# bigpon/QPNet

Measured on AMD Instinct MI355X. Metric: train steps/sec (batch-1 chunk-steps of RF+20000 samples, aggregate over GPUs), higher is better.
Workload: dtype f32; 1 GPU; config[1]: paper-size SI-QPNet (C=64,S=256,4F+4A) training step, forward+CE+backward+Adam on one chunk of 20900 samples (RF 946 + batch_length 19954), batch 1 per GPU; global_batch=1, parallelism=dp1 (utterance-sharded chunks, one flat-gradient all-reduce per step), backend=none, world_size=1, aux_1x1=frame rate (hoisted: K = 128 + one 4-deep step)

## Files before the change

qpnet_amd/csrc/train_bwd.hip:

```cpp
#include "train_common.h"
#include "train_post.h"
#include "qpn_handle.h"
#include <string.h>
#include <stdlib.h>
#include <math.h>

template <int MT>
__global__ __launch_bounds__(512) void k_post_bwd(TrainParams p, TrainBwd bw) {
    constexpr int TM = 16 * MT;
    extern __shared__ float sm[];
    const int S = p.S, Q = p.Q, LC = p.LC;
    const int ldp = tr_lda(Q > S ? Q : S), ldr = tr_lda(S);
    float* P = sm; float* R = sm + TM * ldp;
    const int b = blockIdx.y, t0 = blockIdx.x * TM;
    const int tid = threadIdx.x, lane = tid & 63, wave = tid >> 6;
    const int NTS = S / 16;
    const int npairs = (NTS + 1) / 2;
    const int np0 = wave < npairs ? wave : 0;
    const int pnt[2] = {2 * np0, (2 * np0 + 1 < NTS) ? 2 * np0 + 1 : 2 * np0};
    float my[2][MT][4], ms[2][MT][4];
    auto mask_load = [&](const float* src, float (&m)[2][MT][4]) {
#pragma unroll
        for (int j = 0; j < 2; ++j)
#pragma unroll
// ... 288 lines not shown
        rdg = *(const float4*)(DGS + (__umul24((unsigned)nw, (unsigned)p.LC) + 4u * sc4));
    };
    auto store_rows = [&](int t, float* B) {
        const int n = ly.s_out + t * 16 + srow;
        const bool in = n < N1;
        const float4 z = make_float4(0.f, 0.f, 0.f, 0.f);
        const float4 dx = (in && !LAST) ? make_float4(ra.x + rb2.x, ra.y + rb2.y, ra.z + rb2.z, ra.w + rb2.w) : z;
        const float4 sg = in ? rsg : z, th = in ? rth : z, dg = (in && n >= win0) ? rdg : z;
        float* d0 = B + (size_t)srow * ldx + 4 * sc4;
        *(float2*)d0 = make_float2(dx.x, dx.y); *(float2*)(d0 + 2) = make_float2(dx.z, dx.w);
        float* d1 = d0 + 16 * ldx; *(float2*)d1 = make_float2(sg.x, sg.y); *(float2*)(d1 + 2) = make_float2(sg.z, sg.w);
        float* d2 = d1 + 16 * ldx; *(float2*)d2 = make_float2(th.x, th.y); *(float2*)(d2 + 2) = make_float2(th.z, th.w);
        float* d3 = d2 + 16 * ldx; *(float2*)d3 = make_float2(dg.x, dg.y); *(float2*)(d3 + 2) = make_float2(dg.z, dg.w);
    };
    const int zrow = tid >> 6, zc2 = (tid & 63) * 2;
    float* const dmy = dummy + (size_t)(blockIdx.y * gridDim.x + blockIdx.x) * 2 * 128;
    int tprow[4], tpnext[4];
    auto load_taps = [&](int t, int (&tp)[4]) {
#pragma unroll
        for (int i = 0; i < 4; ++i) { const int n = ly.s_out + t * 16 + 4 * wave + i; tp[i] = taps[n < N1 ? n : N1 - 1]; }
    };
    float2 cwj[4], nwj[4]; float cpa[4], npa[4]; int cpoff = 0, npoff = 0;
    auto load_aux = [&](int t, float2 (&wj)[4], float (&pa)[4], int& poff) {
        const int n0 = ly.s_out + t * 16;
        poff = tr_pa_off(p, l, b, n0);
        const float2* w = p.WJ + n0 + 4 * (lane >> 4);
        const float* q4 = p.PA + poff + 16 * wave + (lane & 15);
#pragma unroll
        for (int i = 0; i < 4; ++i) wj[i] = w[i];
        pa[0] = q4[0]; pa[1] = q4[C]; pa[2] = q4[2 * C]; pa[3] = q4[3 * C];
    };
    load_rows(t_first);
    if constexpr (HOIST) load_aux(t_first, cwj, cpa, cpoff);
    load_taps(t_first, tprow);
    store_rows(t_first, sm);
    const int arow = lane & 15, ak = lane >> 4;
    const int c = 16 * wave + (lane & 15);
    for (int ti = 0; ti < t_count; ++ti) {
        const int t = t_first + ti, n0 = ly.s_out + t * 16;
        float* Dx = sm + (ti & 1) * 4 * 16 * ldx; float* Sg = Dx + 16 * ldx; float* Th = Sg + 16 * ldx; float* Dg = Th + 16 * ldx;
        { const int tn = t + 1 < t_last ? t + 1 : t_last; load_rows(tn); load_taps(tn, tpnext); if constexpr (HOIST) load_aux(tn, nwj, npa, npoff); }
        TR_LDS_BARRIER();
        float xa[4][4];
#pragma unroll
        for (int ks = 0; ks < 4; ++ks) { const float* ap = Dx + (size_t)arow * ldx + 16 * ks + ak; xa[ks][0] = ap[0]; xa[ks][1] = ap[4]; xa[ks][2] = ap[8]; xa[ks][3] = ap[12]; }
        __builtin_amdgcn_sched_barrier(0);
        f32x4 a0 = (f32x4){0, 0, 0, 0}, a1 = (f32x4){0, 0, 0, 0};
        if (!LAST) {
#pragma unroll
            for (int ks = 0; ks < 4; ks += 2) {
                a0 = __builtin_amdgcn_mfma_f32_16x16x4f32(xa[ks][0], wr[ks].x, a0, 0, 0, 0); a1 = __builtin_amdgcn_mfma_f32_16x16x4f32(xa[ks + 1][0], wr[ks + 1].x, a1, 0, 0, 0);
                a0 = __builtin_amdgcn_mfma_f32_16x16x4f32(xa[ks][1], wr[ks].y, a0, 0, 0, 0); a1 = __builtin_amdgcn_mfma_f32_16x16x4f32(xa[ks + 1][1], wr[ks + 1].y, a1, 0, 0, 0);
                a0 = __builtin_amdgcn_mfma_f32_16x16x4f32(xa[ks][2], wr[ks].z, a0, 0, 0, 0); a1 = __builtin_amdgcn_mfma_f32_16x16x4f32(xa[ks + 1][2], wr[ks + 1].z, a1, 0, 0, 0);
                a0 = __builtin_amdgcn_mfma_f32_16x16x4f32(xa[ks][3], wr[ks].w, a0, 0, 0, 0); a1 = __builtin_amdgcn_mfma_f32_16x16x4f32(xa[ks + 1][3], wr[ks + 1].w, a1, 0, 0, 0);
            }
        }
        float dzs[4], dzt[4];
#pragma unroll
        for (int i = 0; i < 4; ++i) {
            const int r = 4 * (lane >> 4) + i;
            const float dg = (a0[i] + a1[i]) + Dg[(size_t)r * ldx + c];
            const float sg = Sg[(size_t)r * ldx + c], th = Th[(size_t)r * ldx + c];
            tr_gate_bwd(dg, sg, th, dzs[i], dzt[i]);
            Dz[(size_t)r * ldz + c] = dzs[i];
            Dz[(size_t)r * ldz + C + c] = dzt[i];
        }
        float dacc[4] = {0.f, 0.f, 0.f, 0.f}, eacc[2] = {0.f, 0.f};
        if constexpr (HOIST) {
            const TrAuxBwd ab = tr_aux_bwd(cwj, cpa, dzs, dzt, lane);
#pragma unroll
            for (int k = 0; k < 4; ++k) dacc[k] = ab.d[k];
            eacc[0] = ab.e[0]; eacc[1] = ab.e[1];
            if ((lane & 15) == 0) { float* gq = Gp + 16 * wave + 4 * (lane >> 4); gq[0] = ab.gp[0]; gq[1] = ab.gp[1]; gq[2] = ab.gp[2]; gq[3] = ab.gp[3]; }
        }
        TR_LDS_BARRIER();
        float za[8][4];
#pragma unroll
        for (int ks = 0; ks < 8; ++ks) { const float* zp = Dz + (size_t)arow * ldz + 16 * ks + ak; za[ks][0] = zp[0]; za[ks][1] = zp[4]; za[ks][2] = zp[8]; za[ks][3] = zp[12]; }
        __builtin_amdgcn_sched_barrier(0);
        f32x4 acc[NJ];
#pragma unroll
        for (int j = 0; j < NJ; ++j) acc[j] = (f32x4){0, 0, 0, 0};
#pragma unroll
        for (int ks = 0; ks < 8; ++ks) {
#pragma unroll
            for (int j = 0; j < NJ; ++j) acc[j] = __builtin_amdgcn_mfma_f32_16x16x4f32(za[ks][0], w1[j][ks].x, acc[j], 0, 0, 0);
#pragma unroll
            for (int j = 0; j < NJ; ++j) acc[j] = __builtin_amdgcn_mfma_f32_16x16x4f32(za[ks][1], w1[j][ks].y, acc[j], 0, 0, 0);
#pragma unroll
            for (int j = 0; j < NJ; ++j) acc[j] = __builtin_amdgcn_mfma_f32_16x16x4f32(za[ks][2], w1[j][ks].z, acc[j], 0, 0, 0);
#pragma unroll
            for (int j = 0; j < NJ; ++j) acc[j] = __builtin_amdgcn_mfma_f32_16x16x4f32(za[ks][3], w1[j][ks].w, acc[j], 0, 0, 0);
        }
        {
#pragma unroll
            for (int k = 0; k < 4; ++k) {
                const int r = zrow + 4 * k;
                float* d = DZg + (__umul24((unsigned)(n0 + r), 2u * C) + zc2);
                d = n0 + r < N1 ? d : dmy + zc2;
                *(float2*)d = *(const float2*)(Dz + (size_t)r * ldz + zc2);
            }
        }
#pragma unroll
        for (int j = 0; j < NJ; ++j) {
            const int nt = wave + 4 * j;
            if (nt >= NTK) continue;
#pragma unroll
            for (int i = 0; i < 4; ++i) Os[(size_t)(4 * (lane >> 4) + i) * ldo + 16 * nt + (lane & 15)] = acc[j][i];
        }
        TR_LDS_BARRIER();
#pragma unroll
        for (int i = 0; i < 4; ++i) {
            const int r = 4 * wave + i, n = n0 + r;
            const bool in = n < N1;
            const float own = Os[(size_t)r * ldo + lane] + Dx[(size_t)r * ldx + lane];
            float* da = DAout + (__umul24((unsigned)n, (unsigned)C) + lane);
            *(in ? da : dmy + lane) = own;
            const float past = Os[(size_t)r * ldo + C + lane];
            float* db = DBout + (__umul24((unsigned)tprow[i], (unsigned)C) + lane);
            db = in ? db : dmy + 128 + lane;
            if (ly.adaptive) atomicAdd(db, past);
            else *db = past;
            if constexpr (!HOIST) if (lane < Ap) {
                float* dh = DH + (__umul24((unsigned)n, (unsigned)Ap) + lane);
                atomicAdd(in ? dh : dmy + 192 + lane, Os[(size_t)r * ldo + 2 * C + lane]);
            }
        }
        if constexpr (HOIST) {
            if (lane < 16) {
                float* dp = bw.DPA + cpoff + 16 * wave + lane;
                atomicAdd(dp, dacc[0]); atomicAdd(dp + C, dacc[1]); atomicAdd(dp + 2 * C, dacc[2]); atomicAdd(dp + 3 * C, dacc[3]);
                float* ep = bw.EB + (size_t)(l * TR_EB_SLOTS + (blockIdx.x & (TR_EB_SLOTS - 1))) * 2 * C + 16 * wave + lane;
                atomicAdd(ep, eacc[0]); atomicAdd(ep + C, eacc[1]);
            }
            if (tid < 16 && n0 + tid < N1) GWl[n0 + tid] = (Gp[tid] + Gp[16 + tid]) + (Gp[32 + tid] + Gp[48 + tid]);
        }
        store_rows(t + 1 < t_last ? t + 1 : t_last, sm + ((ti + 1) & 1) * 4 * 16 * ldx);
#pragma unroll
        for (int i = 0; i < 4; ++i) tprow[i] = tpnext[i];
        if constexpr (HOIST) {
#pragma unroll
            for (int i = 0; i < 4; ++i) { cwj[i] = nwj[i]; cpa[i] = npa[i]; }
            cpoff = npoff;
        }
    }
}

struct Wg2 {
    const float* A; const float* A2; size_t A_lstride; int lda, M;
    int rowsA;
    int bmode; const float* B1; const float* B2; size_t B_lstride; int ldb, N, Nvalid;
    int rowsB;
    const float* hup; const int* tap; int C, Ap;
    const int* xc;
    int nb, nlayers;
    float* slab; int gstage;
    int row0A[TR_MAXL], row0B[TR_MAXL], R[TR_MAXL];
    int goff[TR_MAXL], gbias[TR_MAXL], tap_off[TR_MAXL], dil[TR_MAXL];
    int ldc, ncol_groups;
};

struct Wg2L {
    const float* A; const float* A2; const float* B1; const float* B2; const float* hup; const int* tap;
    int lda, ldb, M, Ng, Nvalid, rowsA, rowsB, row0A, row0B, C, Ap, dil, nb, ncol0, rend;
    unsigned uR;
};

template <int NB>
__device__ __forceinline__ void wg_taps(const Wg2L& q, int rs, int (&tp)[NB], bool b_act, int b_row0, int b_rstep) {
#pragma unroll
    for (int k = 0; k < NB; ++k) {
        const int r = b_row0 + k * b_rstep, rr = rs + r;
        int v = 0;
        if (b_act && r < 32 && rr < q.rend) {
            const unsigned b = q.nb > 1 ? (unsigned)rr / q.uR : 0u; const int i = rr - (int)(b * q.uR);
            const int nloc = q.row0B + i;
            v = q.tap ? q.tap[(size_t)b * q.rowsB + nloc] : nloc - q.dil;
        }
        tp[k] = v;
    }
}

template <int BMODE, int NA, int NB>
__device__ __forceinline__ void wg_fetch(const Wg2L& q, int rs, float4 (&ra)[NA], float4 (&ra2)[NA], float4 (&rb)[NB], float4 (&rb2)[NB], const int (&tpv)[NB],
                                         bool a_act, int a_row0, int a_rstep, int a_col, bool b_act, int b_row0, int b_rstep, int b_col) {
#pragma unroll
    for (int k = 0; k < NA; ++k) {
        const int r = a_row0 + k * a_rstep, rr = rs + r;
        float4 v = make_float4(0.f, 0.f, 0.f, 0.f), v2 = v;
        if (a_act && r < 32 && rr < q.rend && a_col < q.M) {
            const unsigned b = q.nb > 1 ? (unsigned)rr / q.uR : 0u; const int i = rr - (int)(b * q.uR);
            const size_t o = ((size_t)b * q.rowsA + q.row0A + i) * q.lda + a_col;
            v = *(const float4*)(q.A + o);
            if (q.A2) v2 = *(const float4*)(q.A2 + o);
        }
        ra[k] = v; ra2[k] = v2;
    }
#pragma unroll
    for (int k = 0; k < NB; ++k) {
        const int r = b_row0 + k * b_rstep, rr = rs + r;
        const int n = q.ncol0 + b_col;
        float4 v = make_float4(0.f, 0.f, 0.f, 0.f), v2 = make_float4(1.f, 1.f, 1.f, 1.f);
        if (b_act && r < 32 && rr < q.rend && b_col < q.Ng && n < q.Nvalid) {
            const unsigned b = q.nb > 1 ? (unsigned)rr / q.uR : 0u; const int i = rr - (int)(b * q.uR);
            const int nloc = q.row0B + i;
            const size_t row = (size_t)b * q.rowsB + nloc;
            if (BMODE <= 1) v = *(const float4*)(q.B1 + row * q.ldb + n);
            else if (BMODE == 2) { v = *(const float4*)(q.B1 + row * q.ldb + n); v2 = *(const float4*)(q.B2 + row * q.ldb + n); }
            else {
                if (n < q.C) v = *(const float4*)(q.B1 + row * q.C + n);
                else if (n < 2 * q.C) v = *(const float4*)(q.B1 + ((size_t)b * q.rowsB + tpv[k]) * q.C + (n - q.C));
                else v = *(const float4*)(q.hup + row * q.Ap + (n - 2 * q.C));
            }
        }
        rb[k] = v; rb2[k] = v2;
    }
}

template <int BMODE, int MPW, int NTMAX>
__global__ __launch_bounds__(256) void k_wgrad2(Wg2 w, int nch) {
    extern __shared__ float sm[];
    constexpr int RS = 32;
    constexpr int NA = 2 * MPW;
    constexpr int NB = (NTMAX + 1) / 2 + 1;
    const int y = blockIdx.y, ch = blockIdx.x, zg = blockIdx.z;
    const int Mp = (w.M + 15) & ~15, Ng = w.N / w.ncol_groups, Np = (Ng + 15) & ~15;
    const int ldA = tr_ldt(Mp), ldB = tr_ldt(Np);
    float* As = sm; float* Bs = sm + RS * ldA;
    const int tid = threadIdx.x, lane = tid & 63, wave = tid >> 6;
    const int MT = Mp / 16, NT = Np / 16;
    const int Rl = w.R[y];
    const int64_t total = (int64_t)Rl * w.nb;
    const int64_t per = ((total + nch - 1) / nch + RS - 1) / RS * RS;
    const int rbeg = (int)(per * ch), rend = (int)(per * ch + per < total ? per * ch + per : total);
    Wg2L q;
    q.A = w.A + (size_t)y * w.A_lstride; q.A2 = w.A2 ? w.A2 + (size_t)y * w.A_lstride : nullptr;
    q.B1 = w.B1 + (size_t)y * w.B_lstride; q.B2 = w.B2 ? w.B2 + (size_t)y * w.B_lstride : nullptr;
    q.hup = w.hup; q.tap = (w.tap && w.tap_off[y] >= 0) ? w.tap + w.tap_off[y] : nullptr;
    q.lda = w.lda; q.ldb = w.ldb; q.M = w.M; q.Ng = Ng; q.Nvalid = w.Nvalid; q.rowsA = w.rowsA; q.rowsB = w.rowsB;
    q.row0A = w.row0A[y]; q.row0B = w.row0B[y]; q.C = w.C; q.Ap = w.Ap; q.dil = w.dil[y]; q.nb = w.nb; q.ncol0 = zg * Ng; q.rend = rend;
    q.uR = (unsigned)(Rl > 0 ? Rl : 1);
    const int gbias = zg == 0 ? w.gbias[y] : -1, goff = w.goff[y];
    const int A4 = Mp / 4, B4 = Np / 4;
    const int a_col = (tid % A4) * 4, a_row0 = tid / A4, a_rstep = 256 / A4;
    const int b_rstep = 256 / B4 > 0 ? 256 / B4 : 1;
    const int b_col = (tid % B4) * 4, b_row0 = tid / B4;
    const bool a_act = tid < a_rstep * A4, b_act = tid < b_rstep * B4;
    f32x4 acc[MPW][NTMAX];
#pragma unroll
    for (int a = 0; a < MPW; ++a)
#pragma unroll
        for (int b = 0; b < NTMAX; ++b) acc[a][b] = (f32x4){0, 0, 0, 0};
    float csum = 0.f;
    float4 ra[NA], ra2[NA], rb[NB], rb2[NB];
    int tpv[NB];
#pragma unroll
    for (int k = 0; k < NB; ++k) tpv[k] = 0;
    if (BMODE == 3 && rbeg < rend) wg_taps<NB>(q, rbeg, tpv, b_act, b_row0, b_rstep);
    if (rbeg < rend) wg_fetch<BMODE, NA, NB>(q, rbeg, ra, ra2, rb, rb2, tpv, a_act, a_row0, a_rstep, a_col, b_act, b_row0, b_rstep, b_col);
    if (BMODE == 3 && rbeg + RS < rend) wg_taps<NB>(q, rbeg + RS, tpv, b_act, b_row0, b_rstep);
    const int g = lane >> 4, cl = lane & 15;
    for (int rs = rbeg; rs < rend; rs += RS) {
#pragma unroll
        for (int k = 0; k < NA; ++k) {
            const int r = a_row0 + k * a_rstep;
            if (a_act && r < RS) {
                float4 v = ra[k];
                v.x += ra2[k].x; v.y += ra2[k].y; v.z += ra2[k].z; v.w += ra2[k].w;
                *(float4*)(As + (size_t)r * ldA + a_col) = v;
            }
        }
#pragma unroll
        for (int k = 0; k < NB; ++k) {
            const int r = b_row0 + k * b_rstep;
            if (b_act && r < RS) {
                float4 v = rb[k];
                if (BMODE == 1) { v.x = fmaxf(v.x, 0.f); v.y = fmaxf(v.y, 0.f); v.z = fmaxf(v.z, 0.f); v.w = fmaxf(v.w, 0.f); }
                else if (BMODE == 2) { v.x *= rb2[k].x; v.y *= rb2[k].y; v.z *= rb2[k].z; v.w *= rb2[k].w; }
                *(float4*)(Bs + (size_t)r * ldB + b_col) = v;
            }
        }
        __syncthreads();
        if (rs + RS < rend) wg_fetch<BMODE, NA, NB>(q, rs + RS, ra, ra2, rb, rb2, tpv, a_act, a_row0, a_rstep, a_col, b_act, b_row0, b_rstep, b_col);
        if (BMODE == 3 && rs + 2 * RS < rend) wg_taps<NB>(q, rs + 2 * RS, tpv, b_act, b_row0, b_rstep);
        if (gbias >= 0 && tid < q.M) { float s = 0.f; for (int r = 0; r < RS; ++r) s += As[r * ldA + tid]; csum += s; }
#pragma unroll
        for (int ks = 0; ks < RS / 4; ++ks) {
            float bfr[NTMAX];
#pragma unroll
            for (int nt = 0; nt < NTMAX; ++nt) bfr[nt] = nt < NT ? Bs[(4 * ks + g) * ldB + 16 * nt + cl] : 0.f;
#pragma unroll
            for (int mi = 0; mi < MPW; ++mi) {
                const int mt = wave + 4 * mi;
                if (mt < MT) {
                    const float a = As[(4 * ks + g) * ldA + 16 * mt + cl];
#pragma unroll
                    for (int nt = 0; nt < NTMAX; ++nt)
                        if (nt < NT) acc[mi][nt] = __builtin_amdgcn_mfma_f32_16x16x4f32(a, bfr[nt], acc[mi][nt], 0, 0, 0);
                }
            }
        }
        __syncthreads();
    }
    float* out = w.slab + (size_t)ch * w.gstage;
#pragma unroll
    for (int mi = 0; mi < MPW; ++mi) {
        const int mt = wave + 4 * mi;
        if (mt >= MT) continue;
#pragma unroll
        for (int nt = 0; nt < NTMAX; ++nt) {
            if (nt >= NT) continue;
#pragma unroll
            for (int i = 0; i < 4; ++i) {
                const int m = 16 * mt + 4 * (lane >> 4) + i, n = 16 * nt + (lane & 15);
                if (m < q.M && n < Ng) out[goff + (size_t)m * w.ldc + q.ncol0 + n] = acc[mi][nt][i];
            }
        }
    }
    if (gbias >= 0 && tid < q.M) out[gbias + tid] = csum;
}

template <int BMODE, int MPW, int NTMAX>
static int launch_wgrad2(const Wg2& w, int nch, hipStream_t stream) {
    const int Mp = (w.M + 15) & ~15, Np = ((w.N / w.ncol_groups) + 15) & ~15;
    if (Mp / 16 > 4 * MPW || Np / 16 > NTMAX) return -1;
    const size_t lds = (size_t)32 * (tr_ldt(Mp) + tr_ldt(Np)) * sizeof(float);
    if (lds > 64 * 1024) (void)hipFuncSetAttribute((const void*)k_wgrad2<BMODE, MPW, NTMAX>, hipFuncAttributeMaxDynamicSharedMemorySize, (int)lds);
    hipLaunchKernelGGL((k_wgrad2<BMODE, MPW, NTMAX>), dim3(nch, w.nlayers, w.ncol_groups), dim3(256), lds, stream, w, nch);
    return 0;
}
template <int BMODE>
static bool wgrad2_mode(const Wg2& w, int nch, hipStream_t stream) {
    if (launch_wgrad2<BMODE, 1, 4>(w, nch, stream) == 0) return true;
    if (launch_wgrad2<BMODE, 4, 4>(w, nch, stream) == 0) return true;
    if (launch_wgrad2<BMODE, 2, 12>(w, nch, stream) == 0) return true;
    if (launch_wgrad2<BMODE, 4, 8>(w, nch, stream) == 0) return true;
    return false;
}
struct UpArgs { const float* h; const float* DHUP; float* gflat; int64_t up_w, up_b; float gscale; int U, Ap, A, F, N1, nfr, B; };
static UpArgs up_args(const TrainParams& p, const TrainBwd& bw) {
    UpArgs u; u.h = p.h; u.DHUP = bw.DHUP; u.gflat = bw.gflat; u.gscale = bw.gscale; u.U = p.U; u.Ap = p.Ap; u.A = p.A; u.F = p.F; u.N1 = p.N1;
    u.up_w = p.up_w; u.up_b = p.up_b; u.B = p.B;
    const int64_t q0 = (int64_t)p.F * p.U - p.N1;
    u.nfr = p.U > 0 ? (int)(((int64_t)p.F * p.U - 1) / p.U - q0 / p.U + 1) : 0;
    return u;
}
__device__ __forceinline__ void up_bwd_body(const UpArgs& p, int fx, int b, int tid, int nthr) {
    __shared__ float hcol[64];
    __shared__ float red[4];
    const int U = p.U, Ap = p.Ap, A = p.A;
    const int64_t q0 = (int64_t)p.F * U - p.N1;
    const int f = (int)(q0 / U) + fx;
    float dsum = 0.f;
    for (int a0 = 0; a0 < A; a0 += 64) {
        __syncthreads();
        if (tid < 64) hcol[tid] = (a0 + tid < A && f < p.F) ? p.h[((size_t)b * A + a0 + tid) * p.F + f] : 0.f;
        __syncthreads();
        for (int j = tid; j < U; j += nthr) {
            const int64_t n = (int64_t)f * U + j - q0;
            if (n < 0 || n >= p.N1 || f >= p.F) continue;
            const float* row = p.DHUP + ((size_t)b * p.N1 + n) * Ap + a0;
            float acc = 0.f;
            const int na = A - a0 < 64 ? A - a0 : 64;
            const int nq = na >> 2;
            float4 v[16];
#pragma unroll
            for (int q = 0; q < 16; ++q) v[q] = *(const float4*)(row + 4 * (q < nq ? q : 0));
#pragma unroll
            for (int q = 0; q < 16; ++q)
                if (q < nq) { acc += v[q].x * hcol[4 * q] + v[q].y * hcol[4 * q + 1] + v[q].z * hcol[4 * q + 2] + v[q].w * hcol[4 * q + 3]; dsum += (v[q].x + v[q].y) + (v[q].z + v[q].w); }
            for (int a = 4 * nq; a < na; ++a) { const float v1 = row[a]; acc += v1 * hcol[a]; dsum += v1; }
            atomicAdd(&p.gflat[p.up_w + j], acc * p.gscale);
        }
    }
    for (int s = 32; s >= 1; s >>= 1) dsum += __shfl_xor(dsum, s);
    if ((tid & 63) == 0) red[tid >> 6] = dsum;
    __syncthreads();
    if (tid == 0) { float a = 0.f; for (int k = 0; k < nthr / 64; ++k) a += red[k]; atomicAdd(&p.gflat[p.up_b], a * p.gscale); }
}

template <int BMODE, int MPW, int NT, bool TWO_A>
__device__ __forceinline__ void wgrad3_body(const Wg2& w, const int nch, const int ch, const int y, const int zg) {
    extern __shared__ float sm[];
    constexpr int RS = 32, Mp = 64 * MPW, Np = 16 * NT;
    constexpr int ldA = ((Mp + 15) / 32) * 32 + 16, ldB = ((Np + 15) / 32) * 32 + 16;
    constexpr int A4 = Mp / 4, ARS = 256 / A4, NA = RS / ARS;
    constexpr int B4 = Np / 4, BRS = 256 / B4, NB = (RS + BRS - 1) / BRS;
    static_assert(256 % A4 == 0 && RS % ARS == 0, "A staging must tile the stage's rows exactly");
    constexpr int BUF = RS * (ldA + ldB);
    float* As = sm; float* Bs = sm + RS * ldA;
    const int tid = threadIdx.x, lane = tid & 63, wave = tid >> 6;
    const int Rl = w.R[y];
    const int64_t total = (int64_t)Rl * w.nb;
    const int64_t per = ((total + nch - 1) / nch + RS - 1) / RS * RS;
    const int rbeg = (int)(per * ch), rend = (int)(per * ch + per < total ? per * ch + per : total);
    const float* A = w.A + (size_t)y * w.A_lstride;
    const float* A2 = TWO_A ? w.A2 + (size_t)y * w.A_lstride : nullptr;
    const float* B1 = BMODE == 4 ? nullptr : w.B1 + (size_t)y * w.B_lstride;
    const float* B2 = w.B2 ? w.B2 + (size_t)y * w.B_lstride : nullptr;
    const int* tap = BMODE == 3 ? w.tap + w.tap_off[y] : nullptr;
    const int row0A = w.row0A[y], row0B = w.row0B[y], ncol0 = zg * Np;
    const unsigned uR = (unsigned)(Rl > 0 ? Rl : 1);
    const bool multi = w.nb > 1;
    const int gbias = zg == 0 ? w.gbias[y] : -1, goff = w.goff[y];
    const int a_col = (tid % A4) * 4, a_row0 = tid / A4;
    const int b_col = (tid % B4) * 4, b_row0 = tid / B4;
    const int n = ncol0 + b_col;
    const bool b_act = tid < BRS * B4;
    const bool b_pad = n >= w.Nvalid;
    const float* bbase; int bstride; bool use_tap = false;
    if (BMODE == 3) {
        if (n < w.C) { bbase = B1 + n; bstride = w.C; }
        else if (n < 2 * w.C) { bbase = B1 + (n - w.C); bstride = w.C; use_tap = true; }
        else { bbase = w.hup + (b_pad ? 0 : n - 2 * w.C); bstride = w.Ap; }
    } else if (BMODE == 4) { bbase = nullptr; bstride = 0; }
    else { bbase = B1 + n; bstride = w.ldb; }
    const ptrdiff_t b2off = (BMODE == 2) ? (B2 - B1) : 0;

    f32x4 acc[MPW][NT];
#pragma unroll
    for (int a = 0; a < MPW; ++a)
#pragma unroll
        for (int b = 0; b < NT; ++b) acc[a][b] = (f32x4){0, 0, 0, 0};
    float4 cs4 = make_float4(0.f, 0.f, 0.f, 0.f);
    float4 ra[NA], ra2[NA], rb[NB], rb2[NB];
    int tpv[NB];
    int rbi[NB];
    unsigned okA = 0, okB = 0;

    const unsigned a_voff = (unsigned)a_row0 * (unsigned)w.lda + (unsigned)a_col, a_kstep = (unsigned)ARS * (unsigned)w.lda;
    const unsigned b_voff = (unsigned)b_row0 * (unsigned)w.ldb + (unsigned)n, b_kstep = (unsigned)BRS * (unsigned)w.ldb;

    auto rowsplit = [&](int rr, int& b, int& i) { if (multi) { b = (int)((unsigned)rr / uR); i = rr - b * (int)uR; } else { b = 0; i = rr; } };
    auto stage_fast = [&](int rs, int& b0, int& i0) {
        rowsplit(rs, b0, i0);
        return rs + RS <= rend && i0 + RS <= (int)uR;
    };
    auto taps = [&](int rs) {
        int b0, i0;
        if (stage_fast(rs, b0, i0)) {
            const int* tst = tap + ((size_t)b0 * w.rowsB + row0B + i0);
#pragma unroll
            for (int k = 0; k < NB; ++k) { const int r = b_row0 + k * BRS; tpv[k] = tst[r < RS ? r : b_row0]; }
            return;
        }
#pragma unroll
        for (int k = 0; k < NB; ++k) {
            const int r = b_row0 + k * BRS;
            int rr = rs + r; rr = rr < rend ? rr : rend - 1;
            int b, i; rowsplit(rr, b, i);
            const int nloc = row0B + i;
            tpv[k] = tap[(size_t)b * w.rowsB + nloc];
        }
    };
    auto fetch = [&](int rs) {
        const float* pa[NA]; const float* pb[NB]; const int* pi[NB];
        int b0, i0;
        if (stage_fast(rs, b0, i0)) {
            const float* Ast = A + ((size_t)b0 * w.rowsA + row0A + i0) * w.lda;
#pragma unroll
            for (int k = 0; k < NA; ++k) pa[k] = Ast + (k * a_kstep + a_voff);
            okA = ~0u;
            const size_t brow = (size_t)b0 * w.rowsB + row0B + i0;
            const float* bsrc = BMODE == 3 ? bbase + (size_t)b0 * w.rowsB * bstride : B1 + brow * w.ldb;
#pragma unroll
            for (int k = 0; k < NB; ++k) {
                const int r = b_row0 + k * BRS;
                if (BMODE == 4) pi[k] = w.xc + brow + (r < RS ? r : b_row0);
                else if (BMODE == 3) {
                    const unsigned row = use_tap ? (unsigned)tpv[k] : (unsigned)(row0B + i0 + (r < RS ? r : b_row0));
                    pb[k] = bsrc + __umul24(row, (unsigned)bstride);
                } else pb[k] = bsrc + ((r < RS ? k * b_kstep : 0u) + b_voff);
            }
            okB = b_pad ? 0u : ~0u;
        } else {
            okA = 0; okB = 0;
#pragma unroll
            for (int k = 0; k < NA; ++k) {
                const int r = a_row0 + k * ARS;
                int rr = rs + r; const bool ok = rr < rend; rr = ok ? rr : rend - 1;
                int b, i; rowsplit(rr, b, i);
                pa[k] = A + (((size_t)b * w.rowsA + row0A + i) * w.lda + a_col);
                okA |= ok ? 1u << k : 0u;
            }
#pragma unroll
            for (int k = 0; k < NB; ++k) {
                const int r = b_row0 + k * BRS;
                int rr = rs + r; const bool ok = r < RS && rr < rend && !b_pad; rr = rr < rend ? rr : rend - 1;
                int b, i; rowsplit(rr, b, i);
                const size_t row = (size_t)b * w.rowsB + ((BMODE == 3 && use_tap) ? tpv[k] : row0B + i);
                if (BMODE == 4) pi[k] = w.xc + row; else pb[k] = bbase + row * bstride;
                okB |= ok ? 1u << k : 0u;
            }
        }
#pragma unroll
        for (int k = 0; k < NA; ++k) {
            ra[k] = *(const float4*)pa[k];
            if (TWO_A) ra2[k] = *(const float4*)(pa[k] + (A2 - A));
        }
        if (b_act) {
#pragma unroll
            for (int k = 0; k < NB; ++k) {
                if (BMODE == 4) rbi[k] = *pi[k];
                else {
                    rb[k] = *(const float4*)pb[k];
                    if (BMODE == 2) rb2[k] = *(const float4*)(pb[k] + b2off);
                }
            }
        }
    };
    if (rbeg < rend) {
        if (BMODE == 3) taps(rbeg);
        fetch(rbeg);
        if (BMODE == 3 && rbeg + RS < rend) taps(rbeg + RS);
    }
    const int g = lane >> 4, cl = lane & 15;
    auto to_lds = [&](int buf) {
        float* Ab = As + buf * BUF; float* Bb = Bs + buf * BUF;
#pragma unroll
        for (int k = 0; k < NA; ++k) {
            float4 v = ra[k];
            if (TWO_A) { v.x += ra2[k].x; v.y += ra2[k].y; v.z += ra2[k].z; v.w += ra2[k].w; }
            { const bool ok = (okA >> k) & 1u; v.x = ok ? v.x : 0.f; v.y = ok ? v.y : 0.f; v.z = ok ? v.z : 0.f; v.w = ok ? v.w : 0.f; }
            cs4.x += v.x; cs4.y += v.y; cs4.z += v.z; cs4.w += v.w;
            *(float4*)(Ab + (size_t)(a_row0 + k * ARS) * ldA + a_col) = v;
        }
        if (b_act) {
#pragma unroll
            for (int k = 0; k < NB; ++k) {
                const int r = b_row0 + k * BRS;
                if (r < RS) {
                    float4 v;
                    if (BMODE == 4) { const int dlt = rbi[k] - n; v = make_float4(dlt == 0 ? 1.f : 0.f, dlt == 1 ? 1.f : 0.f, dlt == 2 ? 1.f : 0.f, dlt == 3 ? 1.f : 0.f); }
                    else v = rb[k];
                    if (BMODE == 1) { v.x = fmaxf(v.x, 0.f); v.y = fmaxf(v.y, 0.f); v.z = fmaxf(v.z, 0.f); v.w = fmaxf(v.w, 0.f); }
                    else if (BMODE == 2) { v.x *= rb2[k].x; v.y *= rb2[k].y; v.z *= rb2[k].z; v.w *= rb2[k].w; }
                    { const bool ok = (okB >> k) & 1u; v.x = ok ? v.x : 0.f; v.y = ok ? v.y : 0.f; v.z = ok ? v.z : 0.f; v.w = ok ? v.w : 0.f; }
                    *(float4*)(Bb + (size_t)r * ldB + b_col) = v;
                }
            }
        }
    };
    auto ksteps = [&](int buf, int k0, int k1) {
        const float* Ab = As + buf * BUF; const float* Bb = Bs + buf * BUF;
#pragma unroll
        for (int ks = k0; ks < k1; ++ks) {
            float bfr[NT];
#pragma unroll
            for (int nt = 0; nt < NT; ++nt) bfr[nt] = Bb[(4 * ks + g) * ldB + 16 * nt + cl];
#pragma unroll
            for (int mi = 0; mi < MPW; ++mi) {
                const float a = Ab[(4 * ks + g) * ldA + 16 * (wave + 4 * mi) + cl];
#pragma unroll
                for (int nt = 0; nt < NT; ++nt) acc[mi][nt] = __builtin_amdgcn_mfma_f32_16x16x4f32(a, bfr[nt], acc[mi][nt], 0, 0, 0);
            }
        }
    };
    for (int rs = rbeg; rs < rend; rs += RS) {
        to_lds(0);
        __syncthreads();
        if (rs + RS < rend) {
            fetch(rs + RS);
            if (BMODE == 3 && rs + 2 * RS < rend) taps(rs + 2 * RS);
        }
        ksteps(0, 0, RS / 4);
        __syncthreads();
    }
    float* out = w.slab + (size_t)ch * w.gstage;
#pragma unroll
    for (int mi = 0; mi < MPW; ++mi) {
        const int mt = wave + 4 * mi;
#pragma unroll
        for (int nt = 0; nt < NT; ++nt) {
#pragma unroll
            for (int i = 0; i < 4; ++i) {
                const int m = 16 * mt + 4 * (lane >> 4) + i, nn = 16 * nt + (lane & 15);
                out[goff + (size_t)m * w.ldc + ncol0 + nn] = acc[mi][nt][i];
            }
        }
    }
    if (gbias >= 0) {
        *(float4*)(sm + (size_t)a_row0 * Mp + a_col) = cs4;
        __syncthreads();
        if (tid < Mp) { float s = 0.f; for (int r = 0; r < ARS; ++r) s += sm[r * Mp + tid]; out[gbias + tid] = s; }
    }
}
template <int BMODE, int MPW, int NT, bool TWO_A, int MINW = 1>
__global__ __launch_bounds__(256, MINW) void k_wgrad3(Wg2 w, int nch) {
    wgrad3_body<BMODE, MPW, NT, TWO_A>(w, nch, blockIdx.x, blockIdx.y, blockIdx.z);
}

#ifndef QPN_WGRAD_MINW
#define QPN_WGRAD_MINW 2
#endif
template <int BMODE, int MPW, int NT, bool TWO_A>
static void launch_wgrad3_k(const Wg2& w, int nch, size_t lds, hipStream_t stream) {
    constexpr int MINW = (MPW == 4 && NT == 4 && !TWO_A) ? QPN_WGRAD_MINW : 1;
    if (lds > 64 * 1024) (void)hipFuncSetAttribute((const void*)k_wgrad3<BMODE, MPW, NT, TWO_A, MINW>, hipFuncAttributeMaxDynamicSharedMemorySize, (int)lds);
    hipLaunchKernelGGL((k_wgrad3<BMODE, MPW, NT, TWO_A, MINW>), dim3(nch, w.nlayers, w.ncol_groups), dim3(256), lds, stream, w, nch);
}
template <int BMODE, int MPW, int NT>
static bool wgrad3_fits(const Wg2& w) {
    const int Ng = w.N / w.ncol_groups;
    if (w.bmode != BMODE) return false;
    if (w.rowsB >= (1 << 24) || (int64_t)w.rowsB * (w.C > w.ldb ? w.C : w.ldb) >= (1ll << 32)) return false;
    if (w.M != 64 * MPW || Ng != 16 * NT || w.N % w.ncol_groups || (w.Nvalid != w.N && (w.ncol_groups != 1 || w.Nvalid % 4))) return false;
    if (BMODE == 3 && (w.ldb != w.C || w.ncol_groups != 1 || (w.C % 4) || (w.Ap % 4) || !w.tap)) return false;
    if (BMODE == 3) for (int l = 0; l < w.nlayers; ++l) if (w.tap_off[l] < 0) return false;
    return true;
}
template <int MPW, int NT> static constexpr size_t wgrad3_lds() { return (size_t)32 * (tr_ldt(64 * MPW) + tr_ldt(16 * NT)) * sizeof(float); }
template <int BMODE, int MPW, int NT>
static bool launch_wgrad3(const Wg2& w, int nch, hipStream_t stream) {
    if (!wgrad3_fits<BMODE, MPW, NT>(w)) return false;
    const size_t lds = wgrad3_lds<MPW, NT>();
    if (w.A2) launch_wgrad3_k<BMODE, MPW, NT, true>(w, nch, lds, stream);
    else launch_wgrad3_k<BMODE, MPW, NT, false>(w, nch, lds, stream);
    return true;
}
static bool wgrad3_any(const Wg2& w, int nch, bool generic, hipStream_t stream) {
    if (w.bmode == 4) return launch_wgrad3<4, 1, 8>(w, nch, stream) || launch_wgrad3<4, 1, 4>(w, nch, stream);
    if (generic) return false;
    switch (w.bmode) {
    case 3: return launch_wgrad3<3, 2, 11>(w, nch, stream) || launch_wgrad3<3, 2, 8>(w, nch, stream) || launch_wgrad3<3, 1, 7>(w, nch, stream);
    case 0: return launch_wgrad3<0, 1, 4>(w, nch, stream) || launch_wgrad3<0, 4, 4>(w, nch, stream);
    case 1: return launch_wgrad3<1, 4, 4>(w, nch, stream);
    default: return false;
    }
}

static int wgrad_col_groups(int M, int N) {
    const int nt_max = M <= 64 ? 4 : M <= 128 ? 12 : 8;
    for (int g = 1; g <= N / 16; ++g)
        if (N % g == 0 && (N / g) % 4 == 0 && (N / g + 15) / 16 <= nt_max) return g;
    return 1;
}

static bool wgrad2_any(const Wg2& w, int nch, bool generic, hipStream_t stream) {
    if (w.M > 256 && w.bmode != 4) {
        bool ok = true;
        for (int m0 = 0; m0 < w.M && ok; m0 += 256) {
            Wg2 sub = w;
            sub.A = w.A + m0; if (w.A2) sub.A2 = w.A2 + m0;
            sub.M = w.M - m0 < 256 ? w.M - m0 : 256;
            for (int l = 0; l < w.nlayers; ++l) { sub.goff[l] = w.goff[l] + m0 * w.ldc; if (w.gbias[l] >= 0) sub.gbias[l] = w.gbias[l] + m0; }
            sub.ncol_groups = wgrad_col_groups(sub.M, sub.N);
            ok = wgrad2_any(sub, nch, generic, stream);
        }
        return ok;
    }
    if (wgrad3_any(w, nch, generic, stream)) return true;
    switch (w.bmode) {
    case 4: return false;
    case 1: return wgrad2_mode<1>(w, nch, stream);
    case 2: return wgrad2_mode<2>(w, nch, stream);
    case 3: return wgrad2_mode<3>(w, nch, stream);
    default: return wgrad2_mode<0>(w, nch, stream);
    }
}

__global__ void k_reduce_grad_s(const float* __restrict__ slab, const int* __restrict__ gdst, const int* __restrict__ gdst_list, const int* __restrict__ gzero, int n_gzero,
                                int nch, int gstage, int64_t n, float* __restrict__ g, float scale, int append_scale, int s0, int s1, int skip0, int skip1, int tail,
                                const int* __restrict__ status, int flag_again) {
    int64_t i = (int64_t)blockIdx.x * blockDim.x + threadIdx.x + s0;
    if (flag_again && append_scale && i == s0) g[n + 1] = (status && *status) ? 1.f : 0.f;
    if (i < s1) {
        if (i >= skip0 && i < skip1) return;
        const int k0 = gdst[i], k1 = gdst[i + 1];
        if (k0 == k1) return;
        float a = 0.f;
        const float* sp = slab + i;
        int c = 0;
        for (; c + 8 <= nch; c += 8) {
            float v[8];
#pragma unroll
            for (int k = 0; k < 8; ++k) v[k] = sp[(size_t)(c + k) * gstage];
            a += ((v[0] + v[1]) + (v[2] + v[3])) + ((v[4] + v[5]) + (v[6] + v[7]));
        }
        for (; c < nch; ++c) a += sp[(size_t)c * gstage];
        a *= scale;
        for (int k = k0; k < k1; ++k) g[gdst_list[k]] = a;
        return;
    }
    if (!tail) return;
    const int64_t j = i - s1;
    if (j < n_gzero) g[gzero[j]] = 0.f;
    else if (append_scale && j < n_gzero + 4 && !(flag_again && j == n_gzero + 1)) g[n + (j - n_gzero)] = j == n_gzero ? scale : (j == n_gzero + 1 && status && *status) ? 1.f : 0.f;
}

__global__ __launch_bounds__(256) void k_causal_bwd(TrainParams p, TrainBwd bw, int rows_per_wg, int CB) {
    extern __shared__ float tab[];
    const int C = p.C, Q = p.Q;
    const int tid = threadIdx.x;
    const int64_t total = (int64_t)p.B * p.N1;
    const int64_t r0 = (int64_t)blockIdx.x * rows_per_wg, r1 = r0 + rows_per_wg < total ? r0 + rows_per_wg : total;
    for (int cb = 0; cb < C; cb += CB) {
        const int cbv = C - cb < CB ? C - cb : CB;
        for (int i = tid; i < 2 * Q * CB; i += 256) tab[i] = 0.f;
        __syncthreads();
        const int cpr = cbv;
        for (int64_t idx = r0 * cpr + tid; idx < r1 * cpr; idx += 256) {
            const int64_t rr = idx / cpr; const int c = (int)(idx - rr * cpr);
            const int b = (int)(rr / p.N1), n = (int)(rr - (int64_t)b * p.N1);
            const size_t o = ((size_t)b * p.N1 + n) * C + cb + c;
            const float v = bw.DXA[0][o] + bw.DXB[0][o];
            const int64_t xo = (int64_t)p.T - p.N0 + n;
            int64_t s0 = p.x[(size_t)b * p.T + xo] % Q, s1 = p.x[(size_t)b * p.T + xo + 1] % Q;
            if (s0 < 0) s0 += Q;
            if (s1 < 0) s1 += Q;
            atomicAdd(&tab[(0 * Q + s0) * CB + c], v);
            atomicAdd(&tab[(1 * Q + s1) * CB + c], v);
        }
        __syncthreads();
        for (int i = tid; i < 2 * Q * cbv; i += 256) {
            const int c = i / (2 * Q), qt = i - c * 2 * Q, q = qt >> 1, tp = qt & 1;
            const float v = tab[(tp * Q + q) * CB + c];
            if (v != 0.f) atomicAdd(&bw.gflat[p.causal_w + ((size_t)(cb + c) * Q + q) * 2 + tp], v * bw.gscale);
        }
        for (int c = tid; c < cbv; c += 256) {
            float s = 0.f;
            for (int q = 0; q < Q; ++q) s += tab[(0 * Q + q) * CB + c];
            atomicAdd(&bw.gflat[p.causal_b + cb + c], s * bw.gscale);
        }
        __syncthreads();
    }
}

__global__ __launch_bounds__(128) void k_up_bwd(UpArgs u) { up_bwd_body(u, blockIdx.x, blockIdx.y, threadIdx.x, 128); }

__global__ __launch_bounds__(128) void k_aux_tail(AuxArgs p) {
    __shared__ float hrow[1024];
    __shared__ float red[2];
    const AuxGeom& ag = p.g;
    const int C = p.C, A = p.A, L = p.L, tid = threadIdx.x;
    const int bx = blockIdx.x;
    float v = 0.f;
    const bool role_a = bx < L * A;
    if (role_a) {
        const int l = bx / A, a = bx - l * A, n = tid;
        const size_t wi = (n < C ? ag.auxS[l] + (size_t)n * A : ag.auxT[l] + (size_t)(n - C) * A) + a;
        const float va = p.flat[wi];
        float e = 0.f;
        {
            float ev[TR_EB_SLOTS];
#pragma unroll
            for (int k = 0; k < TR_EB_SLOTS; ++k) ev[k] = p.EB[(size_t)(l * TR_EB_SLOTS + k) * 2 * C + n];
#pragma unroll
            for (int k = 0; k < TR_EB_SLOTS; ++k) e += ev[k];
        }
        float acc = 0.f;
        for (int b = 0; b < p.B; ++b) {
            const float* hb = p.h + ((size_t)b * A + a) * p.F + p.ffirst;
            const float* D = p.DPA + (size_t)(l * p.B + b) * (p.nfr + 1) * 2 * C + n;
            for (int f0 = 0; f0 < p.nfr; f0 += 1024) {
                const int nf = p.nfr - f0 < 1024 ? p.nfr - f0 : 1024;
                __syncthreads();
                for (int i = tid; i < nf; i += 128) hrow[i] = hb[f0 + i];
                __syncthreads();
                int f = 0;
                for (; f + 64 <= nf; f += 64) {
                    float d[64];
#pragma unroll
                    for (int k = 0; k < 64; ++k) d[k] = D[(size_t)(f0 + f + k) * 2 * C];
#pragma unroll
                    for (int k = 0; k < 64; ++k) acc += d[k] * hrow[f + k];
                }
                for (; f + 16 <= nf; f += 16) {
                    float d[16];
#pragma unroll
                    for (int k = 0; k < 16; ++k) d[k] = D[(size_t)(f0 + f + k) * 2 * C];
#pragma unroll
                    for (int k = 0; k < 16; ++k) acc += d[k] * hrow[f + k];
                }
                for (; f < nf; ++f) acc += D[(size_t)(f0 + f) * 2 * C] * hrow[f];
            }
        }
        p.gflat[wi] = (acc + p.flat[p.up_b] * e) * p.gscale;
        v = va * e;
    } else {
        const int j = bx - L * A;
        const int q0 = p.F * p.U - p.N1;
        const int items = L * p.B * p.nfr;
        for (int it = tid; it < items; it += 128) {
            const int fx = it % p.nfr, lb = it / p.nfr, l = lb / p.B;
            const int n = (p.ffirst + fx) * p.U + j - q0;
            if (n >= ag.s_out[l] && n < p.N1) v += p.GW[(size_t)lb * p.N1 + n];
        }
    }
    for (int sft = 32; sft >= 1; sft >>= 1) v += __shfl_xor(v, sft);
    if ((tid & 63) == 0) red[tid >> 6] = v;
    __syncthreads();
    if (tid == 0) {
        if (role_a) atomicAdd(p.gflat + p.up_b, (red[0] + red[1]) * p.gscale);
        else p.gflat[p.up_w + (bx - L * A)] = (red[0] + red[1]) * p.gscale;
    }
}

struct AdamReports { int* h_status; double* h_loss; const double* d_loss; };
__device__ __forceinline__ void adam_update(float* __restrict__ w, float* __restrict__ m, float* __restrict__ v, int64_t i, float gi,
                                            float lr, float b1, float b2, float eps, float wd, float bc1, float bc2_sqrt) {
    if (wd != 0.f) gi += wd * w[i];
    const float mi = m[i] + (gi - m[i]) * (1.0f - b1);
    const float vi = v[i] * b2 + (1.0f - b2) * gi * gi;
    m[i] = mi; v[i] = vi;
    const float denom = sqrtf(vi) / bc2_sqrt + eps;
    w[i] = w[i] - (lr / bc1) * (mi / denom);
}
__global__ void k_adam(float* __restrict__ w, const float* __restrict__ g, float* __restrict__ m, float* __restrict__ v, int64_t n,
                       float lr, float b1, float b2, float eps, float wd, float bc1, float bc2_sqrt, const float* __restrict__ den, int* __restrict__ status, AdamReports rep) {
    int64_t i = (int64_t)blockIdx.x * blockDim.x + threadIdx.x;
    const bool peer = den && den[1] > 0.f;
    const bool skip = peer || (status && *status);
    if (blockIdx.x == 0) {
        if (rep.h_loss && threadIdx.x < 64) rep.h_loss[threadIdx.x] = rep.d_loss[threadIdx.x];
        if (threadIdx.x == 0 && status) {
            int st = *status;
            if (peer && !st) { st = 8; atomicOr(status, 8); }
            if (rep.h_status) *rep.h_status = st;
            if (!skip) atomicAdd((unsigned long long*)(status + 2), 1ull);
        }
    }
    if (i >= n || skip) return;
    float gi = g[i];
    if (den) gi = gi / den[0];
    adam_update(w, m, v, i, gi, lr, b1, b2, eps, wd, bc1, bc2_sqrt);
}

__device__ __forceinline__ double block_sum_f64(double x, double* red) {
    for (int sft = 32; sft >= 1; sft >>= 1) x += __shfl_xor(x, sft);
    if ((threadIdx.x & 63) == 0) red[threadIdx.x >> 6] = x;
    __syncthreads();
    return (red[0] + red[1]) + (red[2] + red[3]);
}
__global__ __launch_bounds__(256) void k_grad_sumsq(const float* __restrict__ g, int64_t n, double* __restrict__ part) {
    __shared__ double red[4];
    const int64_t nq = n >> 2, nthr = (int64_t)gridDim.x * 256, t = (int64_t)blockIdx.x * 256 + threadIdx.x;
    double acc = 0.0;
    if ((reinterpret_cast<uintptr_t>(g) & 15) == 0) {
        const float4* g4 = reinterpret_cast<const float4*>(g);
#pragma unroll 4
        for (int64_t q = t; q < nq; q += nthr) {
            const float4 x = g4[q];
            acc += (double)x.x * (double)x.x; acc += (double)x.y * (double)x.y; acc += (double)x.z * (double)x.z; acc += (double)x.w * (double)x.w;
        }
    } else {
#pragma unroll 4
        for (int64_t q = t; q < nq; q += nthr) {
            const float x0 = g[4 * q], x1 = g[4 * q + 1], x2 = g[4 * q + 2], x3 = g[4 * q + 3];
            acc += (double)x0 * (double)x0; acc += (double)x1 * (double)x1; acc += (double)x2 * (double)x2; acc += (double)x3 * (double)x3;
        }
    }
    if (t == nq % nthr) for (int64_t i = nq * 4; i < n; ++i) acc += (double)g[i] * (double)g[i];
    const double s = block_sum_f64(acc, red);
    if (threadIdx.x == 0) part[blockIdx.x] = s;
}

__global__ __launch_bounds__(256) void k_adam_clip(float* __restrict__ w, const float* __restrict__ g, float* __restrict__ m, float* __restrict__ v, int64_t n,
                                                   float lr, float b1, float b2, float eps, float wd, float bc1, float bc2_sqrt, const float* __restrict__ den, int* __restrict__ status, AdamReports rep,
                                                   const double* __restrict__ part, int npart, float max_norm, double* __restrict__ d_norm, double* h_norm) {
    __shared__ double red[4];
    int64_t i = (int64_t)blockIdx.x * blockDim.x + threadIdx.x;
    double total = sqrt(block_sum_f64((int)threadIdx.x < npart ? part[threadIdx.x] : 0.0, red));
    if (den) total = total / (double)den[0];
    const bool bad = !isfinite(total);
    const bool peer = den && den[1] > 0.f;
    const bool skip = bad || peer || (status && *status);
    if (blockIdx.x == 0) {
        if (rep.h_loss && threadIdx.x < 64) rep.h_loss[threadIdx.x] = rep.d_loss[threadIdx.x];
        if (threadIdx.x == 0) {
            *d_norm = total;
            if (h_norm) *h_norm = total;
            if (status) {
                int st = *status;
                if (peer && !st) { st = 8; atomicOr(status, 8); }
                if (bad) { st |= 1 << 16; atomicOr(status, 1 << 16); }
                if (rep.h_status) *rep.h_status = st;
                if (!skip) atomicAdd((unsigned long long*)(status + 2), 1ull);
            }
        }
    }
    if (i >= n || skip) return;
    const double c = (double)max_norm / (total + 1e-6);
    const float coef = c < 1.0 ? (float)c : 1.0f;
    float gi = g[i];
    if (den) gi = gi / den[0];
    gi = __fmul_rn(gi, coef);
    adam_update(w, m, v, i, gi, lr, b1, b2, eps, wd, bc1, bc2_sqrt);
}

__device__ __forceinline__ void zero_dx_slice(const TrainParams& p, const TrainBwd& bw, int j, int b, size_t part, size_t nparts, int t, int nthr) {
    const int C = p.C;
    const TrLayer ly = p.layers[j];
    const size_t nDX = (size_t)p.B * p.N1 * C;
    float* A = bw.DXA[0] + (size_t)j * nDX + (size_t)b * p.N1 * C;
    float* Bq = bw.DXB[0] + (size_t)j * nDX + (size_t)b * p.N1 * C;
    const int a0 = j == 0 ? 0 : ly.s_in, a1 = ly.s_out;
    const int b0 = ly.adaptive ? 0 : p.N1 - ly.dilation, b1 = p.N1;
    const size_t na = (size_t)(a1 - a0) * C / 4, nb = (size_t)(b1 > b0 ? b1 - b0 : 0) * C / 4;
    const float4 z = make_float4(0.f, 0.f, 0.f, 0.f);
    const size_t nh = p.hoist ? (size_t)(p.nfr + 1) * 2 * C / 4 : (j == 0 ? (size_t)p.N1 * p.Ap / 4 : 0);
    const size_t ne = (p.hoist && b == 0) ? (size_t)TR_EB_SLOTS * 2 * C / 4 : 0;
    float* H = p.hoist ? bw.DPA + (size_t)(j * p.B + b) * (p.nfr + 1) * 2 * C : bw.DHUP + (size_t)b * p.N1 * p.Ap;
    for (size_t i = part * nthr + t; i < na + nb + nh + ne; i += nparts * nthr) {
        if (i < na) ((float4*)(A + (size_t)a0 * C))[i] = z;
        else if (i < na + nb) ((float4*)(Bq + (size_t)(b0 > 0 ? b0 : 0) * C))[i - na] = z;
        else if (i < na + nb + nh) ((float4*)H)[i - na - nb] = z;
        else ((float4*)(bw.EB + (size_t)j * TR_EB_SLOTS * 2 * C))[i - na - nb - nh] = z;
    }
}
__global__ void k_zero_dx(TrainParams p, TrainBwd bw) {
    zero_dx_slice(p, bw, blockIdx.y, blockIdx.z, blockIdx.x, gridDim.x, threadIdx.x, blockDim.x);
}

void qpn_launch_zero_dx(const TrainParams& p, const TrainBwd& bw, hipStream_t stream) {
    hipLaunchKernelGGL(k_zero_dx, dim3(64, p.L, p.B), dim3(256), 0, stream, p, bw);
}

static void launch_reduce_early(const TrainBwd& bw, hipStream_t st, int tail, int nch_side) {
    const TrainSlabs& sl = *bw.sl;
    const int64_t n = (int64_t)(sl.g_early1 - sl.g_early0) + (tail ? bw.n_gzero + 4 : 0);
    hipLaunchKernelGGL(k_reduce_grad_s, dim3((unsigned)((n + 255) / 256)), dim3(256), 0, st, bw.slab, bw.gdst, bw.gdst_list, bw.gzero, bw.n_gzero,
                       nch_side, bw.gstage, bw.n_params, bw.gflat, bw.gscale, bw.append_scale, sl.g_early0, sl.g_early1, 0, 0, tail, bw.status, 0);
}
static void launch_up_bwd(const TrainParams& p, const TrainBwd& bw, hipStream_t st) {
    const UpArgs u = up_args(p, bw);
    hipLaunchKernelGGL(k_up_bwd, dim3(u.nfr, p.B), dim3(128), 0, st, u);
}

static void launch_aux_tail(const TrainParams& p, const TrainBwd& bw, const AuxGeom& ag, hipStream_t st) {
    hipLaunchKernelGGL(k_aux_tail, dim3(p.L * p.A + p.U), dim3(128), 0, st, tr_aux_args(p, &bw, ag));
}

int qpn_launch_grad_tail(const TrainParams& p, const TrainBwd& bw, const AuxGeom* ag, hipStream_t stream, bool early_done, bool up_done) {
    const int C = p.C, Q = p.Q, B = p.B, N1 = p.N1;
    const TrainSlabs& sl = *bw.sl;
    hipLaunchKernelGGL(k_reduce_grad_s, dim3((unsigned)(((int64_t)bw.gstage + (up_done ? 0 : bw.n_gzero + 4) + 255) / 256)), dim3(256), 0, stream, bw.slab, bw.gdst, bw.gdst_list, bw.gzero, bw.n_gzero,
                       bw.nch, bw.gstage, bw.n_params, bw.gflat, bw.gscale, bw.append_scale, 0, bw.gstage, early_done ? sl.g_early0 : 0, early_done ? sl.g_early1 : 0, up_done ? 0 : 1, bw.status, bw.append_scale == 1 ? 1 : 0);
    {
        const int64_t total = (int64_t)B * N1;
        const int nwg = 128, rpw = (int)((total + nwg - 1) / nwg);
        if (sl.g_cw < 0) {
            int CB = C < 64 ? C : 64;
            while (CB > 1 && (size_t)2 * Q * CB * sizeof(float) > 128 * 1024) CB /= 2;
            const size_t lds_c = (size_t)2 * Q * CB * sizeof(float);
            if (lds_c > 160 * 1024) { qpn_set_error("causal-table gradient: n_quantize too large for the LDS histogram"); return QPN_EINVAL; }
            if (lds_c > 48 * 1024) QPN_HIP(hipFuncSetAttribute((const void*)k_causal_bwd, hipFuncAttributeMaxDynamicSharedMemorySize, (int)lds_c));
            hipLaunchKernelGGL(k_causal_bwd, dim3(nwg), dim3(256), lds_c, stream, p, bw, rpw, CB);
        }
        if (p.U > 0 && !up_done && !p.hoist) launch_up_bwd(p, bw, stream);
        if (p.hoist && ag && !up_done) launch_aux_tail(p, bw, *ag, stream);
    }
    qpn_prof_mark(PG_GRAD_TAIL, stream);
    QPN_HIP(hipGetLastError());
    return QPN_OK;
}

bool qpn_stack_bwd_fits(const TrainParams& p);
int qpn_launch_stack_bwd(const TrainParams& p, const TrainBwd& bw, const StackQ& q, const TrainKnobs& k, hipStream_t stream);

void qpn_launch_post_fb(const TrainParams& p, const TrainBwd& bw, hipStream_t stream) {
    constexpr int MTW = 5;
    const size_t ldsw = (size_t)16 * MTW * (tr_lda(256) + 2 * tr_lda(64)) * sizeof(float);
    (void)hipFuncSetAttribute((const void*)k_post_fb_w<MTW>, hipFuncAttributeMaxDynamicSharedMemorySize, (int)ldsw);
    hipLaunchKernelGGL((k_post_fb_w<MTW>), dim3((p.BL + 16 * MTW - 1) / (16 * MTW), p.B), dim3(512), ldsw, stream, p, bw, 1);
}

int qpn_launch_bwd(const TrainParams& p, const TrainBwd& bw, const TrainKnobs& k, const AuxGeom& ag, const StackQ* sq, hipStream_t stream, bool post_done) {
    const int C = p.C, S = p.S, Q = p.Q, L = p.L, B = p.B, N1 = p.N1, BL = p.BL;
    const TrainSlabs& sl = *bw.sl;
    const bool off32 = N1 < (1 << 24) && (int64_t)N1 * (p.LC > 2 * C ? p.LC : 2 * C) < (1ll << 32);
    const bool persist = C == 64 && (p.Ktp == 176 || p.hoist) && p.Ap <= 64 && off32 && k.persist_bwd;
    const bool stack_q = persist && k.stack_q_bwd && sq && sq->flags && p.qctl && qpn_stack_bwd_fits(p);
    const bool wr_summed = stack_q;
    const size_t nDX = (size_t)B * N1 * C;
    const size_t lds_post = (size_t)16 * (tr_lda(Q > S ? Q : S) + tr_lda(S)) * sizeof(float);
    const size_t lds_layer = (size_t)16 * (4 * tr_lda(C) + tr_lda(2 * C)) * sizeof(float);
    if (lds_post > 160 * 1024 || lds_layer > 160 * 1024) { qpn_set_error("backward tiles do not fit LDS"); return QPN_EINVAL; }
    hipStream_t side = bw.side; hipEvent_t ev_fork = bw.ev_fork, ev_join = bw.ev_join;
    const bool overlap = side && !qpn_prof_serial() && !k.serial;
    const bool post_wide = S == 256 && Q == 256 && C == 64 && (p.LC == 256 || p.LC == 512) && k.post_wide;
    const bool zero_in_post = post_wide && k.zero_in_post;
    if (post_done) { }
    else if (!zero_in_post) qpn_launch_zero_dx(p, bw, stream);
    if (post_done) { }
    else if (post_wide) {
        constexpr int MTW = 5;
        const size_t ldsw = (size_t)16 * MTW * tr_lda(256) * sizeof(float);
        QPN_HIP(hipFuncSetAttribute((const void*)k_post_bwd_w<MTW>, hipFuncAttributeMaxDynamicSharedMemorySize, (int)ldsw));
        hipLaunchKernelGGL((k_post_bwd_w<MTW>), dim3((BL + 16 * MTW - 1) / (16 * MTW), B), dim3(512), ldsw, stream, p, bw, zero_in_post ? 1 : 0);
    } else {
        if (lds_post > 48 * 1024) (void)hipFuncSetAttribute((const void*)k_post_bwd<1>, hipFuncAttributeMaxDynamicSharedMemorySize, (int)lds_post);
        hipLaunchKernelGGL((k_post_bwd<1>), dim3((BL + 15) / 16, B), dim3(512), lds_post, stream, p, bw);
    }
    qpn_prof_mark(PG_POST_BWD, stream);
    const int nch = bw.nch;
    int nch_side_ = nch;
    const bool gen = k.wgrad_generic;
    Wg2 wbase; memset(&wbase, 0, sizeof(wbase));
    wbase.slab = bw.slab; wbase.gstage = bw.gstage; wbase.nb = B; wbase.C = C; wbase.Ap = p.Ap; wbase.hup = p.HUP; wbase.tap = p.TAP; wbase.ncol_groups = 1;
    bool ok = true;
    auto launch_skip_post = [&](hipStream_t st) {
        Wg2 w = wbase;
        {
            w.nlayers = L;
            w.A = bw.DS0; w.A2 = nullptr; w.A_lstride = 0; w.lda = S; w.M = S; w.rowsA = BL;
            w.bmode = 0; w.B1 = p.TH; w.B2 = nullptr; w.B_lstride = nDX; w.ldb = C; w.N = C; w.Nvalid = C; w.rowsB = N1; w.ldc = C;
            w.ncol_groups = wgrad_col_groups(w.M, w.N);
            for (int l = 0; l < L; ++l) { w.row0A[l] = 0; w.row0B[l] = N1 - BL; w.R[l] = BL; w.goff[l] = sl.g_ws[l]; w.gbias[l] = l == 0 ? sl.g_bs : -1; w.tap_off[l] = -1; }
            ok = ok && wgrad2_any(w, nch_side_, gen, st);
            qpn_prof_mark(PG_WGRAD_SKIP, st);
        }
        {
            w.nlayers = 1; w.A_lstride = w.B_lstride = 0; w.B2 = nullptr; w.bmode = 1; w.rowsA = w.rowsB = BL;
            w.row0A[0] = w.row0B[0] = 0; w.R[0] = BL; w.tap_off[0] = -1;
            w.ncol_groups = S % 64 == 0 ? S / 64 : 1;
            w.A = bw.dlogits; w.lda = Q; w.M = Q; w.B1 = p.Y0; w.ldb = S; w.N = S; w.Nvalid = S; w.ldc = S; w.goff[0] = sl.g_p2; w.gbias[0] = sl.g_bp2;
            if (Q == S && k.post_pair) {
                w.nlayers = 2;
                w.A_lstride = (size_t)(bw.DY0 - bw.dlogits); w.B_lstride = (size_t)(p.S0 - p.Y0);
                w.row0A[1] = w.row0B[1] = 0; w.R[1] = BL; w.tap_off[1] = -1; w.goff[1] = sl.g_p1; w.gbias[1] = sl.g_bp1;
                ok = ok && wgrad2_any(w, nch_side_, gen, st);
            } else {
                ok = ok && wgrad2_any(w, nch_side_, gen, st);
                w.A = bw.DY0; w.lda = S; w.M = S; w.B1 = p.S0; w.goff[0] = sl.g_p1; w.gbias[0] = sl.g_bp1;
                ok = ok && wgrad2_any(w, nch_side_, gen, st);
            }
            qpn_prof_mark(PG_WGRAD_POST, st);
        }
    };
    auto build_w1 = [&]() {
        Wg2 w = wbase;
        w.A = bw.DZ; w.A2 = nullptr; w.A_lstride = (size_t)B * N1 * 2 * C; w.lda = 2 * C; w.M = 2 * C; w.rowsA = N1;
        w.bmode = 3; w.B1 = p.X; w.B2 = nullptr; w.B_lstride = nDX; w.ldb = C; w.N = p.Ktp; w.Nvalid = p.hoist ? 2 * C : 2 * C + p.Ap; w.rowsB = N1;
        w.nlayers = L; w.ldc = p.Ktp; w.ncol_groups = wgrad_col_groups(w.M, w.N);
        for (int l = 0; l < L; ++l) {
            const TrLayer& ly = p.layers[l];
            w.row0A[l] = w.row0B[l] = ly.s_out; w.R[l] = N1 - ly.s_out; w.goff[l] = sl.g_w1[l]; w.gbias[l] = sl.g_b1[l];
            w.tap_off[l] = ly.tap_off; w.dil[l] = ly.dilation;
        }
        return w;
    };
    auto build_wr = [&]() {
        Wg2 w = wbase;
        w.A = bw.DXA[0] + nDX; w.A2 = wr_summed ? nullptr : bw.DXB[0] + nDX; w.A_lstride = nDX; w.lda = C; w.M = C; w.rowsA = N1;
        w.bmode = 0; w.B1 = p.TH; w.B2 = nullptr; w.B_lstride = nDX; w.ldb = C; w.N = C; w.Nvalid = C; w.rowsB = N1; w.ldc = C;
        w.nlayers = L; w.ncol_groups = wgrad_col_groups(w.M, w.N);
        for (int l = 0; l < L; ++l) {
            w.row0A[l] = w.row0B[l] = p.layers[l].s_out;
            w.R[l] = l == L - 1 ? 0 : N1 - p.layers[l].s_out; w.goff[l] = sl.g_wr[l]; w.gbias[l] = sl.g_br[l]; w.tap_off[l] = -1; w.dil[l] = 0;
        }
        return w;
    };
    const bool early_reduce = overlap && bw.gdst && sl.g_early1 > sl.g_early0 && k.reduce_early;
    const bool up_side = early_reduce && p.U > 0 && k.up_side;
    if (early_reduce) {
        nch_side_ = k.wgrad_chunks_side > 0 && k.wgrad_chunks_side <= nch ? k.wgrad_chunks_side : (nch <= 48 ? nch : 48);
    }
    if (overlap) {
        QPN_HIP(hipEventRecord(ev_fork, stream));
        QPN_HIP(hipStreamWaitEvent(side, ev_fork, 0));
        qpn_prof_mark(-1, side);
        launch_skip_post(side);
        if (early_reduce) { launch_reduce_early(bw, side, up_side ? 1 : 0, nch_side_); qpn_prof_mark(PG_GRAD_TAIL, side); }
        if (early_reduce && up_side && bw.ev_early && bw.early_recorded) { QPN_HIP(hipEventRecord(bw.ev_early, side)); *bw.early_recorded = 1; }
    }
    const int swz = k.xcd_swizzle ? 1 : 0;
    if (p.hoist && !persist) { qpn_set_error("internal: the frame-rate aux term needs the register-resident layer kernels"); return QPN_EINVAL; }
    if (stack_q) {
        const int rcq = qpn_launch_stack_bwd(p, bw, *sq, k, stream);
        if (rcq) return rcq;
    }
    for (int l = L - 1; l >= 0 && !stack_q; --l) {
        const TrLayer& ly = p.layers[l];
        const int rows = N1 - ly.s_out;
        const int tiles = (rows + 15) / 16;
        if (persist) {
            int G = qpn_num_cus() * 2; if (G > tiles) G = tiles;
            if (G > 1024) G = 1024;
            const size_t ldsp = (size_t)(8 * 16 * tr_lda(C) + 16 * tr_lda(2 * C) + 16 * tr_lda(p.Ktp) + 64) * sizeof(float);
            const bool last = l == L - 1;
            const void* kf = p.hoist ? (last ? (const void*)k_layer_bwd_p<8, true> : (const void*)k_layer_bwd_p<8, false>)
                                     : (last ? (const void*)k_layer_bwd_p<11, true> : (const void*)k_layer_bwd_p<11, false>);
            (void)hipFuncSetAttribute(kf, hipFuncAttributeMaxDynamicSharedMemorySize, (int)ldsp);
            if (p.hoist) {
                if (last) hipLaunchKernelGGL((k_layer_bwd_p<8, true>), dim3(G, B), dim3(256), ldsp, stream, p, bw, l, swz ? 2 : 0, tiles, p.scratch_rows);
                else hipLaunchKernelGGL((k_layer_bwd_p<8, false>), dim3(G, B), dim3(256), ldsp, stream, p, bw, l, swz ? 2 : 0, tiles, p.scratch_rows);
            } else {
                if (last) hipLaunchKernelGGL((k_layer_bwd_p<11, true>), dim3(G, B), dim3(256), ldsp, stream, p, bw, l, swz ? 2 : 0, tiles, p.scratch_rows);
                else hipLaunchKernelGGL((k_layer_bwd_p<11, false>), dim3(G, B), dim3(256), ldsp, stream, p, bw, l, swz ? 2 : 0, tiles, p.scratch_rows);
            }
        } else {
            if (lds_layer > 48 * 1024) (void)hipFuncSetAttribute((const void*)k_layer_bwd<1>, hipFuncAttributeMaxDynamicSharedMemorySize, (int)lds_layer);
            hipLaunchKernelGGL((k_layer_bwd<1>), dim3(tiles, B), dim3(256), lds_layer, stream, p, bw, l, l == L - 1 ? 1 : 0, swz);
        }
    }
    auto build_causal = [&]() {
        Wg2 w = wbase;
        w.nlayers = 2; w.ncol_groups = Q / (Q % 64 == 0 ? 64 : 128);      w.bmode = 4; w.xc = p.XC; w.B1 = w.B2 = nullptr; w.B_lstride = 0;
        w.A = bw.DXA[0]; w.A2 = bw.DXB[0]; w.A_lstride = 0; w.lda = C; w.M = C; w.rowsA = N1;
        w.N = Q; w.Nvalid = Q; w.rowsB = N1 + 1; w.ldb = 0; w.ldc = Q;
        for (int tp = 0; tp < 2; ++tp) { w.row0A[tp] = 0; w.row0B[tp] = tp; w.R[tp] = N1; w.goff[tp] = sl.g_cw + tp * C * Q; w.gbias[tp] = tp == 0 ? sl.g_cb : -1; w.tap_off[tp] = -1; w.dil[tp] = 0; }
        return w;
    };
    const bool wr_side = overlap && k.wr_side;
    if (wr_side || up_side) {
        QPN_HIP(hipEventRecord(bw.ev_mid, stream));
        QPN_HIP(hipStreamWaitEvent(side, bw.ev_mid, 0));
        qpn_prof_mark(-1, side);
        if (up_side) { if (p.hoist) launch_aux_tail(p, bw, ag, side); else launch_up_bwd(p, bw, side); qpn_prof_mark(PG_GRAD_TAIL, side); }
        if (wr_side) { ok = ok && wgrad2_any(build_wr(), nch, gen, side); qpn_prof_mark(PG_WGRAD_WR, side); }
    }
    if (overlap) QPN_HIP(hipEventRecord(ev_join, side));
    qpn_prof_mark(PG_LAYER_BWD, stream);
    ok = ok && wgrad2_any(build_w1(), nch, gen, stream);
    qpn_prof_mark(PG_WGRAD, stream);
    if (!wr_side) { ok = ok && wgrad2_any(build_wr(), nch, gen, stream); qpn_prof_mark(PG_WGRAD_WR, stream); }
    if (!overlap) launch_skip_post(stream);
    if (sl.g_cw >= 0) ok = ok && wgrad2_any(build_causal(), nch, gen, stream);
    qpn_prof_mark(PG_WGRAD_CAUSAL, stream);
    if (overlap) { QPN_HIP(hipStreamWaitEvent(stream, ev_join, 0)); qpn_prof_mark(-1, stream); }
    if (!ok) { qpn_set_error("weight-gradient tiles: unsupported geometry (n_resch <= 128 on this path; wider stacks take the GEMM path)"); return QPN_EINVAL; }
    return qpn_launch_grad_tail(p, bw, &ag, stream, early_reduce, up_side);
}

int qpn_launch_adam(float* w, const float* g, float* m, float* v, int64_t n, int step, float lr, float b1, float b2, float eps, float wd, const float* den, int* status,
                    int* h_status, double* h_loss, const double* d_loss, hipStream_t stream) {
    const double bc1 = 1.0 - pow((double)b1, step), bc2 = 1.0 - pow((double)b2, step);
    AdamReports rep; rep.h_status = status ? h_status : nullptr; rep.h_loss = d_loss ? h_loss : nullptr; rep.d_loss = d_loss;
    hipLaunchKernelGGL(k_adam, dim3((unsigned)((n + 255) / 256)), dim3(256), 0, stream, w, g, m, v, n, lr, b1, b2, eps, wd, (float)bc1, (float)sqrt(bc2), den, status, rep);
    qpn_prof_mark(PG_ADAM, stream);
    QPN_HIP(hipGetLastError());
    return QPN_OK;
}

int qpn_launch_adam_clip(float* w, const float* g, float* m, float* v, int64_t n, int step, float lr, float b1, float b2, float eps, float wd, const float* den, int* status,
                         int* h_status, double* h_loss, const double* d_loss, float max_norm, double* part, double* d_norm, double* h_norm, hipStream_t stream) {
    const double bc1 = 1.0 - pow((double)b1, step), bc2 = 1.0 - pow((double)b2, step);
    AdamReports rep; rep.h_status = status ? h_status : nullptr; rep.h_loss = d_loss ? h_loss : nullptr; rep.d_loss = d_loss;
    const int64_t want = ((n >> 2) + 1 + 255) / 256;
    const int nb = want < TR_GN_BLOCKS ? (int)want : TR_GN_BLOCKS;
    hipLaunchKernelGGL(k_grad_sumsq, dim3(nb), dim3(256), 0, stream, g, n, part);
    hipLaunchKernelGGL(k_adam_clip, dim3((unsigned)((n + 255) / 256)), dim3(256), 0, stream, w, g, m, v, n, lr, b1, b2, eps, wd, (float)bc1, (float)sqrt(bc2), den, status, rep,
                       (const double*)part, nb, max_norm, d_norm, h_norm);
    qpn_prof_mark(PG_ADAM, stream);
    QPN_HIP(hipGetLastError());
    return QPN_OK;
}
```

qpnet_amd/csrc/train_common.h:

```cpp
#pragma once
#include "qpn_common.h"

typedef float f32x4 __attribute__((ext_vector_type(4)));

#define TR_MAXL QPN_MAX_LAYERS

__host__ __device__ static inline int tr_lda(int K) { return ((K + 29) / 32) * 32 + 2; }
__host__ __device__ static inline int tr_ldt(int N) { return ((N + 15) / 32) * 32 + 16; }

struct TrLayer {
    int adaptive, dilation;
    int s_in, s_out;
    int tap_off;
    int w1_f4, wr_f4;
    int w1t_f4, wrt_f4;
    int bias1, biasr;
};

struct TrainParams {
    int C, S, Q, A, Ap, L, U;
    int B, T, F, Td, BL, N1, N0, maxd;
    int Kt, Ktp;
    int LC;
    const float* flat;
    const float4* wp;
    const float* ct;
    float* bp;
    const int64_t* x; const float* h; const float* d;
    float* X;
    float* SG; float* TH;
    float* HUP;
    int hoist;
    int nfr, ffirst;
    float* PA;
    float2* WJ;
    int* TAP;
    int* XC;
    float* S0; float* Y0;
    float* logits;
    const int64_t* ce_tgt; int64_t ce_stride; float* ce_dlogits; double* ce_loss;
    int* status;
    float* scratch_rows;
    unsigned* qctl;
    int4* qtab;
    int4* qtab_b;
    int qtotal;
    int qP[TR_MAXL + 1];
    int qT[TR_MAXL];
    int ws_f4, p1_f4, p2_f4;
    int wst_f4, p1t_f4, p2t_f4;
    int bias_s, bias_p1, bias_p2;
    int64_t causal_w, causal_b, up_w, up_b;
    TrLayer layers[TR_MAXL];
};

struct TrainSlabs {
    int g_w1[TR_MAXL], g_b1[TR_MAXL], g_wr[TR_MAXL], g_br[TR_MAXL], g_ws[TR_MAXL], g_bs;
    int g_p1, g_bp1, g_p2, g_bp2;
    int g_early0, g_early1;
    int g_cw, g_cb;
};

struct TrainBwd {
    const float* dlogits; float* gflat;
    float* DXA[2]; float* DXB[2];
    float* DZ;
    float* DS0; float* DY0;
    float* DGS;
    float* DHUP;
    float* DPA;
    float* GW;
    float* EB;
    float* slab;
    const int* gdst; const int* gdst_list;
    const int* gzero; int n_gzero;
    int nch, gstage;
    int64_t n_params;
    const struct TrainSlabs* sl;
    float gscale;
    int append_scale;
    const int* status;
    hipStream_t side; hipEvent_t ev_fork, ev_join, ev_mid;
    hipEvent_t ev_early; int* early_recorded;
};


struct AuxGeom { int auxS[TR_MAXL], auxT[TR_MAXL], bias1[TR_MAXL], s_out[TR_MAXL]; };
struct AuxArgs {
    const float* flat; const float* h; float* PA; float* bp; const float* DPA; const float* EB; const float* GW; float* gflat;
    float gscale; int C, A, L, B, F, U, N1, nfr, ffirst; int64_t up_w, up_b;
    AuxGeom g;
};
static inline AuxArgs tr_aux_args(const TrainParams& p, const TrainBwd* bw, const AuxGeom& ag) {
    AuxArgs a; a.flat = p.flat; a.h = p.h; a.PA = p.PA; a.bp = p.bp; a.DPA = bw ? bw->DPA : nullptr; a.EB = bw ? bw->EB : nullptr; a.GW = bw ? bw->GW : nullptr;
    a.gflat = bw ? bw->gflat : nullptr; a.gscale = bw ? bw->gscale : 1.f;
    a.C = p.C; a.A = p.A; a.L = p.L; a.B = p.B; a.F = p.F; a.U = p.U; a.N1 = p.N1; a.nfr = p.nfr; a.ffirst = p.ffirst; a.up_w = p.up_w; a.up_b = p.up_b; a.g = ag;
    return a;
}
struct TrainKnobs {
    bool serial;
    bool stack_q_fwd, stack_q_bwd;
    int stack_wgs, stack_wgs_bwd;
    bool persist_fwd, persist_bwd;
    bool wgrad_generic;
    int wgrad_chunks, wgrad_chunks_side;
    bool post_fuse;
    bool up_side, reduce_early, wr_side;
    bool post_pair, zero_in_post, post_wide;
    bool xcd_swizzle;
    bool ce_separate;
    bool event_fence;
    bool aux_hoist;
    bool test_stack_gives_up;
};
void qpn_train_knobs_parse(TrainKnobs& k);

#define TR_QHEAD_STRIDE 1056
#define TR_QHDR_WORDS 17920
struct StackQ {
    unsigned* flags;
    unsigned* head;
    unsigned* stats;
    unsigned* abort;
    const int4* tab;
    unsigned epoch;
    unsigned epoch_pub;
    unsigned spin_limit;
    int total, nq;
};

__host__ __device__ __forceinline__ int tr_pa_off(const TrainParams& p, int l, int b, int n0) {
    const int q = p.F * p.U - p.N1 + n0;
    return ((l * p.B + b) * (p.nfr + 1) + (q / p.U - p.ffirst)) * 2 * p.C;
}

__device__ __forceinline__ void tr_queue_entry_fwd(const TrainParams& p, int pos, int4& a, int4& b) {
    const bool valid = pos < p.qtotal;
    const int ps = valid ? pos : 0;
    int l = 0;
    for (int k = 1; k < p.L; ++k) l += ps >= p.qP[k] ? 1 : 0;
    const int r = ps - p.qP[l], T = p.qT[l];
    const int bi = r / T, t = r - bi * T;
    const TrLayer ly = p.layers[l];
    const int n0 = ly.s_out + 16 * t;
    int first = 0, n = 0;
    if (valid && l > 0) {
        const int reach = ly.s_out - ly.s_in, s_prev = p.layers[l - 1].s_out;
        int lo = n0 - reach; if (lo < s_prev) lo = s_prev;
        int hi = n0 + 15; if (hi > p.N1 - 1) hi = p.N1 - 1;
        const int t_lo = (lo - s_prev) >> 4, t_hi = (hi - s_prev) >> 4;
        first = p.qP[l - 1] + bi * p.qT[l - 1] + t_lo; n = t_hi - t_lo + 1;
    }
    a = make_int4(n0, l | (bi << 8) | (l == p.L - 1 ? 1 << 24 : 0) | (valid ? 1 << 25 : 0), first, n);
    b = make_int4((l * p.B + bi) * p.N1, ly.tap_off + bi * p.N1, p.hoist ? tr_pa_off(p, l, bi, n0) : bi * p.N1, 0);
}

__device__ __forceinline__ void tr_queue_entry_bwd(const TrainParams& p, int pos, int4& a, int4& b) {
    const bool valid = pos < p.qtotal;
    const int ps = valid ? pos : 0;
    int k = 0, base = 0;
    for (int j = 0; j + 1 < p.L; ++j) { const int n = p.B * p.qT[p.L - 1 - j]; if (ps >= base + n) { base += n; k = j + 1; } else break; }
    const int l = p.L - 1 - k;
    const int r = ps - base, T = p.qT[l];
    const int bi = r / T, t = r - bi * T;
    const TrLayer ly = p.layers[l];
    const int n0 = ly.s_out + 16 * t;
    int first = 0, n = 0;
    if (valid && l < p.L - 1) {
        const TrLayer up = p.layers[l + 1];
        const int reach = up.s_out - up.s_in;
        int lo = n0 - up.s_out; if (lo < 0) lo = 0;
        int hi = n0 + 15 + reach; if (hi > p.N1 - 1) hi = p.N1 - 1;
        hi -= up.s_out;
        const int t_lo = lo >> 4, t_hi = hi >> 4;
        const int pbase = base - p.B * p.qT[l + 1];
        first = pbase + bi * p.qT[l + 1] + t_lo; n = t_hi - t_lo + 1;
    }
    a = make_int4(n0, l | (bi << 8) | (l == p.L - 1 ? 1 << 24 : 0) | (valid ? 1 << 25 : 0) | (ly.adaptive ? 1 << 26 : 0), first, n);
    b = make_int4((l * p.B + bi) * p.N1, ly.tap_off + bi * p.N1, p.hoist ? tr_pa_off(p, l, bi, n0) : bi * p.N1, bi * p.BL * p.LC + l * p.C);
}

struct TrainGemm {
    const float* wp;
    float* G;
    int K1;
    int N1g, Cg, Sg, Qg, LCg, Ktg;
    long w1[TR_MAXL], w1t[TR_MAXL], wr[TR_MAXL], wrt[TR_MAXL];
    long ws, wst, p1, p1t, p2, p2t;
};

#define TR_LDS_BARRIER() asm volatile("s_waitcnt lgkmcnt(0)\n\ts_barrier" ::: "memory")

int qpn_num_cus();

#define TR_GN_BLOCKS 256

enum { PG_PREP = 0, PG_LAYER_FWD, PG_POST_FWD, PG_CE, PG_POST_BWD, PG_WGRAD, PG_LAYER_BWD, PG_GRAD_TAIL, PG_ADAM, PG_ALLREDUCE,
       PG_WGRAD_WR, PG_WGRAD_SKIP, PG_WGRAD_POST, PG_WGRAD_CAUSAL, PG_COUNT };
void qpn_prof_mark(int group, hipStream_t stream);
bool qpn_prof_serial();
bool qpn_prof_active();

__device__ __forceinline__ int tr_xcd_tile(int orig, int nwg, int swz) {
    if (!swz || nwg <= 8) return orig;
    const int q = nwg / 8, r = nwg % 8, xcd = orig % 8;
    return (xcd < r ? xcd * (q + 1) : r * (q + 1) + (xcd - r) * q) + orig / 8;
}

__device__ __forceinline__ void tr_tile_range(int orig, int G, int tiles, int swz, int& t_first, int& t_count) {
    const int base = tiles / G, rem = tiles - base * G;
    if (!swz || G <= 8) { t_first = orig * base + (orig < rem ? orig : rem); t_count = base + (orig < rem ? 1 : 0); return; }
    const int q = G / 8, r = G % 8, xcd = orig % 8, j = orig / 8;
    const int g = (xcd < r ? xcd * (q + 1) : r * (q + 1) + (xcd - r) * q) + j;
    int before = 0;
    for (int x = 0; x < xcd; ++x) before += rem > x ? (rem - x + 7) / 8 : 0;
    const int mine = rem > xcd ? (rem - xcd + 7) / 8 : 0;
    before += j < mine ? j : mine;
    t_first = g * base + before; t_count = base + (orig < rem ? 1 : 0);
}

__device__ __forceinline__ int tr_aux_slot(float2 wj, int row) { return __float_as_int(wj.y) < row ? 1 : 0; }
__device__ __forceinline__ float tr_aux_a(float2 wj, int lane) { return tr_aux_slot(wj, lane & 15) == (lane >> 4) ? wj.x : 0.f; }
__device__ __forceinline__ float tr_dpp_row_sum(float a) {
    a += __int_as_float(__builtin_amdgcn_update_dpp(0, __float_as_int(a), 0x128, 0xf, 0xf, true));
    a += __int_as_float(__builtin_amdgcn_update_dpp(0, __float_as_int(a), 0x124, 0xf, 0xf, true));
    a += __int_as_float(__builtin_amdgcn_update_dpp(0, __float_as_int(a), 0x4E, 0xf, 0xf, true));
    a += __int_as_float(__builtin_amdgcn_update_dpp(0, __float_as_int(a), 0xB1, 0xf, 0xf, true));
    return a;
}
__device__ __forceinline__ float tr_wave_max(float a) {
    a = fmaxf(a, __int_as_float(__builtin_amdgcn_update_dpp(0, __float_as_int(a), 0x128, 0xf, 0xf, true)));
    a = fmaxf(a, __int_as_float(__builtin_amdgcn_update_dpp(0, __float_as_int(a), 0x124, 0xf, 0xf, true)));
    a = fmaxf(a, __int_as_float(__builtin_amdgcn_update_dpp(0, __float_as_int(a), 0x4E, 0xf, 0xf, true)));
    a = fmaxf(a, __int_as_float(__builtin_amdgcn_update_dpp(0, __float_as_int(a), 0xB1, 0xf, 0xf, true)));
    const int i = __float_as_int(a);
    return fmaxf(fmaxf(__int_as_float(__builtin_amdgcn_readlane(i, 0)), __int_as_float(__builtin_amdgcn_readlane(i, 16))),
// ... 161 lines not shown
```

qpnet_amd/csrc/train_gemm.hip:

```cpp
#include "train_common.h"
#include "qpn_handle.h"
#include <string.h>

typedef float f32x16 __attribute__((ext_vector_type(16)));

#define GM 128
#define GN 128
#ifndef GK
#define GK 16
#endif
#ifndef GKT
#define GKT 16
#endif
#define G_LDA (GK + 1)
#ifndef GEMM_WAVES
#define GEMM_WAVES
#endif
#define G_LDB 128

enum { AL_PLAIN = 0, AL_SUM2 = 1, AL_RELU = 2 };
enum { EP_BIAS = 0, EP_GATE, EP_RES, EP_MASK, EP_DZ, EP_DA, EP_STORE };

struct GArgs {
    int M, N, K, nb;
// ... 301 lines not shown
    auto put = [&](int buf) {
#pragma unroll
        for (int p = 0; p < PT; ++p) {
            const bool ok = (okm >> p) & 1u;
            float4 v = ra[p], w = rb[p];
            if (TWO_A) { v.x += ra2[p].x; v.y += ra2[p].y; v.z += ra2[p].z; v.w += ra2[p].w; }
            if (BMODE == BM_RELU) { w.x = fmaxf(w.x, 0.f); w.y = fmaxf(w.y, 0.f); w.z = fmaxf(w.z, 0.f); w.w = fmaxf(w.w, 0.f); }
            const bool oa = ok && a_ok, ob = ok && b_ok;
            v.x = oa ? v.x : 0.f; v.y = oa ? v.y : 0.f; v.z = oa ? v.z : 0.f; v.w = oa ? v.w : 0.f;
            w.x = ob ? w.x : 0.f; w.y = ob ? w.y : 0.f; w.z = ob ? w.z : 0.f; w.w = ob ? w.w : 0.f;
            *(float4*)(As + buf * (GKT * GM) + (sk + 8 * p) * GM + c4) = v;
            *(float4*)(Bs + buf * (GKT * GN) + (sk + 8 * p) * GN + c4) = w;
        }
    };
    f32x16 acc[4];
#pragma unroll
    for (int j = 0; j < 4; ++j)
#pragma unroll
        for (int r = 0; r < 16; ++r) acc[j][r] = 0.f;
    const int gbias = blockIdx.x == 0 ? g.gbias[y] : -1;
    float csum = 0.f;
    if (kbeg < kend) { taps(kbeg); load(kbeg); if (kbeg + GKT < kend) taps(kbeg + GKT); put(0); }
    __syncthreads();
    int buf = 0;
    for (long k0 = kbeg; k0 < kend; k0 += GKT, buf ^= 1) {
        const bool more = k0 + GKT < kend;
        if (more) { load(k0 + GKT); if (k0 + 2 * GKT < kend) taps(k0 + 2 * GKT); }
        const float* Aq = As + buf * (GKT * GM) + (lane >> 5) * GM + 32 * wave + (lane & 31);
        const float* Bq = Bs + buf * (GKT * GN) + (lane >> 5) * GN + (lane & 31);
        float an = Aq[0], bn0 = Bq[0], bn1 = Bq[32], bn2 = Bq[64], bn3 = Bq[96];
#pragma unroll
        for (int ks = 0; ks < GKT / 2; ++ks) {
            const float a = an, b0 = bn0, b1 = bn1, b2 = bn2, b3 = bn3;
            if (ks + 1 < GKT / 2) {
                an = Aq[2 * (ks + 1) * GM];
                bn0 = Bq[2 * (ks + 1) * GN]; bn1 = Bq[2 * (ks + 1) * GN + 32]; bn2 = Bq[2 * (ks + 1) * GN + 64]; bn3 = Bq[2 * (ks + 1) * GN + 96];
            }
            __builtin_amdgcn_sched_barrier(0);
            acc[0] = __builtin_amdgcn_mfma_f32_32x32x2f32(a, b0, acc[0], 0, 0, 0);
            acc[1] = __builtin_amdgcn_mfma_f32_32x32x2f32(a, b1, acc[1], 0, 0, 0);
            acc[2] = __builtin_amdgcn_mfma_f32_32x32x2f32(a, b2, acc[2], 0, 0, 0);
            acc[3] = __builtin_amdgcn_mfma_f32_32x32x2f32(a, b3, acc[3], 0, 0, 0);
            __builtin_amdgcn_sched_barrier(0);
        }
        if (gbias >= 0 && tid < GM) {
            const float* Ac = As + buf * (GKT * GM) + tid;
            float s = 0.f;
#pragma unroll
            for (int k = 0; k < GKT; ++k) s += Ac[k * GM];
            csum += s;
        }
        if (more) put(buf ^ 1);
        __syncthreads();
    }
    float* out = g.slab + (size_t)sp * g.gstage;
    const int cl = lane & 31, rq = 4 * (lane >> 5);
    const int goff = g.goff[y];
#pragma unroll
    for (int j = 0; j < 4; ++j) {
        const int n = n0 + 32 * j + cl;
        if (n >= g.N) continue;
#pragma unroll
        for (int r = 0; r < 16; ++r) {
            const int m = m0 + 32 * wave + (r & 3) + 8 * (r >> 2) + rq;
            if (m < g.M) out[goff + (size_t)m * g.ldc + n] = acc[j][r];
        }
    }
    if (gbias >= 0 && tid < GM && m0 + tid < g.M) out[gbias + m0 + tid] = csum;
}

static const size_t LDS_NN = (size_t)(2 * GM * G_LDA + 2 * GK * G_LDB) * sizeof(float);
static const size_t LDS_TN = (size_t)(2 * GKT * GM + 2 * GKT * GN) * sizeof(float);

template <int AL, int EPI>
static void launch_nn(const GArgs& g, int ntiles_n, hipStream_t stream) {
    (void)hipFuncSetAttribute((const void*)k_gemm_nn<AL, EPI>, hipFuncAttributeMaxDynamicSharedMemorySize, (int)LDS_NN);
    if (g.M <= 0) return;
    hipLaunchKernelGGL((k_gemm_nn<AL, EPI>), dim3(ntiles_n, (g.M + GM - 1) / GM, g.nb), dim3(256), LDS_NN, stream, g);
}
template <int BMODE>
static void launch_tn(const TArgs& g, int nlayers, hipStream_t stream) {
    (void)hipFuncSetAttribute((const void*)k_gemm_tn<BMODE, false>, hipFuncAttributeMaxDynamicSharedMemorySize, (int)LDS_TN);
    (void)hipFuncSetAttribute((const void*)k_gemm_tn<BMODE, true>, hipFuncAttributeMaxDynamicSharedMemorySize, (int)LDS_TN);
    const dim3 grid((g.N + GN - 1) / GN, (g.M + GM - 1) / GM, nlayers * g.nsplit);
    if (g.a2) hipLaunchKernelGGL((k_gemm_tn<BMODE, true>), grid, dim3(256), LDS_TN, stream, g);
    else hipLaunchKernelGGL((k_gemm_tn<BMODE, false>), grid, dim3(256), LDS_TN, stream, g);
}

static GArgs gbase(const TrainParams& p) {
    GArgs g; memset(&g, 0, sizeof(g));
    g.nb = p.B; g.C = p.C; g.Ap = p.Ap;
    for (int s = 0; s < 3; ++s) { g.a_kend[s] = 1 << 30; g.a[s] = p.X; }
    return g;
}

void qpn_launch_prep(const TrainParams& p, const AuxGeom& ag, hipStream_t stream);

int qpn_launch_fwd_gemm(const TrainParams& p, const TrainGemm& w, hipStream_t stream) {
    const int C = p.C, S = p.S, Q = p.Q, L = p.L, B = p.B, N1 = p.N1, BL = p.BL;
    const size_t nDX = (size_t)B * N1 * C;
    { AuxGeom ag0; memset(&ag0, 0, sizeof(ag0)); qpn_launch_prep(p, ag0, stream); }
    qpn_prof_mark(PG_PREP, stream);
    for (int l = 0; l < L; ++l) {
        const TrLayer& ly = p.layers[l];
        const int rows = N1 - ly.s_out;
        {
            GArgs g = gbase(p);
            g.M = rows; g.N = 2 * C; g.K = w.K1; g.row_base = ly.s_out;
            const float* Xin = p.X + (size_t)l * nDX;
            g.a[0] = Xin; g.a_ld[0] = C; g.a_kend[0] = C; g.a_kvalid[0] = C; g.a_tap[0] = 0; g.a_row0[0] = ly.s_out; g.a_bs[0] = (long)N1 * C;
            g.a[1] = Xin; g.a_ld[1] = C; g.a_kend[1] = 2 * C; g.a_kvalid[1] = C; g.a_tap[1] = 1; g.a_row0[1] = 0; g.a_bs[1] = (long)N1 * C;
            g.a[2] = p.HUP; g.a_ld[2] = p.Ap; g.a_kend[2] = w.K1; g.a_kvalid[2] = p.Ap; g.a_tap[2] = 0; g.a_row0[2] = ly.s_out; g.a_bs[2] = (long)N1 * p.Ap;
            g.tap = ly.adaptive ? p.TAP + ly.tap_off : nullptr; g.tap_bs = N1; g.dil = ly.dilation;
            g.b = w.wp + w.w1[l]; g.ldb = w.N1g;
            g.bias = p.bp + ly.bias1;
            g.o[0] = p.SG + (size_t)l * nDX; g.o[1] = p.TH + (size_t)l * nDX; g.o[2] = w.G + (size_t)l * nDX; g.o_bs = (long)N1 * C; g.o_ld = C; g.o_row0 = ly.s_out;
            launch_nn<AL_PLAIN, EP_GATE>(g, w.N1g / GN, stream);
        }
        if (l + 1 < L) {
            GArgs g = gbase(p);
            g.M = rows; g.N = C; g.K = C; g.row_base = ly.s_out;
            g.a[0] = w.G + (size_t)l * nDX; g.a_ld[0] = C; g.a_kvalid[0] = C; g.a_row0[0] = ly.s_out; g.a_bs[0] = (long)N1 * C;
            g.b = w.wp + w.wr[l]; g.ldb = w.Cg;
            g.bias = p.bp + ly.biasr;
            g.o[0] = p.X + (size_t)(l + 1) * nDX; g.o_bs = (long)N1 * C; g.o_ld = C; g.o_row0 = ly.s_out;
            g.e[0] = p.X + (size_t)l * nDX; g.e_bs = (long)N1 * C; g.e_ld = C; g.e_row0 = ly.s_out;
            launch_nn<AL_PLAIN, EP_RES>(g, w.Cg / GN, stream);
        }
    }
    qpn_prof_mark(PG_LAYER_FWD, stream);
    {
        GArgs g = gbase(p);
        g.M = BL; g.N = S; g.K = L * C; g.row_base = N1 - BL;
        g.a[0] = w.G; g.a_ld[0] = C; g.a_kvalid[0] = L * C; g.a_row0[0] = N1 - BL; g.a_bs[0] = (long)N1 * C;
        g.a_rep_len = C; g.a_rep_stride = (long)nDX;
        g.b = w.wp + w.ws; g.ldb = w.Sg; g.bias = p.bp + p.bias_s;
        g.o[0] = p.S0; g.o_bs = (long)BL * S; g.o_ld = S; g.o_row0 = 0;
        launch_nn<AL_PLAIN, EP_BIAS>(g, w.Sg / GN, stream);
        g = gbase(p);
        g.M = BL; g.N = S; g.K = S; g.a[0] = p.S0; g.a_ld[0] = S; g.a_kvalid[0] = S; g.a_bs[0] = (long)BL * S;
        g.b = w.wp + w.p1; g.ldb = w.Sg; g.bias = p.bp + p.bias_p1;
        g.o[0] = p.Y0; g.o_bs = (long)BL * S; g.o_ld = S;
        launch_nn<AL_RELU, EP_BIAS>(g, w.Sg / GN, stream);
        g.N = Q; g.a[0] = p.Y0; g.b = w.wp + w.p2; g.ldb = w.Qg; g.bias = p.bp + p.bias_p2;
        g.o[0] = p.logits; g.o_bs = (long)BL * Q; g.o_ld = Q;
        launch_nn<AL_RELU, EP_BIAS>(g, w.Qg / GN, stream);
    }
    qpn_prof_mark(PG_POST_FWD, stream);
    QPN_HIP(hipGetLastError());
    return QPN_OK;
}

void qpn_launch_zero_dx(const TrainParams& p, const TrainBwd& bw, hipStream_t stream);
int qpn_launch_grad_tail(const TrainParams& p, const TrainBwd& bw, const AuxGeom* ag, hipStream_t stream, bool early_done, bool up_done);

static void launch_post_wgrad_gemm(const TrainParams& p, const TrainBwd& bw, hipStream_t stream) {
    TArgs a; memset(&a, 0, sizeof(a));
    a.nb = p.B; a.nsplit = bw.nch; a.slab = bw.slab; a.gstage = bw.gstage; a.C = p.C; a.Ap = p.Ap;
    a.M = p.Q; a.N = p.S; a.a = bw.dlogits; a.lda = p.Q; a.rowsA = p.BL; a.b1 = p.Y0; a.ldb = p.S; a.rowsB = p.BL; a.ldc = p.S;
    a.R[0] = p.BL; a.goff[0] = bw.sl->g_p2; a.gbias[0] = bw.sl->g_bp2; a.tap_off[0] = -1;
    launch_tn<BM_RELU>(a, 1, stream);
    a.M = p.S; a.a = bw.DY0; a.lda = p.S; a.b1 = p.S0; a.goff[0] = bw.sl->g_p1; a.gbias[0] = bw.sl->g_bp1;
    launch_tn<BM_RELU>(a, 1, stream);
}

int qpn_launch_bwd_gemm(const TrainParams& p, const TrainBwd& bw, const TrainGemm& w, hipStream_t stream) {
    const int C = p.C, S = p.S, Q = p.Q, L = p.L, B = p.B, N1 = p.N1, BL = p.BL;
    const size_t nDX = (size_t)B * N1 * C;
    qpn_launch_zero_dx(p, bw, stream);
    {
        GArgs g = gbase(p);
        g.M = BL; g.N = S; g.K = Q; g.a[0] = bw.dlogits; g.a_ld[0] = Q; g.a_kvalid[0] = Q; g.a_bs[0] = (long)BL * Q;
        g.b = w.wp + w.p2t; g.ldb = w.Sg;
        g.o[0] = bw.DY0; g.o_bs = (long)BL * S; g.o_ld = S; g.e[0] = p.Y0; g.e_bs = (long)BL * S; g.e_ld = S;
        launch_nn<AL_PLAIN, EP_MASK>(g, w.Sg / GN, stream);
        g.K = S; g.a[0] = bw.DY0; g.a_ld[0] = S; g.a_kvalid[0] = S; g.a_bs[0] = (long)BL * S;
        g.b = w.wp + w.p1t; g.o[0] = bw.DS0; g.e[0] = p.S0;
        launch_nn<AL_PLAIN, EP_MASK>(g, w.Sg / GN, stream);
        g = gbase(p);
        g.M = BL; g.N = L * C; g.K = S; g.a[0] = bw.DS0; g.a_ld[0] = S; g.a_kvalid[0] = S; g.a_bs[0] = (long)BL * S;
        g.b = w.wp + w.wst; g.ldb = w.LCg;
        g.o[0] = bw.DGS; g.o_bs = (long)BL * L * C; g.o_ld = L * C;
        launch_nn<AL_PLAIN, EP_STORE>(g, w.LCg / GN, stream);
    }
    qpn_prof_mark(PG_POST_BWD, stream);
    for (int l = L - 1; l >= 0; --l) {
        const TrLayer& ly = p.layers[l];
        const int rows = N1 - ly.s_out;
        const bool last = l == L - 1;
        float* DZl = bw.DZ + (size_t)l * B * N1 * 2 * C;
        {
            GArgs g = gbase(p);
            g.M = rows; g.N = C; g.K = last ? 0 : C; g.row_base = ly.s_out;
            g.a[0] = bw.DXA[0] + (size_t)(l + 1) * nDX; g.a2 = bw.DXB[0] + (size_t)(l + 1) * nDX;
            g.a_ld[0] = C; g.a_kvalid[0] = C; g.a_row0[0] = ly.s_out; g.a_bs[0] = (long)N1 * C;
            g.b = w.wp + w.wrt[l]; g.ldb = w.Cg;
            g.o[0] = DZl; g.o_bs = (long)N1 * 2 * C; g.o_ld = 2 * C; g.o_row0 = ly.s_out;
            g.e[0] = p.SG + (size_t)l * nDX; g.e[1] = p.TH + (size_t)l * nDX; g.e_bs = (long)N1 * C; g.e_ld = C; g.e_row0 = ly.s_out;
            g.e3 = bw.DGS; g.e3_bs = (long)BL * L * C; g.e3_ld = L * C; g.e3_col0 = l * C; g.e3_rowmin = N1 - BL;
            launch_nn<AL_SUM2, EP_DZ>(g, w.Cg / GN, stream);
        }
        {
            GArgs g = gbase(p);
            g.M = rows; g.N = 2 * C + p.Ap; g.K = 2 * C; g.row_base = ly.s_out;
            g.a[0] = DZl; g.a_ld[0] = 2 * C; g.a_kvalid[0] = 2 * C; g.a_row0[0] = ly.s_out; g.a_bs[0] = (long)N1 * 2 * C;
            g.b = w.wp + w.w1t[l]; g.ldb = w.Ktg;
            g.tap = ly.adaptive ? p.TAP + ly.tap_off : nullptr; g.tap_bs = N1; g.dil = ly.dilation; g.adaptive = ly.adaptive; g.last = last;
            g.o[0] = bw.DXA[0] + (size_t)l * nDX; g.o_bs = (long)N1 * C; g.o_ld = C;
            g.e[0] = bw.DXA[0] + (size_t)(l + 1) * nDX; g.e[1] = bw.DXB[0] + (size_t)(l + 1) * nDX; g.e_bs = (long)N1 * C; g.e_ld = C; g.e_row0 = ly.s_out;
            g.db = bw.DXB[0] + (size_t)l * nDX; g.db_bs = (long)N1 * C;
            g.dh = bw.DHUP; g.dh_bs = (long)N1 * p.Ap;
            launch_nn<AL_PLAIN, EP_DA>(g, w.Ktg / GN, stream);
        }
    }
    qpn_prof_mark(PG_LAYER_BWD, stream);
    TArgs t; memset(&t, 0, sizeof(t));
    t.nb = B; t.nsplit = bw.nch; t.slab = bw.slab; t.gstage = bw.gstage; t.hup = p.HUP; t.tap = p.TAP; t.C = C; t.Ap = p.Ap;
    {
        TArgs a = t;
        a.M = 2 * C; a.N = 2 * C + p.Ap; a.a = bw.DZ; a.a_ls = (long)B * N1 * 2 * C; a.lda = 2 * C; a.rowsA = N1;
        a.b1 = p.X; a.b_ls = (long)nDX; a.ldb = C; a.rowsB = N1; a.ldc = p.Ktp;
        for (int l = 0; l < L; ++l) {
            const TrLayer& ly = p.layers[l];
            a.row0A[l] = a.row0B[l] = ly.s_out; a.R[l] = N1 - ly.s_out; a.goff[l] = bw.sl->g_w1[l]; a.gbias[l] = bw.sl->g_b1[l];
            a.tap_off[l] = ly.adaptive ? ly.tap_off : -1; a.dil[l] = ly.dilation;
        }
        launch_tn<BM_GATHER>(a, L, stream);
    }
    {
        TArgs a = t;
        a.M = C; a.N = C; a.a = bw.DXA[0] + nDX; a.a2 = bw.DXB[0] + nDX; a.a_ls = (long)nDX; a.lda = C; a.rowsA = N1;
        a.b1 = w.G; a.b_ls = (long)nDX; a.ldb = C; a.rowsB = N1; a.ldc = C;
        for (int l = 0; l < L; ++l) {
            a.row0A[l] = a.row0B[l] = p.layers[l].s_out; a.R[l] = l == L - 1 ? 0 : N1 - p.layers[l].s_out;
            a.goff[l] = bw.sl->g_wr[l]; a.gbias[l] = bw.sl->g_br[l]; a.tap_off[l] = -1;
        }
        launch_tn<BM_PLAIN>(a, L, stream);
    }
    {
        TArgs a = t;
        a.M = S; a.N = C; a.a = bw.DS0; a.a_ls = 0; a.lda = S; a.rowsA = BL;
        a.b1 = w.G; a.b_ls = (long)nDX; a.ldb = C; a.rowsB = N1; a.ldc = C;
        for (int l = 0; l < L; ++l) { a.row0A[l] = 0; a.row0B[l] = N1 - BL; a.R[l] = BL; a.goff[l] = bw.sl->g_ws[l]; a.gbias[l] = l == 0 ? bw.sl->g_bs : -1; a.tap_off[l] = -1; }
        launch_tn<BM_PLAIN>(a, L, stream);
    }
    launch_post_wgrad_gemm(p, bw, stream);
    qpn_prof_mark(PG_WGRAD, stream);
    return qpn_launch_grad_tail(p, bw, nullptr, stream, false, false);
}
```

qpnet_amd/csrc/train_host.hip:

```cpp
#include "train_common.h"
#include "qpn_handle.h"
#include <algorithm>
#include <string.h>

int qpn_launch_fwd(const TrainParams& p, const TrainKnobs& k, const AuxGeom& ag, const StackQ* sq, hipStream_t stream, const TrainBwd* fuse_post_bwd);
void qpn_stack_fill(TrainParams& p);
int qpn_launch_ce(const float* logits, const int64_t* tgt, int64_t tgt_stride, int B, int BL, int Q, float* dlogits, double* loss, int* status, bool loss_cleared, hipStream_t stream);
int qpn_launch_bwd(const TrainParams& p, const TrainBwd& bw, const TrainKnobs& k, const AuxGeom& ag, const StackQ* sq, hipStream_t stream, bool post_done);
int qpn_launch_fwd_gemm(const TrainParams& p, const TrainGemm& w, hipStream_t stream);
int qpn_launch_bwd_gemm(const TrainParams& p, const TrainBwd& bw, const TrainGemm& w, hipStream_t stream);
int qpn_launch_adam(float* w, const float* g, float* m, float* v, int64_t n, int step, float lr, float b1, float b2, float eps, float wd, const float* den, int* status,
                    int* h_status, double* h_loss, const double* d_loss, hipStream_t stream);
int qpn_launch_adam_clip(float* w, const float* g, float* m, float* v, int64_t n, int step, float lr, float b1, float b2, float eps, float wd, const float* den, int* status,
                         int* h_status, double* h_loss, const double* d_loss, float max_norm, double* part, double* d_norm, double* h_norm, hipStream_t stream);

#define LOSS_SLOT 72

struct TrainState {
    std::vector<int> h_wmap;
    std::vector<int> h_bstart, h_blist;
    std::vector<int> h_gsrc;
    int* d_wmap; float* d_wp; int* d_bstart; int* d_blist; float* d_bp; int n_bias;
    int* d_gdst; int* d_gdst_list; int* d_gzero; int n_gzero;
    bool hoist;
    TrainParams tp;
    TrainBwd bw;
    TrainSlabs slabs;
    TrainKnobs knobs;
    AuxGeom ag;
    float* d_ws; size_t ws_cap;
    int* d_tap; size_t tap_cap;
    int* d_status; double* d_loss;
    hipStream_t last_stream;
    int* h_status_pinned; hipEvent_t ev_status[2]; bool status_pending[2]; int status_newest;
    double* h_loss_pinned; hipEvent_t ev_loss[2]; bool loss_pending[2]; int loss_newest;
    double* d_gnorm; bool gnorm_last;
    bool gnorm_slot[2];
    double gnorm_collected; bool gnorm_collected_valid;
    bool fwd_valid;
    bool loss_clear;
    bool use_gemm;
    int* d_ctmap; float* d_ct;
    std::vector<int> h_gmap; int* d_gmap; float* d_gwp;
    TrainGemm gm;
    int64_t generation;
    hipStream_t side; hipEvent_t ev_fork, ev_join, ev_mid;
    hipEvent_t ev_early; int early_recorded; int64_t early_first;
    int64_t bwd_generation;
    const float* post_bwd_dlogits;
    bool post_bwd_done;
    bool stack_disabled;
    unsigned* d_sq; size_t sq_pos_cap, sq_per_dir;
    StackQ sqf, sqb;
};

static int env_int(const char* name, int dflt) { const char* e = getenv(name); return (e && *e) ? atoi(e) : dflt; }
void qpn_train_knobs_parse(TrainKnobs& k) {
    k.serial = env_int("QPN_TRAIN_SERIAL", 0) != 0;
    k.stack_q_fwd = env_int("QPN_STACK_QUEUE", 1) != 0;
    k.stack_q_bwd = k.stack_q_fwd && env_int("QPN_STACK_QUEUE_BWD", 1) != 0;
    k.stack_wgs = env_int("QPN_STACK_WGS", 0); if (k.stack_wgs < 0 || k.stack_wgs > 4096) k.stack_wgs = 0;
    k.stack_wgs_bwd = env_int("QPN_STACK_WGS_BWD", 0); if (k.stack_wgs_bwd < 0 || k.stack_wgs_bwd > 4096) k.stack_wgs_bwd = 0;
    k.persist_fwd = env_int("QPN_LAYER_PERSIST", 1) != 0;
    k.persist_bwd = env_int("QPN_LAYER_BWD_PERSIST", 1) != 0;
    k.wgrad_generic = getenv("QPN_WGRAD_GENERIC") != nullptr;
    k.wgrad_chunks = env_int("QPN_WGRAD_CHUNKS", 0); if (k.wgrad_chunks < 1 || k.wgrad_chunks > 512) k.wgrad_chunks = 0;
    k.wgrad_chunks_side = env_int("QPN_WGRAD_CHUNKS_SIDE", 0); if (k.wgrad_chunks_side < 1 || k.wgrad_chunks_side > 512) k.wgrad_chunks_side = 0;
    k.up_side = env_int("QPN_UP_SIDE", 1) != 0;
    k.reduce_early = env_int("QPN_REDUCE_EARLY", 1) != 0;
    k.wr_side = env_int("QPN_WR_SIDE", 1) != 0;
    k.post_fuse = env_int("QPN_POST_FUSE", 1) != 0;
    k.post_pair = env_int("QPN_POST_WGRAD_PAIR", 1) != 0;
    k.zero_in_post = env_int("QPN_ZERO_IN_POST", 1) != 0;
    k.post_wide = env_int("QPN_POST_WIDE", 1) != 0;
    k.xcd_swizzle = getenv("QPN_NO_XCD_SWIZZLE") == nullptr;
    k.ce_separate = getenv("QPN_CE_SEPARATE") != nullptr;
    k.event_fence = env_int("QPN_EVENT_FENCE", 0) == 1;
    k.aux_hoist = env_int("QPN_AUX_HOIST", 1) != 0;
    k.test_stack_gives_up = false;
#ifdef QPN_TESTING
    k.test_stack_gives_up = env_int("QPN_TEST_STACK_GIVES_UP", 0) == 1;
#endif
}

int qpn_num_cus() {
    static int cached[64] = {0};
    int dev = 0;
    if (hipGetDevice(&dev) != hipSuccess || dev < 0 || dev >= 64) return 256;
    if (!cached[dev]) { int n = 0; if (hipDeviceGetAttribute(&n, hipDeviceAttributeMultiprocessorCount, dev) != hipSuccess || n < 1) n = 256; cached[dev] = n; }
    return cached[dev];
}

struct Prof { bool on = false; bool overlapped = false; std::vector<hipEvent_t> ev; std::vector<int> grp; std::vector<hipStream_t> st; size_t used = 0; };
static thread_local Prof g_prof;
bool qpn_prof_active() { return g_prof.on; }
bool qpn_prof_serial() { return g_prof.on && !g_prof.overlapped; }
void qpn_prof_mark(int group, hipStream_t stream) {
    Prof& P = g_prof;
    if (!P.on) return;
    if (P.used == P.ev.size()) { hipEvent_t e; if (hipEventCreate(&e) != hipSuccess) return; P.ev.push_back(e); P.grp.push_back(0); P.st.push_back(nullptr); }
    P.grp[P.used] = group; P.st[P.used] = stream;
    (void)hipEventRecord(P.ev[P.used++], stream);
}
extern "C" int qpn_train_profile_begin(qpn_handle* h, void* stream) {
    (void)h; g_prof.on = true; g_prof.overlapped = false; g_prof.used = 0;
    qpn_prof_mark(-1, (hipStream_t)stream);
    return QPN_OK;
}
extern "C" int qpn_train_profile_begin_overlapped(qpn_handle* h, void* stream) {
    (void)h; g_prof.on = true; g_prof.overlapped = true; g_prof.used = 0;
    qpn_prof_mark(-1, (hipStream_t)stream);
    return QPN_OK;
}
extern "C" int qpn_train_profile_mark(qpn_handle* h, int group, void* stream) {
    (void)h; qpn_prof_mark(group, (hipStream_t)stream); return QPN_OK;
}
extern "C" int qpn_train_profile_end(qpn_handle* h, float* h_ms, int n, void* stream) {
    Prof& P = g_prof;
    QPN_HIP(hipStreamSynchronize((hipStream_t)stream));
    if (h && h->train && h->train->side) QPN_HIP(hipStreamSynchronize(h->train->side));
    for (int i = 0; i < n; ++i) h_ms[i] = 0.f;
    for (size_t i = 1; i < P.used; ++i) {
        if (P.grp[i] < 0 || P.grp[i] >= n) continue;
        size_t j = i;
        while (j > 0 && P.st[j - 1] != P.st[i]) --j;
        if (j == 0) continue;
        float ms = 0.f;
        QPN_HIP(hipEventElapsedTime(&ms, P.ev[j - 1], P.ev[i]));
        h_ms[P.grp[i]] += ms;
    }
    P.on = false;
    return QPN_OK;
}

__global__ void k_gather_f(const float* __restrict__ flat, const int* __restrict__ map, float* __restrict__ out, int64_t n) {
    int64_t i = (int64_t)blockIdx.x * blockDim.x + threadIdx.x;
    if (i < n) { int m = map[i]; out[i] = m >= 0 ? flat[m] : 0.0f; }
}
__global__ void k_refresh(const float* __restrict__ flat, const int* __restrict__ wmap, float* __restrict__ wout, int64_t nw,
                          const int* __restrict__ ctmap, float* __restrict__ ct, int64_t nct,
                          const int* __restrict__ bstart, const int* __restrict__ blist, float* __restrict__ bp, int nb,
                          int* __restrict__ status, double* __restrict__ loss) {
    int64_t i = (int64_t)blockIdx.x * blockDim.x + threadIdx.x;
    if (i < nw) { const int m = wmap[i]; wout[i] = m >= 0 ? flat[m] : 0.0f; return; }
    i -= nw;
    if (i < nct) { ct[i] = flat[ctmap[i]]; return; }
    i -= nct;
    if (i < nb) { float a = 0.f; for (int j = bstart[i]; j < bstart[i + 1]; ++j) a += flat[blist[j]]; bp[i] = a; return; }
    i -= nb;
    (void)status;
    if (i >= 16 && i < 16 + 64) loss[i - 16] = 0.0;
}
template <class F>
static long kmajor_pack(std::vector<int>& map, int K, int Kp, int N, int Np, F src) {
    const long off = (long)map.size();
    map.resize(map.size() + (size_t)Kp * Np, -1);
    int* m = map.data() + off;
    for (int k = 0; k < K; ++k)
        for (int n = 0; n < N; ++n) m[(size_t)k * Np + n] = (int)src(k, n);
    return off;
}
static inline int pad_to(int v, int q) { return (v + q - 1) / q * q; }

template <class F>
static int frag_pack(std::vector<int>& map, int K, int N, F src) {
    const int NT = N / 16, off4 = (int)(map.size() / 4);
    map.resize(map.size() + (size_t)K * N);
    int* m = map.data() + (size_t)off4 * 4;
    for (int ks4 = 0; ks4 < K / 16; ++ks4)
        for (int nt = 0; nt < NT; ++nt)
            for (int lane = 0; lane < 64; ++lane)
                for (int e = 0; e < 4; ++e) {
                    int k = 16 * ks4 + 4 * e + (lane >> 4), n = 16 * nt + (lane & 15);
                    m[(((size_t)ks4 * NT + nt) * 64 + lane) * 4 + e] = (int)src(k, n);
                }
    return off4;
}

static int train_init(qpn_handle* h) {
    if (h->train) return QPN_OK;
    const Geom& g = h->g;
    const int C = g.C, S = g.S, Q = g.Q, A = g.A, L = g.L;
    if (L > TR_MAXL) { qpn_set_error("training kernels support up to %d residual layers", TR_MAXL); return QPN_EINVAL; }
    if (C % 16 || S % 16 || Q % 16) { qpn_set_error("training kernels need n_resch, n_skipch, n_quantize multiples of 16"); return QPN_EINVAL; }
    TrainState* t = new TrainState();
    memset(&t->tp, 0, sizeof(t->tp)); memset(&t->bw, 0, sizeof(t->bw));
    t->d_wmap = nullptr; t->d_wp = nullptr; t->d_bstart = t->d_blist = nullptr; t->d_bp = nullptr;
    t->d_gdst = t->d_gdst_list = t->d_gzero = nullptr; t->n_gzero = 0;
    t->d_ws = nullptr; t->ws_cap = 0; t->d_tap = nullptr; t->tap_cap = 0; t->d_status = nullptr; t->d_loss = nullptr; t->fwd_valid = false; t->loss_clear = false;
    t->generation = 0; t->side = nullptr; t->ev_fork = t->ev_join = t->ev_mid = nullptr; t->ev_early = nullptr; t->early_recorded = 0; t->early_first = -1;
    t->d_sq = nullptr; t->sq_pos_cap = 0; t->sq_per_dir = 0; t->bwd_generation = -1; t->stack_disabled = false; memset(&t->sqf, 0, sizeof(t->sqf)); memset(&t->sqb, 0, sizeof(t->sqb));
    qpn_train_knobs_parse(t->knobs);
    memset(&t->slabs, 0, sizeof(t->slabs));
    t->use_gemm = (C > 128 || getenv("QPN_TRAIN_GEMM")) && !getenv("QPN_TRAIN_TILES");
    t->d_gmap = nullptr; t->d_gwp = nullptr; t->d_ctmap = nullptr; t->d_ct = nullptr; memset(&t->gm, 0, sizeof(t->gm));
    if (t->use_gemm && (C % 32 || S % 32 || Q % 32)) { qpn_set_error("the GEMM training path needs n_resch, n_skipch, n_quantize multiples of 32"); delete t; return QPN_EINVAL; }
    TrainParams& p = t->tp;
    const int Ap = (A + 3) / 4 * 4;
    t->hoist = !t->use_gemm && C == 64 && g.U >= 16 && A <= 64 && t->knobs.aux_hoist && t->knobs.persist_fwd && t->knobs.persist_bwd;
    p.hoist = t->hoist ? 1 : 0;
    p.C = C; p.S = S; p.Q = Q; p.A = A; p.Ap = Ap; p.L = L; p.U = g.U;
    p.Kt = t->hoist ? 2 * C : 2 * C + Ap; p.Ktp = (p.Kt + 15) / 16 * 16; p.LC = L * C;
    p.causal_w = g.causal_w; p.causal_b = g.causal_b; p.up_w = g.up_w; p.up_b = g.up_b;
    std::vector<int>& map = t->h_wmap;
    std::vector<std::vector<int>> biases;
    auto add_bias = [&](int n, auto f) { int off = (int)biases.size(); for (int i = 0; i < n; ++i) biases.push_back(f(i)); return off; };
    const int Ktp = p.Ktp;
    int n_adapt = 0;
    for (int l = 0; l < L; ++l) {
        const LayerGeom y = g.layers[l];
        TrLayer& ly = p.layers[l];
        ly.adaptive = y.adaptive; ly.dilation = y.dilation;
        ly.tap_off = y.adaptive ? n_adapt++ : -1;
        auto w1src = [&](int k, int n) -> int64_t {
            const int half = n / C, r = n % C;
            if (k < C) return y.adaptive ? (half ? y.wT : y.wS) + (int64_t)r * C + k : (half ? y.wT : y.wS) + ((int64_t)r * C + k) * 2 + 1;
            if (k < 2 * C) { const int kk = k - C; return y.adaptive ? (half ? y.wTP : y.wSP) + (int64_t)r * C + kk : (half ? y.wT : y.wS) + ((int64_t)r * C + kk) * 2; }
            if (k < 2 * C + A) return (half ? y.auxT : y.auxS) + (int64_t)r * A + (k - 2 * C);
            return -1;
        };
        ly.w1_f4 = frag_pack(map, Ktp, 2 * C, w1src);
        ly.w1t_f4 = frag_pack(map, 2 * C, Ktp, [&](int k, int n) { return w1src(n, k); });
        ly.wr_f4 = frag_pack(map, C, C, [&](int k, int n) { return y.res + (int64_t)n * C + k; });
        ly.wrt_f4 = frag_pack(map, C, C, [&](int k, int n) { return y.res + (int64_t)k * C + n; });
        ly.bias1 = add_bias(2 * C, [&](int n) {
            const int half = n / C, r = n % C;
            std::vector<int> v{(int)((half ? y.bT : y.bS) + r), (int)((half ? y.auxTb : y.auxSb) + r)};
            if (y.adaptive) v.push_back((int)((half ? y.bTP : y.bSP) + r));
            return v; });
        ly.biasr = add_bias(C, [&](int n) { return std::vector<int>{(int)(y.resb + n)}; });
    }
    p.ws_f4 = frag_pack(map, L * C, S, [&](int k, int n) { return g.layers[k / C].skip + (int64_t)n * C + (k % C); });
    p.wst_f4 = frag_pack(map, S, L * C, [&](int k, int n) { return g.layers[n / C].skip + (int64_t)k * C + (n % C); });
    p.p1_f4 = frag_pack(map, S, S, [&](int k, int n) { return g.post1_w + (int64_t)n * S + k; });
    p.p1t_f4 = frag_pack(map, S, S, [&](int k, int n) { return g.post1_w + (int64_t)k * S + n; });
    p.p2_f4 = frag_pack(map, S, Q, [&](int k, int n) { return g.post2_w + (int64_t)n * S + k; });
    p.p2t_f4 = frag_pack(map, Q, S, [&](int k, int n) { return g.post2_w + (int64_t)k * S + n; });
    p.bias_s = add_bias(S, [&](int n) { std::vector<int> v; for (int l = 0; l < L; ++l) v.push_back((int)(g.layers[l].skipb + n)); return v; });
    p.bias_p1 = add_bias(S, [&](int n) { return std::vector<int>{(int)(g.post1_b + n)}; });
    p.bias_p2 = add_bias(Q, [&](int n) { return std::vector<int>{(int)(g.post2_b + n)}; });
    if (t->use_gemm) {
        TrainGemm& gm = t->gm;
        std::vector<int>& gmap = t->h_gmap;
        const int Apad = pad_to(Ap, 32);
        gm.K1 = 2 * C + Apad; gm.N1g = pad_to(C, 64) * 2; gm.Cg = pad_to(C, 128); gm.Sg = pad_to(S, 128); gm.Qg = pad_to(Q, 128);
        gm.LCg = pad_to(L * C, 128); gm.Ktg = pad_to(2 * C + Ap, 128);
        for (int l = 0; l < L; ++l) {
            const LayerGeom y = g.layers[l];
            auto w1src = [&](int k, int n) -> int64_t {
                const int half = n / C, r = n % C;
                if (k < C) return y.adaptive ? (half ? y.wT : y.wS) + (int64_t)r * C + k : (half ? y.wT : y.wS) + ((int64_t)r * C + k) * 2 + 1;
                if (k < 2 * C) { const int kk = k - C; return y.adaptive ? (half ? y.wTP : y.wSP) + (int64_t)r * C + kk : (half ? y.wT : y.wS) + ((int64_t)r * C + kk) * 2; }
                if (k < 2 * C + A) return (half ? y.auxT : y.auxS) + (int64_t)r * A + (k - 2 * C);
                return -1;
            };
            gm.w1[l] = kmajor_pack(gmap, 2 * C + A, gm.K1, gm.N1g, gm.N1g, [&](int k, int q) -> int64_t {
                const int tile = q / 128, w = q % 128, half = w / 64, c = 64 * tile + w % 64;
                return c < C ? w1src(k, half * C + c) : -1; });
            gm.w1t[l] = kmajor_pack(gmap, 2 * C, 2 * C, 2 * C + A, gm.Ktg, [&](int k, int n) { return w1src(n, k); });
            gm.wr[l] = kmajor_pack(gmap, C, C, C, gm.Cg, [&](int k, int n) { return y.res + (int64_t)n * C + k; });
            gm.wrt[l] = kmajor_pack(gmap, C, C, C, gm.Cg, [&](int k, int n) { return y.res + (int64_t)k * C + n; });
        }
        gm.ws = kmajor_pack(gmap, L * C, L * C, S, gm.Sg, [&](int k, int n) { return g.layers[k / C].skip + (int64_t)n * C + (k % C); });
        gm.wst = kmajor_pack(gmap, S, S, L * C, gm.LCg, [&](int k, int n) { return g.layers[n / C].skip + (int64_t)k * C + (n % C); });
        gm.p1 = kmajor_pack(gmap, S, S, S, gm.Sg, [&](int k, int n) { return g.post1_w + (int64_t)n * S + k; });
        gm.p1t = kmajor_pack(gmap, S, S, S, gm.Sg, [&](int k, int n) { return g.post1_w + (int64_t)k * S + n; });
        gm.p2 = kmajor_pack(gmap, S, S, Q, gm.Qg, [&](int k, int n) { return g.post2_w + (int64_t)n * S + k; });
        gm.p2t = kmajor_pack(gmap, Q, Q, S, gm.Sg, [&](int k, int n) { return g.post2_w + (int64_t)k * S + n; });
    }
    memset(&t->ag, 0, sizeof(t->ag));
    for (int l = 0; l < L; ++l) { t->ag.auxS[l] = (int)g.layers[l].auxS; t->ag.auxT[l] = (int)g.layers[l].auxT; t->ag.bias1[l] = p.layers[l].bias1; }
    t->n_bias = (int)biases.size();
    t->h_bstart.assign(1, 0);
    for (auto& v : biases) { for (int x : v) t->h_blist.push_back(x); t->h_bstart.push_back((int)t->h_blist.size()); }

    TrainBwd& bw = t->bw;
    TrainSlabs& sl = t->slabs;
    bw.sl = &t->slabs;
    int go = 0;
    auto gtake = [&](int n) { int r = go; go += (n + 63) & ~63; return r; };
    std::vector<int>& gs = t->h_gsrc;
    gs.assign(g.n_params, -1);
    for (int l = 0; l < L; ++l) {
        sl.g_w1[l] = gtake(2 * C * Ktp);
        sl.g_b1[l] = gtake(2 * C);
        sl.g_wr[l] = gtake(C * C);
        sl.g_br[l] = gtake(C);
    }
    sl.g_early0 = go;
    for (int l = 0; l < L; ++l) sl.g_ws[l] = gtake(S * C);
    for (int l = 0; l < L; ++l) {
        const LayerGeom y = g.layers[l];
        for (int n = 0; n < 2 * C; ++n) {
            const int half = n / C, r = n % C;
            if (t->hoist) for (int a = 0; a < A; ++a) gs[(half ? y.auxT : y.auxS) + (int64_t)r * A + a] = -2;
            for (int k = 0; k < (t->hoist ? 2 * C : 2 * C + A); ++k) {
                int64_t dst;
                if (k < C) dst = y.adaptive ? (half ? y.wT : y.wS) + (int64_t)r * C + k : (half ? y.wT : y.wS) + ((int64_t)r * C + k) * 2 + 1;
                else if (k < 2 * C) { const int kk = k - C; dst = y.adaptive ? (half ? y.wTP : y.wSP) + (int64_t)r * C + kk : (half ? y.wT : y.wS) + ((int64_t)r * C + kk) * 2; }
                else dst = (half ? y.auxT : y.auxS) + (int64_t)r * A + (k - 2 * C);
                gs[dst] = sl.g_w1[l] + n * Ktp + k;
            }
            gs[(half ? y.bT : y.bS) + r] = sl.g_b1[l] + n;
            gs[(half ? y.auxTb : y.auxSb) + r] = sl.g_b1[l] + n;
            if (y.adaptive) gs[(half ? y.bTP : y.bSP) + r] = sl.g_b1[l] + n;
        }
        for (int o = 0; o < C; ++o) { for (int c = 0; c < C; ++c) gs[y.res + (int64_t)o * C + c] = sl.g_wr[l] + o * C + c; gs[y.resb + o] = sl.g_br[l] + o; }
        for (int s = 0; s < S; ++s) for (int c = 0; c < C; ++c) gs[y.skip + (int64_t)s * C + c] = sl.g_ws[l] + s * C + c;
    }
    sl.g_bs = gtake(S);
    for (int l = 0; l < L; ++l) for (int s = 0; s < S; ++s) gs[g.layers[l].skipb + s] = sl.g_bs + s;
    sl.g_p1 = gtake(S * S); sl.g_bp1 = gtake(S); sl.g_p2 = gtake(Q * S); sl.g_bp2 = gtake(Q);
    sl.g_early1 = go;
    t->early_first = (g.post1_b == g.post1_w + (int64_t)S * S && g.post2_w == g.post1_b + S && g.post2_b == g.post2_w + (int64_t)Q * S && g.post2_b + Q == g.n_params) ? g.post1_w : -1;
    for (int o = 0; o < S; ++o) { for (int s = 0; s < S; ++s) gs[g.post1_w + (int64_t)o * S + s] = sl.g_p1 + o * S + s; gs[g.post1_b + o] = sl.g_bp1 + o; }
    for (int q = 0; q < Q; ++q) { for (int s = 0; s < S; ++s) gs[g.post2_w + (int64_t)q * S + s] = sl.g_p2 + q * S + s; gs[g.post2_b + q] = sl.g_bp2 + q; }
    sl.g_cw = sl.g_cb = -1;
    if (C == 64 && Q % 128 == 0 && !t->use_gemm) {
        sl.g_cw = gtake(2 * C * Q); sl.g_cb = gtake(C);
        for (int c = 0; c < C; ++c) {
            for (int q = 0; q < Q; ++q) for (int tp = 0; tp < 2; ++tp) gs[g.causal_w + ((int64_t)c * Q + q) * 2 + tp] = sl.g_cw + tp * C * Q + c * Q + q;
            gs[g.causal_b + c] = sl.g_cb + c;
        }
    }
    bw.gstage = go; bw.nch = t->use_gemm ? 4 : 64; bw.n_params = g.n_params;
    if (t->knobs.wgrad_chunks > 0) bw.nch = t->knobs.wgrad_chunks;
    if (t->hoist) for (int j = 0; j < g.U; ++j) gs[g.up_w + j] = -2;

    const size_t nmap = t->use_gemm ? 4 : map.size();
    QPN_HIP(hipMalloc(&t->d_wmap, nmap * sizeof(int)));
    QPN_HIP(hipMalloc(&t->d_wp, nmap * sizeof(float)));
    QPN_HIP(hipMalloc(&t->d_bstart, t->h_bstart.size() * sizeof(int)));
    QPN_HIP(hipMalloc(&t->d_blist, t->h_blist.size() * sizeof(int)));
    QPN_HIP(hipMalloc(&t->d_bp, (size_t)t->n_bias * sizeof(float)));
    QPN_HIP(hipMalloc(&t->d_status, 64));
    QPN_HIP(hipMemset(t->d_status, 0, 64));
    t->last_stream = nullptr;
    t->h_status_pinned = nullptr; t->ev_status[0] = t->ev_status[1] = nullptr; t->status_pending[0] = t->status_pending[1] = false; t->status_newest = 0;
    QPN_HIP(hipHostMalloc((void**)&t->h_status_pinned, 64, hipHostMallocDefault));
    t->h_loss_pinned = nullptr; t->ev_loss[0] = t->ev_loss[1] = nullptr; t->loss_pending[0] = t->loss_pending[1] = false; t->loss_newest = 0;
    QPN_HIP(hipHostMalloc((void**)&t->h_loss_pinned, 2 * LOSS_SLOT * sizeof(double), hipHostMallocDefault));
    t->d_gnorm = nullptr; t->gnorm_last = false; t->gnorm_slot[0] = t->gnorm_slot[1] = false; t->gnorm_collected = 0.0; t->gnorm_collected_valid = false;
    QPN_HIP(hipMalloc(&t->d_gnorm, TR_GN_BLOCKS * sizeof(double)));
    QPN_HIP(hipMemset(t->d_gnorm, 0, TR_GN_BLOCKS * sizeof(double)));
    QPN_HIP(hipEventCreateWithFlags(&t->ev_loss[0], hipEventDisableTiming));
    QPN_HIP(hipEventCreateWithFlags(&t->ev_loss[1], hipEventDisableTiming));
    QPN_HIP(hipEventCreateWithFlags(&t->ev_status[0], hipEventDisableTiming));
    QPN_HIP(hipEventCreateWithFlags(&t->ev_status[1], hipEventDisableTiming));
    QPN_HIP(hipMalloc(&t->d_loss, LOSS_SLOT * sizeof(double)));
    QPN_HIP(hipMemset(t->d_loss, 0, LOSS_SLOT * sizeof(double)));
    if (!t->use_gemm) QPN_HIP(hipMemcpy(t->d_wmap, map.data(), nmap * sizeof(int), hipMemcpyHostToDevice));
    QPN_HIP(hipMemcpy(t->d_bstart, t->h_bstart.data(), t->h_bstart.size() * sizeof(int), hipMemcpyHostToDevice));
    QPN_HIP(hipMemcpy(t->d_blist, t->h_blist.data(), t->h_blist.size() * sizeof(int), hipMemcpyHostToDevice));
    {
        std::vector<int> start((size_t)go + 1, 0), list, gz;
        for (int64_t i = 0; i < g.n_params; ++i) { if (gs[i] >= 0) ++start[(size_t)gs[i] + 1]; else if (gs[i] == -1) gz.push_back((int)i); }
        for (int k = 0; k < go; ++k) start[(size_t)k + 1] += start[k];
        list.resize((size_t)start[go] + 1);
        std::vector<int> fill(start.begin(), start.end() - 1);
        for (int64_t i = 0; i < g.n_params; ++i) if (gs[i] >= 0) list[(size_t)fill[gs[i]]++] = (int)i;
        QPN_HIP(hipMalloc(&t->d_gdst, start.size() * sizeof(int)));
        QPN_HIP(hipMemcpy(t->d_gdst, start.data(), start.size() * sizeof(int), hipMemcpyHostToDevice));
        QPN_HIP(hipMalloc(&t->d_gdst_list, list.size() * sizeof(int)));
        QPN_HIP(hipMemcpy(t->d_gdst_list, list.data(), list.size() * sizeof(int), hipMemcpyHostToDevice));
        t->n_gzero = (int)gz.size();
        QPN_HIP(hipMalloc(&t->d_gzero, (gz.size() + 1) * sizeof(int)));
        if (!gz.empty()) QPN_HIP(hipMemcpy(t->d_gzero, gz.data(), gz.size() * sizeof(int), hipMemcpyHostToDevice));
    }
    if (t->use_gemm) {
        QPN_HIP(hipMalloc(&t->d_gmap, t->h_gmap.size() * sizeof(int)));
        QPN_HIP(hipMalloc(&t->d_gwp, t->h_gmap.size() * sizeof(float)));
        QPN_HIP(hipMemcpy(t->d_gmap, t->h_gmap.data(), t->h_gmap.size() * sizeof(int), hipMemcpyHostToDevice));
        t->gm.wp = t->d_gwp;
        std::vector<int>().swap(t->h_wmap);
    }
    {
        std::vector<int> ctm((size_t)2 * Q * C);
        for (int tp = 0; tp < 2; ++tp) for (int q = 0; q < Q; ++q) for (int c = 0; c < C; ++c)
            ctm[((size_t)tp * Q + q) * C + c] = (int)(g.causal_w + ((int64_t)c * Q + q) * 2 + tp);
        QPN_HIP(hipMalloc(&t->d_ctmap, ctm.size() * sizeof(int)));
        QPN_HIP(hipMalloc(&t->d_ct, ctm.size() * sizeof(float)));
        QPN_HIP(hipMemcpy(t->d_ctmap, ctm.data(), ctm.size() * sizeof(int), hipMemcpyHostToDevice));
    }
    QPN_HIP(hipStreamCreateWithFlags(&t->side, hipStreamNonBlocking));
    const unsigned evf = hipEventDisableTiming | (t->knobs.event_fence ? 0u : (unsigned)hipEventDisableSystemFence);
    QPN_HIP(hipEventCreateWithFlags(&t->ev_fork, evf));
    QPN_HIP(hipEventCreateWithFlags(&t->ev_join, evf));
    QPN_HIP(hipEventCreateWithFlags(&t->ev_mid, evf));
    QPN_HIP(hipEventCreateWithFlags(&t->ev_early, evf));
    h->train = t;
    return QPN_OK;
}

void qpn_train_destroy(TrainState* t) {
    if (!t) return;
    void* bufs[] = {t->d_wmap, t->d_wp, t->d_bstart, t->d_blist, t->d_bp, t->d_gdst, t->d_gdst_list, t->d_gzero, t->d_ws, t->d_tap, t->d_status, t->d_loss, t->d_gmap, t->d_gwp, t->d_ctmap, t->d_ct, t->d_sq, t->d_gnorm};
    for (void* b : bufs) if (b) (void)hipFree(b);
    if (t->h_status_pinned) (void)hipHostFree(t->h_status_pinned);
    if (t->h_loss_pinned) (void)hipHostFree(t->h_loss_pinned);
    for (int i = 0; i < 2; ++i) if (t->ev_loss[i]) (void)hipEventDestroy(t->ev_loss[i]);
    for (int i = 0; i < 2; ++i) if (t->ev_status[i]) (void)hipEventDestroy(t->ev_status[i]);
    if (t->side) (void)hipStreamDestroy(t->side);
    if (t->ev_fork) (void)hipEventDestroy(t->ev_fork);
    if (t->ev_join) (void)hipEventDestroy(t->ev_join);
    if (t->ev_mid) (void)hipEventDestroy(t->ev_mid);
    if (t->ev_early) (void)hipEventDestroy(t->ev_early);
    delete t;
}

static int need_dev(qpn_handle* h) {
    if (!h) { qpn_set_error("null handle"); return QPN_EINVAL; }
    if (h->device < 0) { qpn_set_error("no HIP device: libqpnet_hip has no CPU fallback"); return QPN_ENODEV; }
    return QPN_OK;
}

static int train_forward_impl(qpn_handle* h, const float* d_flat, int B, int64_t T, int64_t F, int64_t Td, int BL, int maxd,
                              const int64_t* d_x, const float* d_h, const float* d_dfac, float* d_logits,
                              const int64_t* d_targets, int64_t tgt_stride, float* d_dlogits, int want_logits, void* stream_, bool fuse_bwd = false) {
    int rc = need_dev(h); if (rc) return rc;
    rc = train_init(h); if (rc) return rc;
    TrainState* t = h->train;
    hipStream_t stream = (hipStream_t)stream_;
    const Geom& g = h->g;
    if (!d_flat || !d_x || !d_h || !d_dfac || !d_logits || B < 1 || BL < 1 || maxd < 1) { qpn_set_error("bad train_forward arguments"); return QPN_EINVAL; }
    if (d_targets && tgt_stride < BL) { qpn_set_error("bad train_forward_loss arguments: target rows shorter than batch_length"); return QPN_EINVAL; }
    const int64_t N0 = (int64_t)g.recA * maxd + g.recF + 1 + BL;
    if (N0 > T || N0 - 1 > Td || N0 - 1 > (g.U > 0 ? F * g.U : F)) {
        qpn_set_error("chunk too short: need receptive field (%lld) + batch_length (%d) = %lld samples, have x:%lld d:%lld h_up:%lld",
                      (long long)(N0 - BL), BL, (long long)N0, (long long)T, (long long)Td, (long long)(g.U > 0 ? F * g.U : F));
        return QPN_EINVAL;
    }
    if (T >= ((int64_t)1 << 31) || Td >= ((int64_t)1 << 31) || F * (g.U > 0 ? g.U : 1) >= ((int64_t)1 << 31) || (int64_t)B * N0 >= ((int64_t)1 << 31)) {
        qpn_set_error("chunk too long: the training kernels index rows with 32 bits"); return QPN_EINVAL;
    }
    TrainParams& p = t->tp;
    p.B = B; p.T = (int)T; p.F = (int)F; p.Td = (int)Td; p.BL = BL; p.N0 = (int)N0; p.N1 = (int)N0 - 1; p.maxd = maxd;
    const int C = g.C, S = g.S, L = g.L, N1 = p.N1;
    int s = 0, nA = 0;
    for (int l = 0; l < L; ++l) {
        TrLayer& ly = p.layers[l];
        ly.s_in = s; s += ly.adaptive ? ly.dilation * maxd : ly.dilation; ly.s_out = s;
        ly.tap_off = (nA++) * B * N1;
        t->ag.s_out[l] = ly.s_out;
    }
    if (t->hoist) {
        if (N1 >= (1 << 24)) { qpn_set_error("chunk too long for the register-resident layer kernels (%d rows; QPN_AUX_HOIST=0 QPN_LAYER_PERSIST=0 QPN_LAYER_BWD_PERSIST=0 selects the tile-per-workgroup kernels)", N1); return QPN_EINVAL; }
        p.ffirst = (int)(((int64_t)F * g.U - N1) / g.U); p.nfr = (int)F - p.ffirst;
    } else { p.ffirst = 0; p.nfr = 0; }
    const size_t nPA = t->hoist ? (size_t)L * B * (p.nfr + 1) * 2 * C : 0, nWJ = t->hoist ? (size_t)2 * (N1 + 16) : 0, nGW = t->hoist ? (size_t)L * B * N1 : 0;
    const size_t nX = (size_t)(L + 1) * B * N1 * C, nG = (size_t)L * B * N1 * C, nH = t->hoist ? 64 : (size_t)B * N1 * p.Ap, nS = (size_t)B * BL * S;
    TrainBwd& bw = t->bw;
    const size_t nDX = (size_t)B * N1 * C, nDZ = (size_t)B * N1 * 2 * C, nDGS = (size_t)B * BL * L * C, nSlab = (size_t)bw.nch * bw.gstage;
    const size_t nXC = (size_t)B * (N1 + 1);
    const size_t nScr = (size_t)B * 1024 * 2 * 128;
    size_t need = nScr + nX + 2 * nG + nH + 2 * (nS + 96 * (size_t)S + 64) + 2 * (size_t)(L + 1) * nDX + (size_t)L * nDZ + 2 * nS + nDGS + nH + nSlab + nXC + (t->use_gemm ? nG : 0) + 2 * nPA + nWJ + nGW + (size_t)L * TR_EB_SLOTS * 2 * C + 8192;
    if (need > t->ws_cap) {
        if (t->d_ws) (void)hipFree(t->d_ws);
        t->d_ws = nullptr; t->ws_cap = 0;
        hipError_t e = hipMalloc(&t->d_ws, need * sizeof(float));
        if (e != hipSuccess) { qpn_set_error("hipMalloc(%zu MiB) for the training workspace failed", need * 4 >> 20); return QPN_ENOMEM; }
        t->ws_cap = need;
    }
    const size_t ntap = (size_t)std::max(nA, 1) * B * N1;
    if (ntap > t->tap_cap) {
        if (t->d_tap) (void)hipFree(t->d_tap);
        t->d_tap = nullptr; t->tap_cap = 0;
        QPN_HIP(hipMalloc(&t->d_tap, ntap * sizeof(int)));
        t->tap_cap = ntap;
    }
    float* w = t->d_ws;
    auto carve = [&](size_t n) { float* r = w; w += (n + 63) & ~(size_t)63; return r; };
    p.X = carve(nX); p.SG = carve(nG); p.TH = carve(nG); p.HUP = carve(nH); p.S0 = carve(nS + 96 * (size_t)S); p.Y0 = carve(nS + 96 * (size_t)S);
    bw.DXA[0] = carve((size_t)(L + 1) * nDX); bw.DXB[0] = carve((size_t)(L + 1) * nDX); bw.DXA[1] = bw.DXB[1] = nullptr;
    bw.DZ = carve((size_t)L * nDZ); bw.DS0 = carve(nS); bw.DY0 = carve(nS); bw.DGS = carve(nDGS); bw.DHUP = carve(nH); bw.slab = carve(nSlab);
    p.XC = (int*)carve(nXC);
    p.scratch_rows = carve(nScr);
    if (t->use_gemm) t->gm.G = carve(nG);
    p.PA = nullptr; p.WJ = nullptr; bw.DPA = nullptr; bw.GW = nullptr;
    bw.EB = nullptr;
    if (t->hoist) { p.PA = carve(nPA); bw.DPA = carve(nPA + (size_t)L * TR_EB_SLOTS * 2 * C); bw.EB = bw.DPA + nPA; p.WJ = (float2*)carve(nWJ); bw.GW = carve(nGW); }
    p.TAP = t->d_tap; p.status = t->d_status;
    t->last_stream = stream;
    {
        qpn_stack_fill(p);
        if ((size_t)p.qtotal > t->sq_pos_cap) {
            if (t->d_sq) (void)hipFree(t->d_sq);
            t->d_sq = nullptr; t->sq_pos_cap = 0;
            const size_t cap = (size_t)p.qtotal + (size_t)p.qtotal / 2 + 64;
            const size_t per_dir = (cap / 32 + 2) * 1056;
            const size_t nsq = TR_QHDR_WORDS + 2 * per_dir + 2 * (cap + 1) * 8;
            QPN_HIP(hipMalloc(&t->d_sq, nsq * sizeof(unsigned)));
            QPN_HIP(hipMemsetAsync(t->d_sq, 0, nsq * sizeof(unsigned), stream));
            t->sq_pos_cap = cap; t->sq_per_dir = per_dir;
        }
        hipStreamCaptureStatus cap_st = hipStreamCaptureStatusNone;
        (void)hipStreamIsCapturing(stream, &cap_st);
        const bool no_queue = t->stack_disabled || cap_st != hipStreamCaptureStatusNone;
        p.qctl = no_queue ? nullptr : t->d_sq;
        p.qtab = no_queue ? nullptr : (int4*)(t->d_sq + TR_QHDR_WORDS + 2 * t->sq_per_dir);
        p.qtab_b = no_queue ? nullptr : p.qtab + 2 * (t->sq_pos_cap + 1);
        const unsigned epoch = (unsigned)((t->generation + 1) % 0xFFFFFFFFll) + 1u;
        StackQ& f = t->sqf; StackQ& bq = t->sqb;
        f.flags = t->d_sq + TR_QHDR_WORDS; f.head = t->d_sq + 1024; f.abort = t->d_sq + 1; f.stats = t->d_sq + 4; f.epoch = epoch; f.total = p.qtotal; f.tab = p.qtab;
        bq.flags = f.flags + t->sq_per_dir; bq.head = f.head + 8 * TR_QHEAD_STRIDE; bq.abort = f.abort; bq.stats = t->d_sq + 8; bq.epoch = epoch; bq.total = p.qtotal; bq.tab = p.qtab_b;
    }
    p.flat = d_flat; p.wp = (const float4*)t->d_wp; p.bp = t->d_bp; p.x = d_x; p.h = d_h; p.d = d_dfac; p.logits = d_logits;
    {
        const int* wmap = t->use_gemm ? t->d_gmap : t->d_wmap;
        float* wout = t->use_gemm ? t->d_gwp : t->d_wp;
        const int64_t nw = (int64_t)(t->use_gemm ? t->h_gmap.size() : t->h_wmap.size()), nct = (int64_t)2 * g.Q * g.C;
        const int64_t tot = nw + nct + t->n_bias + 16 + 64;
        hipLaunchKernelGGL(k_refresh, dim3((unsigned)((tot + 255) / 256)), dim3(256), 0, stream, d_flat, wmap, wout, nw, t->d_ctmap, t->d_ct, nct,
                           t->d_bstart, t->d_blist, t->d_bp, t->n_bias, t->d_status, t->d_loss);
        p.ct = t->d_ct;
    }
    qpn_prof_mark(PG_PREP, stream);
    t->fwd_valid = false; t->loss_clear = true;
    ++t->generation;
    const bool fuse_ce = d_targets && !t->use_gemm && g.Q <= g.S && g.Q % 256 == 0 && !t->knobs.ce_separate;
    p.ce_tgt = fuse_ce ? d_targets : nullptr; p.ce_stride = tgt_stride; p.ce_dlogits = d_dlogits; p.ce_loss = t->d_loss;
    if (fuse_ce && !want_logits) p.logits = nullptr;
    const bool fuse_post = fuse_bwd && fuse_ce && d_dlogits && t->knobs.post_fuse && t->knobs.post_wide && t->knobs.zero_in_post && g.S == 256 && g.Q == 256 && g.C == 64 && (p.LC == 256 || p.LC == 512);
    t->post_bwd_done = false;
    rc = t->use_gemm ? qpn_launch_fwd_gemm(p, t->gm, stream) : qpn_launch_fwd(p, t->knobs, t->ag, &t->sqf, stream, fuse_post ? &t->bw : nullptr);
    if (!rc) { t->post_bwd_done = fuse_post; t->post_bwd_dlogits = d_dlogits; }
    p.ce_tgt = nullptr; p.logits = d_logits;
    if (rc) return rc;
    t->fwd_valid = true;
    if (fuse_ce) { t->loss_clear = false; qpn_prof_mark(PG_CE, stream); }
    else if (d_targets) {
        rc = qpn_launch_ce(d_logits, d_targets, tgt_stride, B, BL, g.Q, d_dlogits, t->d_loss, t->d_status, t->loss_clear, stream); if (rc) return rc;
        t->loss_clear = false;
    }
    return QPN_OK;
}

extern "C" int qpn_train_forward(qpn_handle* h, const float* d_flat, int B, int64_t T, int64_t F, int64_t Td, int BL, int maxd,
                                 const int64_t* d_x, const float* d_h, const float* d_dfac, float* d_logits, void* stream_) {
    return train_forward_impl(h, d_flat, B, T, F, Td, BL, maxd, d_x, d_h, d_dfac, d_logits, nullptr, 0, nullptr, 1, stream_);
}

extern "C" int qpn_train_forward_loss(qpn_handle* h, const float* d_flat, int B, int64_t T, int64_t F, int64_t Td, int BL, int maxd,
                                      const int64_t* d_x, const float* d_h, const float* d_dfac, const int64_t* d_targets, int64_t tgt_stride,
                                      float* d_logits, int want_logits, float* d_dlogits, void* stream_) {
    if (!d_targets) { qpn_set_error("bad train_forward_loss arguments: no targets"); return QPN_EINVAL; }
    return train_forward_impl(h, d_flat, B, T, F, Td, BL, maxd, d_x, d_h, d_dfac, d_logits, d_targets, tgt_stride, d_dlogits, want_logits & 1, stream_, (want_logits & QPN_FWD_BACKWARD_FOLLOWS) != 0);
}

extern "C" int qpn_train_loss(qpn_handle* h, double* h_loss, void* stream_) {
    int rc = need_dev(h); if (rc) return rc;
    if (!h->train || !h_loss) { qpn_set_error("qpn_train_loss needs a preceding qpn_train_forward_loss / qpn_ce_loss"); return QPN_ESTATE; }
    hipStream_t stream = (hipStream_t)stream_;
    double parts[64];
    QPN_HIP(hipMemcpyAsync(parts, h->train->d_loss, sizeof(parts), hipMemcpyDeviceToHost, stream));
    QPN_HIP(hipStreamSynchronize(stream));
    double sum = 0.0;
    for (int i = 0; i < 64; ++i) sum += parts[i];
    *h_loss = sum;
    return QPN_OK;
}

extern "C" int qpn_train_loss_enqueue(qpn_handle* h, void* stream_) {
    int rc = need_dev(h); if (rc) return rc;
    if (!h->train) { qpn_set_error("qpn_train_loss_enqueue needs a preceding qpn_train_forward_loss / qpn_ce_loss"); return QPN_ESTATE; }
    TrainState* t = h->train;
    const int slot = t->loss_newest ^ 1;
    if (t->loss_pending[slot]) QPN_HIP(hipEventSynchronize(t->ev_loss[slot]));
    QPN_HIP(hipMemcpyAsync(t->h_loss_pinned + LOSS_SLOT * slot, t->d_loss, (t->gnorm_last ? 65 : 64) * sizeof(double), hipMemcpyDeviceToHost, (hipStream_t)stream_));
    t->gnorm_slot[slot] = t->gnorm_last;
    QPN_HIP(hipEventRecord(t->ev_loss[slot], (hipStream_t)stream_));
    t->loss_pending[slot] = true; t->loss_newest = slot;
    return QPN_OK;
}
extern "C" int qpn_train_loss_collect(qpn_handle* h, int newest, double* h_loss, int* h_valid) {
    int rc = need_dev(h); if (rc) return rc;
    if (!h_loss || !h_valid) { qpn_set_error("bad loss_collect arguments"); return QPN_EINVAL; }
    *h_valid = 0; *h_loss = 0.0;
    if (!h->train) return QPN_OK;
    TrainState* t = h->train;
    const int slot = newest ? t->loss_newest : t->loss_newest ^ 1;
    t->gnorm_collected_valid = false;
    if (!t->loss_pending[slot]) return QPN_OK;
    QPN_HIP(hipEventSynchronize(t->ev_loss[slot]));
    t->loss_pending[slot] = false;
    double sum = 0.0;
    for (int i = 0; i < 64; ++i) sum += t->h_loss_pinned[LOSS_SLOT * slot + i];
    *h_loss = sum; *h_valid = 1;
    if (t->gnorm_slot[slot]) { t->gnorm_collected = t->h_loss_pinned[LOSS_SLOT * slot + 64]; t->gnorm_collected_valid = true; }
    return QPN_OK;
}

static int status_to_rc(int st);
extern "C" int qpn_train_status(qpn_handle* h, void* stream_) {
    int rc = need_dev(h); if (rc) return rc;
    if (!h->train) { qpn_set_error("no training call yet"); return QPN_ESTATE; }
    QPN_HIP(hipStreamSynchronize((hipStream_t)stream_));
    int st = 0;
    QPN_HIP(hipMemcpy(&st, h->train->d_status, sizeof(int), hipMemcpyDeviceToHost));
    if (st) QPN_HIP(hipMemsetAsync(h->train->d_status, 0, sizeof(int), (hipStream_t)stream_));
    h->train->last_stream = (hipStream_t)stream_;
    if (st & 4) h->train->stack_disabled = true;
    h->train->status_pending[0] = h->train->status_pending[1] = false;
    return status_to_rc(st);
}

static int status_to_rc(int st) {
    if (st & 1) { qpn_set_error("pitch-dependent tap outside the layer input (dilated factor > maxd or < 0; reference assert qpnet.py:294)"); return QPN_ERANGE; }
    if (st & 4) { qpn_set_error("the one-launch residual stack gave up waiting for a peer workgroup: the flagged step's results are invalid (its Adam update, and that of the steps enqueued behind it until this report, were skipped on the device: parameters and moments are those of the last clean step); the handle runs a launch per layer from here on (QPN_STACK_QUEUE=0 selects that from the start)"); return QPN_ENODEV; }
    if (st & 2) { qpn_set_error("target class outside [0, n_quantize) (reference assert qpnet_train.py:525)"); return QPN_ERANGE; }
    if (st & (1 << 16)) { qpn_set_error("non-finite gradient norm (an inf or NaN in the gradient): the step's Adam update, and that of the steps enqueued behind it until this report, were skipped on the device: parameters and moments are those of the last clean step"); return QPN_ERANGE; }
    if (st & 8) { qpn_set_error("a peer rank flagged its chunk of this data-parallel step (a tap or target out of range, or an abandoned stack launch there): every rank skipped the update, the replicas are unchanged"); return QPN_ERANGE; }
    return QPN_OK;
}

static int status_collect_slot(TrainState* t, int slot) {
    if (!t->status_pending[slot]) return QPN_OK;
    QPN_HIP(hipEventSynchronize(t->ev_status[slot]));
    t->status_pending[slot] = false;
    const int st = t->h_status_pinned[slot];
    if (st & 4) t->stack_disabled = true;
    if (st) {
        QPN_HIP(hipMemsetAsync(t->d_status, 0, sizeof(int), t->last_stream));
        const int other = slot ^ 1;
        if (t->status_pending[other]) {
            QPN_HIP(hipEventSynchronize(t->ev_status[other]));
            t->h_status_pinned[other] &= ~st;
            if (!t->h_status_pinned[other]) t->status_pending[other] = false;
        }
    }
    return status_to_rc(st);
}
extern "C" int qpn_train_status_enqueue(qpn_handle* h, void* stream_) {
    int rc = need_dev(h); if (rc) return rc;
    if (!h->train) { qpn_set_error("no training call yet"); return QPN_ESTATE; }
    TrainState* t = h->train;
    const int slot = t->status_newest ^ 1;
    t->last_stream = (hipStream_t)stream_;
    rc = status_collect_slot(t, slot); if (rc) return rc;
    QPN_HIP(hipMemcpyAsync(t->h_status_pinned + slot, t->d_status, sizeof(int), hipMemcpyDeviceToHost, (hipStream_t)stream_));
    QPN_HIP(hipEventRecord(t->ev_status[slot], (hipStream_t)stream_));
    t->status_pending[slot] = true; t->status_newest = slot;
    return QPN_OK;
}
extern "C" int qpn_train_status_collect(qpn_handle* h) {
    int rc = need_dev(h); if (rc) return rc;
    if (!h->train) return QPN_OK;
    TrainState* t = h->train;
    rc = status_collect_slot(t, t->status_newest ^ 1); if (rc) return rc;
    return status_collect_slot(t, t->status_newest);
}
extern "C" int qpn_train_status_poll(qpn_handle* h, int* pending) {
    int rc = need_dev(h); if (rc) return rc;
    if (pending) *pending = 0;
    if (!h->train) return QPN_OK;
    TrainState* t = h->train;
    for (int k = 0; k < 2; ++k) {
        const int slot = k == 0 ? t->status_newest ^ 1 : t->status_newest;
        if (!t->status_pending[slot]) continue;
        if (hipEventQuery(t->ev_status[slot]) != hipSuccess) { (void)hipGetLastError(); if (pending) ++*pending; continue; }
        rc = status_collect_slot(t, slot); if (rc) return rc;
    }
    return QPN_OK;
}
extern "C" int qpn_train_status_collect_lagged(qpn_handle* h) {
    int rc = need_dev(h); if (rc) return rc;
    if (!h->train) return QPN_OK;
    return status_collect_slot(h->train, h->train->status_newest ^ 1);
}

extern "C" int qpn_ce_loss(qpn_handle* h, const float* d_logits, const int64_t* d_targets, int64_t tgt_stride, int B, int BL,
                           float* d_dlogits, double* h_loss, void* stream_) {
    int rc = need_dev(h); if (rc) return rc;
    rc = train_init(h); if (rc) return rc;
    hipStream_t stream = (hipStream_t)stream_;
    if (!d_logits || !d_targets || B < 1 || BL < 1 || tgt_stride < BL) { qpn_set_error("bad ce_loss arguments"); return QPN_EINVAL; }
    rc = qpn_launch_ce(d_logits, d_targets, tgt_stride, B, BL, h->g.Q, d_dlogits, h->train->d_loss, h->train->d_status, h->train->loss_clear, stream); if (rc) return rc;
    h->train->loss_clear = false;
    if (h_loss) {
        double parts[64];
        QPN_HIP(hipMemcpyAsync(parts, h->train->d_loss, sizeof(parts), hipMemcpyDeviceToHost, stream));
        QPN_HIP(hipStreamSynchronize(stream));
        double sum = 0.0;
        for (int i = 0; i < 64; ++i) sum += parts[i];
        *h_loss = sum;
    }
    return QPN_OK;
}

extern "C" int qpn_train_stack_stats(qpn_handle* h, unsigned* h_out, int n, void* stream_) {
    int rc = need_dev(h); if (rc) return rc;
    if (!h->train || !h->train->d_sq || !h_out || n < 1) { qpn_set_error("no stack-queue launch yet"); return QPN_ESTATE; }
    QPN_HIP(hipStreamSynchronize((hipStream_t)stream_));
    QPN_HIP(hipMemcpy(h_out, h->train->d_sq, sizeof(unsigned) * (size_t)(n < 1024 ? n : 1024), hipMemcpyDeviceToHost));
    return QPN_OK;
}

extern "C" int qpn_train_applied_updates(qpn_handle* h, int64_t* applied, void* stream_) {
    int rc = need_dev(h); if (rc) return rc;
    if (!applied) { qpn_set_error("bad applied_updates arguments"); return QPN_EINVAL; }
    *applied = 0;
    if (!h->train) return QPN_OK;
    QPN_HIP(hipStreamSynchronize((hipStream_t)stream_));
    unsigned long long v = 0;
    QPN_HIP(hipMemcpy(&v, h->train->d_status + 2, sizeof(v), hipMemcpyDeviceToHost));
    *applied = (int64_t)v;
    return QPN_OK;
}

#ifdef QPN_TESTING
extern "C" int qpn_test_postnet_activations(qpn_handle* h, float* d_s0, float* d_y0, int64_t n, void* stream_) {
    int rc = need_dev(h); if (rc) return rc;
    if (!h->train || !h->train->fwd_valid || !d_s0 || !d_y0) { qpn_set_error("no forward to read"); return QPN_ESTATE; }
    const TrainParams& p = h->train->tp;
    if (n != (int64_t)p.B * p.BL * p.S) { qpn_set_error("postnet_activations: n != B * BL * S"); return QPN_EINVAL; }
    QPN_HIP(hipMemcpyAsync(d_s0, p.S0, sizeof(float) * (size_t)n, hipMemcpyDeviceToDevice, (hipStream_t)stream_));
    QPN_HIP(hipMemcpyAsync(d_y0, p.Y0, sizeof(float) * (size_t)n, hipMemcpyDeviceToDevice, (hipStream_t)stream_));
    return QPN_OK;
}
#endif

extern "C" int64_t qpn_train_generation(qpn_handle* h) { return (h && h->train) ? h->train->generation : 0; }

extern "C" int qpn_train_backward(qpn_handle* h, const float* d_dlogits, float* d_flatgrad, void* stream_) {
    return qpn_train_backward_ex(h, d_dlogits, d_flatgrad, 1.0f, 0, stream_);
}

extern "C" int qpn_train_backward_ex(qpn_handle* h, const float* d_dlogits, float* d_flatgrad, float grad_scale, int append_scale, void* stream_) {
    int rc = need_dev(h); if (rc) return rc;
    if (!h->train || !h->train->fwd_valid) { qpn_set_error("qpn_train_backward needs a preceding qpn_train_forward"); return QPN_ESTATE; }
    if (!d_dlogits || !d_flatgrad) { qpn_set_error("bad train_backward arguments"); return QPN_EINVAL; }
    TrainState* t = h->train;
    TrainBwd& bw = t->bw;
    bw.dlogits = d_dlogits; bw.gflat = d_flatgrad; bw.gdst = t->d_gdst; bw.gdst_list = t->d_gdst_list; bw.gzero = t->d_gzero; bw.n_gzero = t->n_gzero;
    bw.gscale = grad_scale; bw.append_scale = append_scale; bw.status = h->train->d_status;
    bw.side = t->side; bw.ev_fork = t->ev_fork; bw.ev_join = t->ev_join; bw.ev_mid = t->ev_mid;
    t->early_recorded = 0; bw.ev_early = t->ev_early; bw.early_recorded = (append_scale && t->early_first >= 0) ? &t->early_recorded : nullptr;
    const bool first_bwd = t->bwd_generation != t->generation;
    t->bwd_generation = t->generation;
    const bool post_done = t->post_bwd_done && first_bwd && d_dlogits == t->post_bwd_dlogits;
    t->post_bwd_done = false;
    return t->use_gemm ? qpn_launch_bwd_gemm(t->tp, bw, t->gm, (hipStream_t)stream_)
                       : qpn_launch_bwd(t->tp, bw, t->knobs, t->ag, first_bwd ? &t->sqb : nullptr, (hipStream_t)stream_, post_done);
}

extern "C" int qpn_train_early_bucket(qpn_handle* h, int64_t* first, int64_t* count, void* stream_) {
    int rc = need_dev(h); if (rc) return rc;
    if (!first || !count) { qpn_set_error("bad early_bucket arguments"); return QPN_EINVAL; }
    *first = 0; *count = 0;
    TrainState* t = h->train;
    if (!t || !t->early_recorded) return QPN_OK;
    *first = t->early_first; *count = t->bw.n_params - t->early_first + 4;
    QPN_HIP(hipStreamWaitEvent((hipStream_t)stream_, t->ev_early, 0));
    return QPN_OK;
}

extern "C" int64_t qpn_train_early_first(qpn_handle* h) { return (h && h->train && h->device >= 0) ? h->train->early_first : -1; }

extern "C" int qpn_adam_step(qpn_handle* h, float* d_flat, const float* d_grad, float* d_m, float* d_v, int64_t n,
                             int step, float lr, float beta1, float beta2, float eps, float weight_decay, void* stream_) {
    return qpn_adam_step_ex(h, d_flat, d_grad, d_m, d_v, n, step, lr, beta1, beta2, eps, weight_decay, nullptr, stream_);
}

extern "C" int qpn_adam_step_ex(qpn_handle* h, float* d_flat, const float* d_grad, float* d_m, float* d_v, int64_t n,
                                int step, float lr, float beta1, float beta2, float eps, float weight_decay,
                                const float* d_grad_denominator, void* stream_) {
    return qpn_adam_step_clip(h, d_flat, d_grad, d_m, d_v, n, step, lr, beta1, beta2, eps, weight_decay, d_grad_denominator, 0.0f, stream_);
}

extern "C" int qpn_adam_step_clip(qpn_handle* h, float* d_flat, const float* d_grad, float* d_m, float* d_v, int64_t n,
                                  int step, float lr, float beta1, float beta2, float eps, float weight_decay,
                                  const float* d_grad_denominator, float max_grad_norm, void* stream_) {
    int rc = need_dev(h); if (rc) return rc;
    if (!d_flat || !d_grad || !d_m || !d_v || n < 1 || step < 1 || max_grad_norm != max_grad_norm) { qpn_set_error("bad adam_step arguments"); return QPN_EINVAL; }
    const bool clip = max_grad_norm > 0.f;
    if (clip) { rc = train_init(h); if (rc) return rc; }
    if (h->train) { h->train->last_stream = (hipStream_t)stream_; h->train->gnorm_last = clip; }
    if (clip) return qpn_launch_adam_clip(d_flat, d_grad, d_m, d_v, n, step, lr, beta1, beta2, eps, weight_decay, d_grad_denominator, h->train->d_status, nullptr, nullptr, nullptr,
                                          max_grad_norm, h->train->d_gnorm, h->train->d_loss + 64, nullptr, (hipStream_t)stream_);
    return qpn_launch_adam(d_flat, d_grad, d_m, d_v, n, step, lr, beta1, beta2, eps, weight_decay, d_grad_denominator, h->train ? h->train->d_status : nullptr, nullptr, nullptr, nullptr, (hipStream_t)stream_);
}

extern "C" int qpn_train_grad_norm(qpn_handle* h, double* h_norm, int* h_valid, void* stream_) {
    int rc = need_dev(h); if (rc) return rc;
    if (!h_norm || !h_valid) { qpn_set_error("bad grad_norm arguments"); return QPN_EINVAL; }
    *h_norm = 0.0; *h_valid = 0;
    if (!h->train || !h->train->gnorm_last) return QPN_OK;
    QPN_HIP(hipStreamSynchronize((hipStream_t)stream_));
    QPN_HIP(hipMemcpy(h_norm, h->train->d_loss + 64, sizeof(double), hipMemcpyDeviceToHost));
    *h_valid = 1;
    return QPN_OK;
}
extern "C" int qpn_train_grad_norm_lagged(qpn_handle* h, double* h_norm, int* h_valid) {
    int rc = need_dev(h); if (rc) return rc;
    if (!h_norm || !h_valid) { qpn_set_error("bad grad_norm arguments"); return QPN_EINVAL; }
    *h_norm = 0.0; *h_valid = 0;
    if (!h->train || !h->train->gnorm_collected_valid) return QPN_OK;
    *h_norm = h->train->gnorm_collected; *h_valid = 1;
    return QPN_OK;
}

extern "C" int qpn_train_step(qpn_handle* h, float* d_flat, int B, int64_t T, int64_t F, int64_t Td, int BL, int maxd,
                              const int64_t* d_x, const float* d_h, const float* d_dfac, const int64_t* d_targets, int64_t tgt_stride,
                              float* d_logits, float* d_dlogits, float* d_grad, float* d_m, float* d_v, int64_t n,
                              int step, float lr, float beta1, float beta2, float eps, float weight_decay,
                              int loss_mode, double* h_loss, int* h_valid, void* stream) {
    return qpn_train_step_clip(h, d_flat, B, T, F, Td, BL, maxd, d_x, d_h, d_dfac, d_targets, tgt_stride, d_logits, d_dlogits, d_grad, d_m, d_v, n,
                               step, lr, beta1, beta2, eps, weight_decay, loss_mode, h_loss, h_valid, 0.0f, nullptr, stream);
}

extern "C" int qpn_train_step_clip(qpn_handle* h, float* d_flat, int B, int64_t T, int64_t F, int64_t Td, int BL, int maxd,
                                   const int64_t* d_x, const float* d_h, const float* d_dfac, const int64_t* d_targets, int64_t tgt_stride,
                                   float* d_logits, float* d_dlogits, float* d_grad, float* d_m, float* d_v, int64_t n,
                                   int step, float lr, float beta1, float beta2, float eps, float weight_decay,
                                   int loss_mode, double* h_loss, int* h_valid, float max_grad_norm, double* h_grad_norm, void* stream) {
    if (h_valid) *h_valid = 0;
    if (h_loss) *h_loss = 0.0;
    if (h_grad_norm) *h_grad_norm = 0.0;
    if (loss_mode < 0 || loss_mode > 2 || (loss_mode && (!h_loss || !h_valid)) || max_grad_norm != max_grad_norm) { qpn_set_error("bad train_step arguments"); return QPN_EINVAL; }
    const bool clip = max_grad_norm > 0.f;
    int rc = need_dev(h); if (rc) return rc;
    rc = qpn_train_status_collect_lagged(h); if (rc) return rc;
    if (!d_targets || !d_dlogits) { qpn_set_error("qpn_train_forward_loss needs targets and a dlogits buffer"); return QPN_EINVAL; }
    rc = train_forward_impl(h, d_flat, B, T, F, Td, BL, maxd, d_x, d_h, d_dfac, d_logits, d_targets, tgt_stride, d_dlogits, 0, stream, true); if (rc) return rc;
    rc = qpn_train_backward(h, d_dlogits, d_grad, stream); if (rc) return rc;
    if (loss_mode == 2) {
        rc = qpn_adam_step_clip(h, d_flat, d_grad, d_m, d_v, n, step, lr, beta1, beta2, eps, weight_decay, nullptr, max_grad_norm, stream); if (rc) return rc;
        rc = qpn_train_loss(h, h_loss, stream); if (rc) return rc;
        *h_valid = 1;
        if (clip && h_grad_norm) { int nv = 0; rc = qpn_train_grad_norm(h, h_grad_norm, &nv, stream); if (rc) return rc; }
        return qpn_train_status(h, stream);
    }
    if (!d_flat || !d_grad || !d_m || !d_v || n < 1 || step < 1) { qpn_set_error("bad adam_step arguments"); return QPN_EINVAL; }
    TrainState* t = h->train;
    const int sslot = t->status_newest ^ 1;
    rc = status_collect_slot(t, sslot); if (rc) return rc;
    const int lslot = t->loss_newest ^ 1;
    if (loss_mode == 1 && t->loss_pending[lslot]) QPN_HIP(hipEventSynchronize(t->ev_loss[lslot]));
    double* const hl = loss_mode == 1 ? t->h_loss_pinned + LOSS_SLOT * lslot : nullptr;
    t->gnorm_last = clip;
    if (clip) rc = qpn_launch_adam_clip(d_flat, d_grad, d_m, d_v, n, step, lr, beta1, beta2, eps, weight_decay, nullptr, t->d_status, t->h_status_pinned + sslot,
                                        hl, loss_mode == 1 ? t->d_loss : nullptr, max_grad_norm, t->d_gnorm, t->d_loss + 64, hl ? hl + 64 : nullptr, (hipStream_t)stream);
    else rc = qpn_launch_adam(d_flat, d_grad, d_m, d_v, n, step, lr, beta1, beta2, eps, weight_decay, nullptr, t->d_status, t->h_status_pinned + sslot,
                              hl, loss_mode == 1 ? t->d_loss : nullptr, (hipStream_t)stream);
    if (rc) return rc;
    QPN_HIP(hipEventRecord(t->ev_status[sslot], (hipStream_t)stream));
    t->status_pending[sslot] = true; t->status_newest = sslot;
    if (loss_mode == 1) {
        QPN_HIP(hipEventRecord(t->ev_loss[lslot], (hipStream_t)stream));
        t->loss_pending[lslot] = true; t->loss_newest = lslot; t->gnorm_slot[lslot] = clip;
        rc = qpn_train_loss_collect(h, 0, h_loss, h_valid); if (rc) return rc;
        if (h_grad_norm && t->gnorm_collected_valid) *h_grad_norm = t->gnorm_collected;
    }
    return QPN_OK;
}
```

Before: 1477 steps/s.

## Replace causal-table weight-grad path with sorted-index row sums and fused fold

Replaces the causal embedding-table gradient, previously an atomic shared-memory scatter or a one-hot wgrad mode, with a deterministic three-stage scheme. An index kernel buckets sample positions by quantized value into a permutation. A rowsum kernel sums dXA+dXB over each bucket in fixed-size groups. A fold stage reduces the partials into the weight and bias gradients and is fused into the existing grad-reduction kernel as extra leading blocks. This removes atomics and the one-hot GEMM work, at the cost of extra workspace buffers, an extra event and two extra kernel launches.

Result: slower. 1443 steps/s (-2.3%).

```diff
diff --git a/qpnet_amd/csrc/train_bwd.hip b/qpnet_amd/csrc/train_bwd.hip
--- a/qpnet_amd/csrc/train_bwd.hip
+++ b/qpnet_amd/csrc/train_bwd.hip
@@ -464,7 +464,6 @@
     int bmode; const float* B1; const float* B2; size_t B_lstride; int ldb, N, Nvalid;
     int rowsB;
     const float* hup; const int* tap; int C, Ap;
-    const int* xc;
     int nb, nlayers;
     float* slab; int gstage;
     int row0A[TR_MAXL], row0B[TR_MAXL], R[TR_MAXL];
@@ -708,7 +707,7 @@
     const int rbeg = (int)(per * ch), rend = (int)(per * ch + per < total ? per * ch + per : total);
     const float* A = w.A + (size_t)y * w.A_lstride;
     const float* A2 = TWO_A ? w.A2 + (size_t)y * w.A_lstride : nullptr;
-    const float* B1 = BMODE == 4 ? nullptr : w.B1 + (size_t)y * w.B_lstride;
+    const float* B1 = w.B1 + (size_t)y * w.B_lstride;
     const float* B2 = w.B2 ? w.B2 + (size_t)y * w.B_lstride : nullptr;
     const int* tap = BMODE == 3 ? w.tap + w.tap_off[y] : nullptr;
     const int row0A = w.row0A[y], row0B = w.row0B[y], ncol0 = zg * Np;
@@ -725,8 +724,7 @@
         if (n < w.C) { bbase = B1 + n; bstride = w.C; }
         else if (n < 2 * w.C) { bbase = B1 + (n - w.C); bstride = w.C; use_tap = true; }
         else { bbase = w.hup + (b_pad ? 0 : n - 2 * w.C); bstride = w.Ap; }
-    } else if (BMODE == 4) { bbase = nullptr; bstride = 0; }
-    else { bbase = B1 + n; bstride = w.ldb; }
+    } else { bbase = B1 + n; bstride = w.ldb; }
     const ptrdiff_t b2off = (BMODE == 2) ? (B2 - B1) : 0;
 
     f32x4 acc[MPW][NT];
@@ -737,7 +735,6 @@
     float4 cs4 = make_float4(0.f, 0.f, 0.f, 0.f);
     float4 ra[NA], ra2[NA], rb[NB], rb2[NB];
     int tpv[NB];
-    int rbi[NB];
     unsigned okA = 0, okB = 0;
 
     const unsigned a_voff = (unsigned)a_row0 * (unsigned)w.lda + (unsigned)a_col, a_kstep = (unsigned)ARS * (unsigned)w.lda;
@@ -766,7 +763,7 @@
         }
     };
     auto fetch = [&](int rs) {
-        const float* pa[NA]; const float* pb[NB]; const int* pi[NB];
+        const float* pa[NA]; const float* pb[NB];
         int b0, i0;
         if (stage_fast(rs, b0, i0)) {
             const float* Ast = A + ((size_t)b0 * w.rowsA + row0A + i0) * w.lda;
@@ -778,8 +775,7 @@
 #pragma unroll
             for (int k = 0; k < NB; ++k) {
                 const int r = b_row0 + k * BRS;
-                if (BMODE == 4) pi[k] = w.xc + brow + (r < RS ? r : b_row0);
-                else if (BMODE == 3) {
+                if (BMODE == 3) {
                     const unsigned row = use_tap ? (unsigned)tpv[k] : (unsigned)(row0B + i0 + (r < RS ? r : b_row0));
                     pb[k] = bsrc + __umul24(row, (unsigned)bstride);
                 } else pb[k] = bsrc + ((r < RS ? k * b_kstep : 0u) + b_voff);
@@ -801,7 +797,7 @@
                 int rr = rs + r; const bool ok = r < RS && rr < rend && !b_pad; rr = rr < rend ? rr : rend - 1;
                 int b, i; rowsplit(rr, b, i);
                 const size_t row = (size_t)b * w.rowsB + ((BMODE == 3 && use_tap) ? tpv[k] : row0B + i);
-                if (BMODE == 4) pi[k] = w.xc + row; else pb[k] = bbase + row * bstride;
+                pb[k] = bbase + row * bstride;
                 okB |= ok ? 1u << k : 0u;
             }
         }
@@ -813,11 +809,8 @@
         if (b_act) {
 #pragma unroll
             for (int k = 0; k < NB; ++k) {
-                if (BMODE == 4) rbi[k] = *pi[k];
-                else {
-                    rb[k] = *(const float4*)pb[k];
-                    if (BMODE == 2) rb2[k] = *(const float4*)(pb[k] + b2off);
-                }
+                rb[k] = *(const float4*)pb[k];
+                if (BMODE == 2) rb2[k] = *(const float4*)(pb[k] + b2off);
             }
         }
     };
@@ -842,9 +835,7 @@
             for (int k = 0; k < NB; ++k) {
                 const int r = b_row0 + k * BRS;
                 if (r < RS) {
-                    float4 v;
-                    if (BMODE == 4) { const int dlt = rbi[k] - n; v = make_float4(dlt == 0 ? 1.f : 0.f, dlt == 1 ? 1.f : 0.f, dlt == 2 ? 1.f : 0.f, dlt == 3 ? 1.f : 0.f); }
-                    else v = rb[k];
+                    float4 v = rb[k];
                     if (BMODE == 1) { v.x = fmaxf(v.x, 0.f); v.y = fmaxf(v.y, 0.f); v.z = fmaxf(v.z, 0.f); v.w = fmaxf(v.w, 0.f); }
                     else if (BMODE == 2) { v.x *= rb2[k].x; v.y *= rb2[k].y; v.z *= rb2[k].z; v.w *= rb2[k].w; }
                     { const bool ok = (okB >> k) & 1u; v.x = ok ? v.x : 0.f; v.y = ok ? v.y : 0.f; v.z = ok ? v.z : 0.f; v.w = ok ? v.w : 0.f; }
@@ -931,7 +922,6 @@
     return true;
 }
 static bool wgrad3_any(const Wg2& w, int nch, bool generic, hipStream_t stream) {
-    if (w.bmode == 4) return launch_wgrad3<4, 1, 8>(w, nch, stream) || launch_wgrad3<4, 1, 4>(w, nch, stream);
     if (generic) return false;
     switch (w.bmode) {
     case 3: return launch_wgrad3<3, 2, 11>(w, nch, stream) || launch_wgrad3<3, 2, 8>(w, nch, stream) || launch_wgrad3<3, 1, 7>(w, nch, stream);
@@ -949,7 +939,7 @@
 }
 
 static bool wgrad2_any(const Wg2& w, int nch, bool generic, hipStream_t stream) {
-    if (w.M > 256 && w.bmode != 4) {
+    if (w.M > 256) {
         bool ok = true;
         for (int m0 = 0; m0 < w.M && ok; m0 += 256) {
             Wg2 sub = w;
@@ -963,7 +953,6 @@
     }
     if (wgrad3_any(w, nch, generic, stream)) return true;
     switch (w.bmode) {
-    case 4: return false;
     case 1: return wgrad2_mode<1>(w, nch, stream);
     case 2: return wgrad2_mode<2>(w, nch, stream);
     case 3: return wgrad2_mode<3>(w, nch, stream);
@@ -971,10 +960,171 @@
     }
 }
 
+__device__ __forceinline__ int cr_wave_isum(int v) { for (int sft = 32; sft >= 1; sft >>= 1) v += __shfl_xor(v, sft); return v; }
+
+__global__ __launch_bounds__(256) void k_causal_index(CausalRows a) {
+    __shared__ int s_lt[4], s_eq[4];
+    const int q = blockIdx.x, b = blockIdx.y, lane = threadIdx.x & 63, wave = threadIdx.x >> 6;
+    const int n = a.N1 + 1;
+    const int* __restrict__ xc = a.xc + (size_t)b * n;
+    const int per = ((n + 3) / 4 + 63) / 64 * 64;
+    const int i0 = wave * per < n ? wave * per : n, i1 = i0 + per < n ? i0 + per : n;
+    int nlt = 0, neq = 0;
+#pragma unroll 8
+    for (int i = i0 + lane; i < i1; i += 64) { const int v = xc[i]; nlt += v < q ? 1 : 0; neq += v == q ? 1 : 0; }
+    nlt = cr_wave_isum(nlt); neq = cr_wave_isum(neq);
+    if (lane == 0) { s_lt[wave] = nlt; s_eq[wave] = neq; }
+    __syncthreads();
+    const int first = (s_lt[0] + s_lt[1]) + (s_lt[2] + s_lt[3]);
+    int run = first;
+    for (int w = 0; w < wave; ++w) run += s_eq[w];
+    if (threadIdx.x == 0) { a.cstart[(size_t)b * a.Q + q] = first; a.cnt[(size_t)b * a.Q + q] = (s_eq[0] + s_eq[1]) + (s_eq[2] + s_eq[3]); }
+    int* __restrict__ perm = a.perm + (size_t)b * n;
+    const unsigned long long below = (1ull << lane) - 1ull;
+    for (int base = i0; base < i1; base += 8 * 64) {
+        int v[8];
+#pragma unroll
+        for (int k = 0; k < 8; ++k) { const int i = base + 64 * k + lane; v[k] = i < i1 ? xc[i] : -1; }
+#pragma unroll
+        for (int k = 0; k < 8; ++k) {
+            const bool m = v[k] == q;
+            const unsigned long long bal = __ballot(m);
+            if (m) perm[run + __popcll(bal & below)] = base + 64 * k + lane;
+            run += __popcll(bal);
+        }
+    }
+}
+
+__device__ __forceinline__ float4 cr_add4(float4 x, float4 y) { return make_float4(x.x + y.x, x.y + y.y, x.z + y.z, x.w + y.w); }
+__device__ __forceinline__ float4 cr_sel4(bool ok, float4 x) { return make_float4(ok ? x.x : 0.f, ok ? x.y : 0.f, ok ? x.z : 0.f, ok ? x.w : 0.f); }
+__device__ __forceinline__ float4 cr_fold_rows(float4 s) {
+    s.x += __shfl_xor(s.x, 16); s.y += __shfl_xor(s.y, 16); s.z += __shfl_xor(s.z, 16); s.w += __shfl_xor(s.w, 16);
+    s.x += __shfl_xor(s.x, 32); s.y += __shfl_xor(s.y, 32); s.z += __shfl_xor(s.z, 32); s.w += __shfl_xor(s.w, 32);
+    return s;
+}
+
+__global__ __launch_bounds__(256) void k_causal_rowsum(CausalRows a) {
+    __shared__ int s_w[4];
+    __shared__ int s_base[CR_PPW], s_m[CR_PPW];
+    __shared__ float4 s_b[CR_PPW][16];
+    const int tid = threadIdx.x, lane = tid & 63, wave = tid >> 6, b = blockIdx.y;
+    const int Q = a.Q, C = a.C, N1 = a.N1;
+    const int* __restrict__ cnt = a.cnt + (size_t)b * Q;
+    const int* __restrict__ cstart = a.cstart + (size_t)b * Q;
+    if (tid < CR_PPW) s_m[tid] = 0;
+    const int cpt = (Q + 255) / 256, q0 = tid * cpt < Q ? tid * cpt : Q, q1 = q0 + cpt < Q ? q0 + cpt : Q;
+    int mine = 0;
+    for (int q = q0; q < q1; ++q) mine += (cnt[q] + CR_P - 1) / CR_P;
+    int inc = mine;
+    for (int d = 1; d < 64; d <<= 1) { const int v = __shfl_up(inc, d); if (lane >= d) inc += v; }
+    if (lane == 63) s_w[wave] = inc;
+    __syncthreads();
+    int pref = inc - mine;
+    for (int w = 0; w < wave; ++w) pref += s_w[w];
+    const int g0 = blockIdx.x * CR_PPW;
+    const bool writer = blockIdx.x == 0 && blockIdx.z == 0;
+    for (int q = q0; q < q1; ++q) {
+        const int n = cnt[q], np = (n + CR_P - 1) / CR_P;
+        if (writer) a.pstart[(size_t)b * Q + q] = pref;
+#pragma unroll
+        for (int k = 0; k < CR_PPW; ++k) {
+            const int io = g0 + k - pref;
+            if (io >= 0 && io < np) { s_base[k] = cstart[q] + io * CR_P; s_m[k] = n - io * CR_P < CR_P ? n - io * CR_P : CR_P; }
+        }
+        pref += np;
+    }
+    __syncthreads();
+    const int m = s_m[wave];
+    const int rg = lane >> 4, cl = lane & 15, c4 = blockIdx.z * 16 + cl;
+    const bool colok = c4 * 4 < C;
+    const int co = colok ? c4 * 4 : 0;
+    float4 s0 = make_float4(0.f, 0.f, 0.f, 0.f), s1 = s0;
+    if (m > 0) {
+        const int* __restrict__ perm = a.perm + (size_t)b * (N1 + 1) + s_base[wave];
+        const float* __restrict__ A = a.dxa + (size_t)b * N1 * C + co;
+        const float* __restrict__ Bq = a.dxb + (size_t)b * N1 * C + co;
+        int j[4];
+#pragma unroll
+        for (int k = 0; k < 4; ++k) { const int e = 4 * k + rg; j[k] = e < m ? perm[e] : -1; }
+        float4 xa0[4], xb0[4], xa1[4], xb1[4];
+#pragma unroll
+        for (int k = 0; k < 4; ++k) {
+            const size_t r0 = (j[k] >= 0 && j[k] < N1) ? (size_t)j[k] : 0, r1 = j[k] >= 1 ? (size_t)(j[k] - 1) : 0;
+            xa0[k] = *(const float4*)(A + r0 * C); xb0[k] = *(const float4*)(Bq + r0 * C);
+            xa1[k] = *(const float4*)(A + r1 * C); xb1[k] = *(const float4*)(Bq + r1 * C);
+        }
+        float4 v0[4], v1[4];
+#pragma unroll
+        for (int k = 0; k < 4; ++k) {
+            v0[k] = cr_sel4(j[k] >= 0 && j[k] < N1, cr_add4(xa0[k], xb0[k]));
+            v1[k] = cr_sel4(j[k] >= 1, cr_add4(xa1[k], xb1[k]));
+        }
+        s0 = cr_add4(cr_add4(v0[0], v0[1]), cr_add4(v0[2], v0[3]));
+        s1 = cr_add4(cr_add4(v1[0], v1[1]), cr_add4(v1[2], v1[3]));
+    }
+    s0 = cr_fold_rows(s0); s1 = cr_fold_rows(s1);
+    if (rg == 0) {
+        if (m > 0 && colok) {
+            float* o = a.part + (((size_t)b * a.MP + g0 + wave) * 2) * C + co;
+            *(float4*)o = s0; *(float4*)(o + C) = s1;
+        }
+        s_b[wave][cl] = s0;
+    }
+    __syncthreads();
+    if (tid < 16 && colok) *(float4*)(a.bpart + ((size_t)b * a.nwg + blockIdx.x) * C + co) = cr_add4(cr_add4(s_b[0][tid], s_b[1][tid]), cr_add4(s_b[2][tid], s_b[3][tid]));
+}
+
+#define CR_FG 8
+template <int NT>
+__device__ __forceinline__ void cr_list_sum(const float* __restrict__ src, unsigned off, unsigned stride, unsigned off1, int lo, int hi, float& a0, float& a1) {
+    for (int i = lo; i < hi; i += CR_FG) {
+        float v0[CR_FG], v1[CR_FG];
+#pragma unroll
+        for (int k = 0; k < CR_FG; ++k) {
+            const unsigned o = off + (unsigned)(i + k < hi ? i + k : hi - 1) * stride;
+            v0[k] = src[o]; if (NT == 2) v1[k] = src[o + off1];
+        }
+#pragma unroll
+        for (int k = 0; k < CR_FG; ++k) { a0 += i + k < hi ? v0[k] : 0.f; if (NT == 2) a1 += i + k < hi ? v1[k] : 0.f; }
+    }
+}
+__device__ __forceinline__ void causal_fold(const CausalRows& a, const int blk) {
+    __shared__ float s_r[4][2][64];
+    const int lane = threadIdx.x & 63, wave = threadIdx.x >> 6;
+    const int C = a.C, Q = a.Q;
+    const bool bias = blk == Q;
+    for (int c0 = 0; c0 < C; c0 += 64) {
+        const int c = c0 + lane;
+        const bool ok = c < C;
+        const int cc = ok ? c : 0;
+        float a0 = 0.f, a1 = 0.f;
+        if (bias) {
+            const int n = a.B * a.nwg;
+            cr_list_sum<1>(a.bpart, (unsigned)cc, (unsigned)C, 0u, (int)((int64_t)n * wave / 4), (int)((int64_t)n * (wave + 1) / 4), a0, a1);
+        } else {
+            for (int b = 0; b < a.B; ++b) {
+                const int np = (a.cnt[(size_t)b * Q + blk] + CR_P - 1) / CR_P, ps = a.pstart[(size_t)b * Q + blk];
+                cr_list_sum<2>(a.part + ((size_t)b * a.MP + ps) * 2 * C, (unsigned)cc, 2u * (unsigned)C, (unsigned)C, (int)((int64_t)np * wave / 4), (int)((int64_t)np * (wave + 1) / 4), a0, a1);
+            }
+        }
+        s_r[wave][0][lane] = a0; s_r[wave][1][lane] = a1;
+        __syncthreads();
+        if (wave < 2 && ok && !(bias && wave == 1)) {
+            const float s = ((s_r[0][wave][lane] + s_r[1][wave][lane]) + (s_r[2][wave][lane] + s_r[3][wave][lane])) * a.scale;
+            if (bias) a.gb[c] = s; else a.gw[((size_t)c * Q + blk) * 2 + wave] = s;
+        }
+        __syncthreads();
+    }
+}
+#ifdef QPN_TESTING
+__global__ __launch_bounds__(256) void k_test_causal_fold(CausalRows a) { causal_fold(a, blockIdx.x); }
+#endif
+
 __global__ void k_reduce_grad_s(const float* __restrict__ slab, const int* __restrict__ gdst, const int* __restrict__ gdst_list, const int* __restrict__ gzero, int n_gzero,
                                 int nch, int gstage, int64_t n, float* __restrict__ g, float scale, int append_scale, int s0, int s1, int skip0, int skip1, int tail,
-                                const int* __restrict__ status, int flag_again) {
-    int64_t i = (int64_t)blockIdx.x * blockDim.x + threadIdx.x + s0;
+                                const int* __restrict__ status, int flag_again, CausalRows cf) {
+    if ((int)blockIdx.x < cf.nblk) { causal_fold(cf, blockIdx.x); return; }
+    int64_t i = (int64_t)((int)blockIdx.x - cf.nblk) * blockDim.x + threadIdx.x + s0;
     if (flag_again && append_scale && i == s0) g[n + 1] = (status && *status) ? 1.f : 0.f;
     if (i < s1) {
         if (i >= skip0 && i < skip1) return;
@@ -998,44 +1148,6 @@
     const int64_t j = i - s1;
     if (j < n_gzero) g[gzero[j]] = 0.f;
     else if (append_scale && j < n_gzero + 4 && !(flag_again && j == n_gzero + 1)) g[n + (j - n_gzero)] = j == n_gzero ? scale : (j == n_gzero + 1 && status && *status) ? 1.f : 0.f;
-}
-
-__global__ __launch_bounds__(256) void k_causal_bwd(TrainParams p, TrainBwd bw, int rows_per_wg, int CB) {
-    extern __shared__ float tab[];
-    const int C = p.C, Q = p.Q;
-    const int tid = threadIdx.x;
-    const int64_t total = (int64_t)p.B * p.N1;
-    const int64_t r0 = (int64_t)blockIdx.x * rows_per_wg, r1 = r0 + rows_per_wg < total ? r0 + rows_per_wg : total;
-    for (int cb = 0; cb < C; cb += CB) {
-        const int cbv = C - cb < CB ? C - cb : CB;
-        for (int i = tid; i < 2 * Q * CB; i += 256) tab[i] = 0.f;
-        __syncthreads();
-        const int cpr = cbv;
-        for (int64_t idx = r0 * cpr + tid; idx < r1 * cpr; idx += 256) {
-            const int64_t rr = idx / cpr; const int c = (int)(idx - rr * cpr);
-            const int b = (int)(rr / p.N1), n = (int)(rr - (int64_t)b * p.N1);
-            const size_t o = ((size_t)b * p.N1 + n) * C + cb + c;
-            const float v = bw.DXA[0][o] + bw.DXB[0][o];
-            const int64_t xo = (int64_t)p.T - p.N0 + n;
-            int64_t s0 = p.x[(size_t)b * p.T + xo] % Q, s1 = p.x[(size_t)b * p.T + xo + 1] % Q;
-            if (s0 < 0) s0 += Q;
-            if (s1 < 0) s1 += Q;
-            atomicAdd(&tab[(0 * Q + s0) * CB + c], v);
-            atomicAdd(&tab[(1 * Q + s1) * CB + c], v);
-        }
-        __syncthreads();
-        for (int i = tid; i < 2 * Q * cbv; i += 256) {
-            const int c = i / (2 * Q), qt = i - c * 2 * Q, q = qt >> 1, tp = qt & 1;
-            const float v = tab[(tp * Q + q) * CB + c];
-            if (v != 0.f) atomicAdd(&bw.gflat[p.causal_w + ((size_t)(cb + c) * Q + q) * 2 + tp], v * bw.gscale);
-        }
-        for (int c = tid; c < cbv; c += 256) {
-            float s = 0.f;
-            for (int q = 0; q < Q; ++q) s += tab[(0 * Q + q) * CB + c];
-            atomicAdd(&bw.gflat[p.causal_b + cb + c], s * bw.gscale);
-        }
-        __syncthreads();
-    }
 }
 
 __global__ __launch_bounds__(128) void k_up_bwd(UpArgs u) { up_bwd_body(u, blockIdx.x, blockIdx.y, threadIdx.x, 128); }
@@ -1231,8 +1343,9 @@
 static void launch_reduce_early(const TrainBwd& bw, hipStream_t st, int tail, int nch_side) {
     const TrainSlabs& sl = *bw.sl;
     const int64_t n = (int64_t)(sl.g_early1 - sl.g_early0) + (tail ? bw.n_gzero + 4 : 0);
+    CausalRows nofold; memset(&nofold, 0, sizeof(nofold));
     hipLaunchKernelGGL(k_reduce_grad_s, dim3((unsigned)((n + 255) / 256)), dim3(256), 0, st, bw.slab, bw.gdst, bw.gdst_list, bw.gzero, bw.n_gzero,
-                       nch_side, bw.gstage, bw.n_params, bw.gflat, bw.gscale, bw.append_scale, sl.g_early0, sl.g_early1, 0, 0, tail, bw.status, 0);
+                       nch_side, bw.gstage, bw.n_params, bw.gflat, bw.gscale, bw.append_scale, sl.g_early0, sl.g_early1, 0, 0, tail, bw.status, 0, nofold);
 }
 static void launch_up_bwd(const TrainParams& p, const TrainBwd& bw, hipStream_t st) {
     const UpArgs u = up_args(p, bw);
@@ -1243,25 +1356,21 @@
     hipLaunchKernelGGL(k_aux_tail, dim3(p.L * p.A + p.U), dim3(128), 0, st, tr_aux_args(p, &bw, ag));
 }
 
-int qpn_launch_grad_tail(const TrainParams& p, const TrainBwd& bw, const AuxGeom* ag, hipStream_t stream, bool early_done, bool up_done) {
-    const int C = p.C, Q = p.Q, B = p.B, N1 = p.N1;
+void qpn_launch_causal_index(const CausalRows& a, hipStream_t st) { hipLaunchKernelGGL(k_causal_index, dim3(a.Q, a.B), dim3(256), 0, st, a); }
+void qpn_launch_causal_rowsum(const CausalRows& a, hipStream_t st) { hipLaunchKernelGGL(k_causal_rowsum, dim3(a.nwg, a.B, (a.C + 63) / 64), dim3(256), 0, st, a); }
+#ifdef QPN_TESTING
+void qpn_test_launch_causal_fold(const CausalRows& a, hipStream_t st) { hipLaunchKernelGGL(k_test_causal_fold, dim3(a.Q + 1), dim3(256), 0, st, a); }
+#endif
+
+int qpn_launch_grad_tail(const TrainParams& p, const TrainBwd& bw, const AuxGeom* ag, hipStream_t stream, bool early_done, bool up_done, bool causal_done) {
     const TrainSlabs& sl = *bw.sl;
-    hipLaunchKernelGGL(k_reduce_grad_s, dim3((unsigned)(((int64_t)bw.gstage + (up_done ? 0 : bw.n_gzero + 4) + 255) / 256)), dim3(256), 0, stream, bw.slab, bw.gdst, bw.gdst_list, bw.gzero, bw.n_gzero,
-                       bw.nch, bw.gstage, bw.n_params, bw.gflat, bw.gscale, bw.append_scale, 0, bw.gstage, early_done ? sl.g_early0 : 0, early_done ? sl.g_early1 : 0, up_done ? 0 : 1, bw.status, bw.append_scale == 1 ? 1 : 0);
-    {
-        const int64_t total = (int64_t)B * N1;
-        const int nwg = 128, rpw = (int)((total + nwg - 1) / nwg);
-        if (sl.g_cw < 0) {
-            int CB = C < 64 ? C : 64;
-            while (CB > 1 && (size_t)2 * Q * CB * sizeof(float) > 128 * 1024) CB /= 2;
-            const size_t lds_c = (size_t)2 * Q * CB * sizeof(float);
-            if (lds_c > 160 * 1024) { qpn_set_error("causal-table gradient: n_quantize too large for the LDS histogram"); return QPN_EINVAL; }
-            if (lds_c > 48 * 1024) QPN_HIP(hipFuncSetAttribute((const void*)k_causal_bwd, hipFuncAttributeMaxDynamicSharedMemorySize, (int)lds_c));
-            hipLaunchKernelGGL(k_causal_bwd, dim3(nwg), dim3(256), lds_c, stream, p, bw, rpw, CB);
-        }
-        if (p.U > 0 && !up_done && !p.hoist) launch_up_bwd(p, bw, stream);
-        if (p.hoist && ag && !up_done) launch_aux_tail(p, bw, *ag, stream);
-    }
+    if (!causal_done) { qpn_launch_causal_index(*bw.cr, stream); qpn_launch_causal_rowsum(*bw.cr, stream); qpn_prof_mark(PG_WGRAD_CAUSAL, stream); }
+    CausalRows cf = *bw.cr;
+    cf.gw = bw.gflat + p.causal_w; cf.gb = bw.gflat + p.causal_b; cf.scale = bw.gscale; cf.nblk = cf.Q + 1;
+    hipLaunchKernelGGL(k_reduce_grad_s, dim3((unsigned)(cf.nblk + ((int64_t)bw.gstage + (up_done ? 0 : bw.n_gzero + 4) + 255) / 256)), dim3(256), 0, stream, bw.slab, bw.gdst, bw.gdst_list, bw.gzero, bw.n_gzero,
+                       bw.nch, bw.gstage, bw.n_params, bw.gflat, bw.gscale, bw.append_scale, 0, bw.gstage, early_done ? sl.g_early0 : 0, early_done ? sl.g_early1 : 0, up_done ? 0 : 1, bw.status, bw.append_scale == 1 ? 1 : 0, cf);
+    if (p.U > 0 && !up_done && !p.hoist) launch_up_bwd(p, bw, stream);
+    if (p.hoist && ag && !up_done) launch_aux_tail(p, bw, *ag, stream);
     qpn_prof_mark(PG_GRAD_TAIL, stream);
     QPN_HIP(hipGetLastError());
     return QPN_OK;
@@ -1375,6 +1484,8 @@
         launch_skip_post(side);
         if (early_reduce) { launch_reduce_early(bw, side, up_side ? 1 : 0, nch_side_); qpn_prof_mark(PG_GRAD_TAIL, side); }
         if (early_reduce && up_side && bw.ev_early && bw.early_recorded) { QPN_HIP(hipEventRecord(bw.ev_early, side)); *bw.early_recorded = 1; }
+        qpn_launch_causal_index(*bw.cr, side); qpn_prof_mark(PG_WGRAD_CAUSAL, side);
+        QPN_HIP(hipEventRecord(bw.ev_idx, side));
     }
     const int swz = k.xcd_swizzle ? 1 : 0;
     if (p.hoist && !persist) { qpn_set_error("internal: the frame-rate aux term needs the register-resident layer kernels"); return QPN_EINVAL; }
@@ -1406,14 +1517,6 @@
             hipLaunchKernelGGL((k_layer_bwd<1>), dim3(tiles, B), dim3(256), lds_layer, stream, p, bw, l, l == L - 1 ? 1 : 0, swz);
         }
     }
-    auto build_causal = [&]() {
-        Wg2 w = wbase;
-        w.nlayers = 2; w.ncol_groups = Q / (Q % 64 == 0 ? 64 : 128);      w.bmode = 4; w.xc = p.XC; w.B1 = w.B2 = nullptr; w.B_lstride = 0;
-        w.A = bw.DXA[0]; w.A2 = bw.DXB[0]; w.A_lstride = 0; w.lda = C; w.M = C; w.rowsA = N1;
-        w.N = Q; w.Nvalid = Q; w.rowsB = N1 + 1; w.ldb = 0; w.ldc = Q;
-        for (int tp = 0; tp < 2; ++tp) { w.row0A[tp] = 0; w.row0B[tp] = tp; w.R[tp] = N1; w.goff[tp] = sl.g_cw + tp * C * Q; w.gbias[tp] = tp == 0 ? sl.g_cb : -1; w.tap_off[tp] = -1; w.dil[tp] = 0; }
-        return w;
-    };
     const bool wr_side = overlap && k.wr_side;
     if (wr_side || up_side) {
         QPN_HIP(hipEventRecord(bw.ev_mid, stream));
@@ -1428,11 +1531,12 @@
     qpn_prof_mark(PG_WGRAD, stream);
     if (!wr_side) { ok = ok && wgrad2_any(build_wr(), nch, gen, stream); qpn_prof_mark(PG_WGRAD_WR, stream); }
     if (!overlap) launch_skip_post(stream);
-    if (sl.g_cw >= 0) ok = ok && wgrad2_any(build_causal(), nch, gen, stream);
+    if (overlap) QPN_HIP(hipStreamWaitEvent(stream, bw.ev_idx, 0)); else qpn_launch_causal_index(*bw.cr, stream);
+    qpn_launch_causal_rowsum(*bw.cr, stream);
     qpn_prof_mark(PG_WGRAD_CAUSAL, stream);
     if (overlap) { QPN_HIP(hipStreamWaitEvent(stream, ev_join, 0)); qpn_prof_mark(-1, stream); }
     if (!ok) { qpn_set_error("weight-gradient tiles: unsupported geometry (n_resch <= 128 on this path; wider stacks take the GEMM path)"); return QPN_EINVAL; }
-    return qpn_launch_grad_tail(p, bw, &ag, stream, early_reduce, up_side);
+    return qpn_launch_grad_tail(p, bw, &ag, stream, early_reduce, up_side, true);
 }
 
 int qpn_launch_adam(float* w, const float* g, float* m, float* v, int64_t n, int step, float lr, float b1, float b2, float eps, float wd, const float* den, int* status,
diff --git a/qpnet_amd/csrc/train_common.h b/qpnet_amd/csrc/train_common.h
--- a/qpnet_amd/csrc/train_common.h
+++ b/qpnet_amd/csrc/train_common.h
@@ -58,8 +58,27 @@
     int g_w1[TR_MAXL], g_b1[TR_MAXL], g_wr[TR_MAXL], g_br[TR_MAXL], g_ws[TR_MAXL], g_bs;
     int g_p1, g_bp1, g_p2, g_bp2;
     int g_early0, g_early1;
-    int g_cw, g_cb;
-};
+};
+
+#define CR_P 16
+#define CR_PPW 4
+struct CausalRows {
+    const int* xc;
+    const float* dxa; const float* dxb;
+    int* perm;
+    int* cnt; int* cstart;
+    int* pstart;
+    float* part;
+    float* bpart;
+    float* gw; float* gb; float scale;
+    int C, Q, B, N1;
+    int MP, nwg;
+    int nblk;
+};
+static inline void tr_causal_geom(CausalRows& a, int C, int Q, int B, int N1) {
+    a.C = C; a.Q = Q; a.B = B; a.N1 = N1;
+    a.MP = (N1 + 1 + CR_P - 1) / CR_P + Q; a.nwg = (a.MP + CR_PPW - 1) / CR_PPW;
+}
 
 struct TrainBwd {
     const float* dlogits; float* gflat;
@@ -82,6 +101,8 @@
     const int* status;
     hipStream_t side; hipEvent_t ev_fork, ev_join, ev_mid;
     hipEvent_t ev_early; int* early_recorded;
+    const struct CausalRows* cr;
+    hipEvent_t ev_idx;
 };
 
 
diff --git a/qpnet_amd/csrc/train_gemm.hip b/qpnet_amd/csrc/train_gemm.hip
--- a/qpnet_amd/csrc/train_gemm.hip
+++ b/qpnet_amd/csrc/train_gemm.hip
@@ -477,7 +477,7 @@
 }
 
 void qpn_launch_zero_dx(const TrainParams& p, const TrainBwd& bw, hipStream_t stream);
-int qpn_launch_grad_tail(const TrainParams& p, const TrainBwd& bw, const AuxGeom* ag, hipStream_t stream, bool early_done, bool up_done);
+int qpn_launch_grad_tail(const TrainParams& p, const TrainBwd& bw, const AuxGeom* ag, hipStream_t stream, bool early_done, bool up_done, bool causal_done);
 
 static void launch_post_wgrad_gemm(const TrainParams& p, const TrainBwd& bw, hipStream_t stream) {
     TArgs a; memset(&a, 0, sizeof(a));
@@ -571,5 +571,5 @@
     }
     launch_post_wgrad_gemm(p, bw, stream);
     qpn_prof_mark(PG_WGRAD, stream);
-    return qpn_launch_grad_tail(p, bw, nullptr, stream, false, false);
-}
+    return qpn_launch_grad_tail(p, bw, nullptr, stream, false, false, false);
+}
diff --git a/qpnet_amd/csrc/train_host.hip b/qpnet_amd/csrc/train_host.hip
--- a/qpnet_amd/csrc/train_host.hip
+++ b/qpnet_amd/csrc/train_host.hip
@@ -9,6 +9,8 @@
 int qpn_launch_bwd(const TrainParams& p, const TrainBwd& bw, const TrainKnobs& k, const AuxGeom& ag, const StackQ* sq, hipStream_t stream, bool post_done);
 int qpn_launch_fwd_gemm(const TrainParams& p, const TrainGemm& w, hipStream_t stream);
 int qpn_launch_bwd_gemm(const TrainParams& p, const TrainBwd& bw, const TrainGemm& w, hipStream_t stream);
+void qpn_launch_causal_index(const CausalRows& a, hipStream_t st);
+void qpn_launch_causal_rowsum(const CausalRows& a, hipStream_t st);
 int qpn_launch_adam(float* w, const float* g, float* m, float* v, int64_t n, int step, float lr, float b1, float b2, float eps, float wd, const float* den, int* status,
                     int* h_status, double* h_loss, const double* d_loss, hipStream_t stream);
 int qpn_launch_adam_clip(float* w, const float* g, float* m, float* v, int64_t n, int step, float lr, float b1, float b2, float eps, float wd, const float* den, int* status,
@@ -26,6 +28,7 @@
     TrainParams tp;
     TrainBwd bw;
     TrainSlabs slabs;
+    CausalRows cr;
     TrainKnobs knobs;
     AuxGeom ag;
     float* d_ws; size_t ws_cap;
@@ -44,7 +47,7 @@
     std::vector<int> h_gmap; int* d_gmap; float* d_gwp;
     TrainGemm gm;
     int64_t generation;
-    hipStream_t side; hipEvent_t ev_fork, ev_join, ev_mid;
+    hipStream_t side; hipEvent_t ev_fork, ev_join, ev_mid, ev_idx;
     hipEvent_t ev_early; int early_recorded; int64_t early_first;
     int64_t bwd_generation;
     const float* post_bwd_dlogits;
@@ -188,10 +191,10 @@
     t->d_wmap = nullptr; t->d_wp = nullptr; t->d_bstart = t->d_blist = nullptr; t->d_bp = nullptr;
     t->d_gdst = t->d_gdst_list = t->d_gzero = nullptr; t->n_gzero = 0;
     t->d_ws = nullptr; t->ws_cap = 0; t->d_tap = nullptr; t->tap_cap = 0; t->d_status = nullptr; t->d_loss = nullptr; t->fwd_valid = false; t->loss_clear = false;
-    t->generation = 0; t->side = nullptr; t->ev_fork = t->ev_join = t->ev_mid = nullptr; t->ev_early = nullptr; t->early_recorded = 0; t->early_first = -1;
+    t->generation = 0; t->side = nullptr; t->ev_fork = t->ev_join = t->ev_mid = t->ev_idx = nullptr; t->ev_early = nullptr; t->early_recorded = 0; t->early_first = -1;
     t->d_sq = nullptr; t->sq_pos_cap = 0; t->sq_per_dir = 0; t->bwd_generation = -1; t->stack_disabled = false; memset(&t->sqf, 0, sizeof(t->sqf)); memset(&t->sqb, 0, sizeof(t->sqb));
     qpn_train_knobs_parse(t->knobs);
-    memset(&t->slabs, 0, sizeof(t->slabs));
+    memset(&t->slabs, 0, sizeof(t->slabs)); memset(&t->cr, 0, sizeof(t->cr));
     t->use_gemm = (C > 128 || getenv("QPN_TRAIN_GEMM")) && !getenv("QPN_TRAIN_TILES");
     t->d_gmap = nullptr; t->d_gwp = nullptr; t->d_ctmap = nullptr; t->d_ct = nullptr; memset(&t->gm, 0, sizeof(t->gm));
     if (t->use_gemm && (C % 32 || S % 32 || Q % 32)) { qpn_set_error("the GEMM training path needs n_resch, n_skipch, n_quantize multiples of 32"); delete t; return QPN_EINVAL; }
@@ -276,7 +279,7 @@
 
     TrainBwd& bw = t->bw;
     TrainSlabs& sl = t->slabs;
-    bw.sl = &t->slabs;
+    bw.sl = &t->slabs; bw.cr = &t->cr;
     int go = 0;
     auto gtake = [&](int n) { int r = go; go += (n + 63) & ~63; return r; };
     std::vector<int>& gs = t->h_gsrc;
@@ -315,14 +318,8 @@
     t->early_first = (g.post1_b == g.post1_w + (int64_t)S * S && g.post2_w == g.post1_b + S && g.post2_b == g.post2_w + (int64_t)Q * S && g.post2_b + Q == g.n_params) ? g.post1_w : -1;
     for (int o = 0; o < S; ++o) { for (int s = 0; s < S; ++s) gs[g.post1_w + (int64_t)o * S + s] = sl.g_p1 + o * S + s; gs[g.post1_b + o] = sl.g_bp1 + o; }
     for (int q = 0; q < Q; ++q) { for (int s = 0; s < S; ++s) gs[g.post2_w + (int64_t)q * S + s] = sl.g_p2 + q * S + s; gs[g.post2_b + q] = sl.g_bp2 + q; }
-    sl.g_cw = sl.g_cb = -1;
-    if (C == 64 && Q % 128 == 0 && !t->use_gemm) {
-        sl.g_cw = gtake(2 * C * Q); sl.g_cb = gtake(C);
-        for (int c = 0; c < C; ++c) {
-            for (int q = 0; q < Q; ++q) for (int tp = 0; tp < 2; ++tp) gs[g.causal_w + ((int64_t)c * Q + q) * 2 + tp] = sl.g_cw + tp * C * Q + c * Q + q;
-            gs[g.causal_b + c] = sl.g_cb + c;
-        }
-    }
+    for (int64_t i = 0; i < (int64_t)2 * C * Q; ++i) gs[g.causal_w + i] = -2;
+    for (int c = 0; c < C; ++c) gs[g.causal_b + c] = -2;
     bw.gstage = go; bw.nch = t->use_gemm ? 4 : 64; bw.n_params = g.n_params;
     if (t->knobs.wgrad_chunks > 0) bw.nch = t->knobs.wgrad_chunks;
     if (t->hoist) for (int j = 0; j < g.U; ++j) gs[g.up_w + j] = -2;
@@ -387,6 +384,7 @@
     QPN_HIP(hipEventCreateWithFlags(&t->ev_fork, evf));
     QPN_HIP(hipEventCreateWithFlags(&t->ev_join, evf));
     QPN_HIP(hipEventCreateWithFlags(&t->ev_mid, evf));
+    QPN_HIP(hipEventCreateWithFlags(&t->ev_idx, evf));
     QPN_HIP(hipEventCreateWithFlags(&t->ev_early, evf));
     h->train = t;
     return QPN_OK;
@@ -404,6 +402,7 @@
     if (t->ev_fork) (void)hipEventDestroy(t->ev_fork);
     if (t->ev_join) (void)hipEventDestroy(t->ev_join);
     if (t->ev_mid) (void)hipEventDestroy(t->ev_mid);
+    if (t->ev_idx) (void)hipEventDestroy(t->ev_idx);
     if (t->ev_early) (void)hipEventDestroy(t->ev_early);
     delete t;
 }
@@ -453,7 +452,10 @@
     const size_t nDX = (size_t)B * N1 * C, nDZ = (size_t)B * N1 * 2 * C, nDGS = (size_t)B * BL * L * C, nSlab = (size_t)bw.nch * bw.gstage;
     const size_t nXC = (size_t)B * (N1 + 1);
     const size_t nScr = (size_t)B * 1024 * 2 * 128;
-    size_t need = nScr + nX + 2 * nG + nH + 2 * (nS + 96 * (size_t)S + 64) + 2 * (size_t)(L + 1) * nDX + (size_t)L * nDZ + 2 * nS + nDGS + nH + nSlab + nXC + (t->use_gemm ? nG : 0) + 2 * nPA + nWJ + nGW + (size_t)L * TR_EB_SLOTS * 2 * C + 8192;
+    CausalRows& cr = t->cr;
+    tr_causal_geom(cr, C, g.Q, B, N1);
+    const size_t nCQ = (size_t)B * g.Q, nCP = (size_t)B * cr.MP * 2 * C, nCB = (size_t)B * cr.nwg * C;
+    size_t need = nXC + 3 * nCQ + nCP + nCB + 6 * 64 + nScr + nX + 2 * nG + nH + 2 * (nS + 96 * (size_t)S + 64) + 2 * (size_t)(L + 1) * nDX + (size_t)L * nDZ + 2 * nS + nDGS + nH + nSlab + nXC + (t->use_gemm ? nG : 0) + 2 * nPA + nWJ + nGW + (size_t)L * TR_EB_SLOTS * 2 * C + 8192;
     if (need > t->ws_cap) {
         if (t->d_ws) (void)hipFree(t->d_ws);
         t->d_ws = nullptr; t->ws_cap = 0;
@@ -474,6 +476,8 @@
     bw.DXA[0] = carve((size_t)(L + 1) * nDX); bw.DXB[0] = carve((size_t)(L + 1) * nDX); bw.DXA[1] = bw.DXB[1] = nullptr;
     bw.DZ = carve((size_t)L * nDZ); bw.DS0 = carve(nS); bw.DY0 = carve(nS); bw.DGS = carve(nDGS); bw.DHUP = carve(nH); bw.slab = carve(nSlab);
     p.XC = (int*)carve(nXC);
+    cr.xc = p.XC; cr.dxa = bw.DXA[0]; cr.dxb = bw.DXB[0];
+    cr.perm = (int*)carve(nXC); cr.cnt = (int*)carve(nCQ); cr.cstart = (int*)carve(nCQ); cr.pstart = (int*)carve(nCQ); cr.part = carve(nCP); cr.bpart = carve(nCB);
     p.scratch_rows = carve(nScr);
     if (t->use_gemm) t->gm.G = carve(nG);
     p.PA = nullptr; p.WJ = nullptr; bw.DPA = nullptr; bw.GW = nullptr;
@@ -717,6 +721,28 @@
     QPN_HIP(hipMemcpyAsync(d_y0, p.Y0, sizeof(float) * (size_t)n, hipMemcpyDeviceToDevice, (hipStream_t)stream_));
     return QPN_OK;
 }
+void qpn_test_launch_causal_fold(const CausalRows& a, hipStream_t st);
+extern "C" int qpn_test_causal_table_grad(qpn_handle* h, int C, int Q, int B, int N1, const int* d_xc, const float* d_dxa, const float* d_dxb, float scale,
+                                          float* d_w, float* d_b, void* stream_) {
+    int rc = need_dev(h); if (rc) return rc;
+    if (C < 4 || C % 4 || Q < 1 || B < 1 || N1 < 1 || !d_xc || !d_dxa || !d_dxb || !d_w || !d_b) { qpn_set_error("bad causal_table_grad arguments"); return QPN_EINVAL; }
+    hipStream_t stream = (hipStream_t)stream_;
+    CausalRows a; memset(&a, 0, sizeof(a));
+    tr_causal_geom(a, C, Q, B, N1);
+    a.xc = d_xc; a.dxa = d_dxa; a.dxb = d_dxb; a.gw = d_w; a.gb = d_b; a.scale = scale;
+    const size_t nXC = (size_t)B * (N1 + 1), nCQ = (size_t)B * Q, nCP = (size_t)B * a.MP * 2 * C, nCB = (size_t)B * a.nwg * C;
+    int* ibuf = nullptr; float* fbuf = nullptr;
+    QPN_HIP(hipMalloc(&ibuf, (nXC + 3 * nCQ) * sizeof(int)));
+    if (hipMalloc(&fbuf, (nCP + nCB) * sizeof(float)) != hipSuccess) { (void)hipFree(ibuf); qpn_set_error("causal_table_grad: out of device memory"); return QPN_ENOMEM; }
+    a.perm = ibuf; a.cnt = ibuf + nXC; a.cstart = a.cnt + nCQ; a.pstart = a.cstart + nCQ; a.part = fbuf; a.bpart = fbuf + nCP;
+    qpn_launch_causal_index(a, stream);
+    qpn_launch_causal_rowsum(a, stream);
+    qpn_test_launch_causal_fold(a, stream);
+    const hipError_t e1 = hipGetLastError(), e2 = hipStreamSynchronize(stream);
+    (void)hipFree(ibuf); (void)hipFree(fbuf);
+    if (e1 != hipSuccess || e2 != hipSuccess) { qpn_set_error("causal_table_grad: %s", hipGetErrorString(e1 != hipSuccess ? e1 : e2)); return QPN_ENODEV; }
+    return QPN_OK;
+}
 #endif
 
 extern "C" int64_t qpn_train_generation(qpn_handle* h) { return (h && h->train) ? h->train->generation : 0; }
@@ -733,7 +759,7 @@
     TrainBwd& bw = t->bw;
     bw.dlogits = d_dlogits; bw.gflat = d_flatgrad; bw.gdst = t->d_gdst; bw.gdst_list = t->d_gdst_list; bw.gzero = t->d_gzero; bw.n_gzero = t->n_gzero;
     bw.gscale = grad_scale; bw.append_scale = append_scale; bw.status = h->train->d_status;
-    bw.side = t->side; bw.ev_fork = t->ev_fork; bw.ev_join = t->ev_join; bw.ev_mid = t->ev_mid;
+    bw.side = t->side; bw.ev_fork = t->ev_fork; bw.ev_join = t->ev_join; bw.ev_mid = t->ev_mid; bw.ev_idx = t->ev_idx;
     t->early_recorded = 0; bw.ev_early = t->ev_early; bw.early_recorded = (append_scale && t->early_first >= 0) ? &t->early_recorded : nullptr;
     const bool first_bwd = t->bwd_generation != t->generation;
     t->bwd_generation = t->generation;
```
